# musbenlahrech/reporter

Measured on AMD Instinct MI355X. Metric: GPS points map-matched/sec (node) at 1/2/4/8 MI355X; % of HBM peak, higher is better.
Workload: dtype f32 geometry / f64 Viterbi + times / u64 (dist,time) route keys

## Files before the change

include/reporter_match.h:

```cpp
#ifndef REPORTER_MATCH_H
#define REPORTER_MATCH_H
#include <stddef.h>
#include <stdint.h>

#ifdef __cplusplus
extern "C" {
#endif

#define RM_ABI_VERSION 1

const char* rm_last_error(void);
int rm_abi_version(void);
int rm_set_device(int device);
int rm_device_count(int* count);

typedef struct rm_matcher rm_matcher;
int rm_configure(const char* conf_json_path, char* err, size_t errlen);
rm_matcher* rm_matcher_create(void);
void rm_matcher_destroy(rm_matcher* m);
int rm_match(rm_matcher* m, const char* trace_json, char** out_json);
int rm_match_batch(rm_matcher* m, const char* const* traces, size_t n, char** outs);
int rm_match_batch_packed(rm_matcher* m, const char* const* traces, size_t n, char** buf, uint64_t* off);
int rm_match_points(rm_matcher* m, const char* trace_json, char** out_json);
int rm_match_points_batch(rm_matcher* m, const char* const* traces, size_t n, char** outs);
void rm_free(char* p);
int rm_matcher_timing(const rm_matcher* m, double out[6]);
int rm_coalesce_stats(uint64_t out[4]);
int rm_coalesce_timing(double out[4]);

typedef struct {
  int32_t mode;
  float sigma_z, beta, search_radius, gps_accuracy, breakage_distance, interpolation_distance,
      max_route_distance_factor, max_route_time_factor, turn_penalty_factor;
} rm_options;
void rm_default_options(rm_options* o);

typedef struct {
  uint32_t rows, cols;
  double block_m;
  uint64_t seed;
  double center_lat, center_lon, jitter;
  uint32_t arterial_every, highway_every;
  double segment_max_m, internal_m, service_frac, oneway_frac, curve_frac, cell_m;
} rm_world_params;
void rm_default_world_params(rm_world_params* p);
int rm_world_build(const rm_world_params* p, const char* out_path);
int rm_graph_info(const char* graph_path, uint64_t out[7]);
int rm_graph_export_osm(const char* graph_path, const char* osm_path);
int rm_graph_export_pbf(const char* graph_path, const char* pbf_path);
int rm_graph_import_osm(const char* osm_path, const char* graph_path, double cell_m);
typedef struct {
  uint32_t rows, cols;
  double block_m;
  uint64_t seed;
  double center_lat, center_lon, jitter;
  uint32_t primary_every, secondary_every, boulevard_every, diagonal_every;
  double roundabout_frac, drop_frac, oneway_frac, spur_frac, service_frac, footway_frac, osmlr_local_frac,
      way_max_m;
  uint32_t trunk;
} rm_city_params;
void rm_default_city_params(rm_city_params* p);
int rm_osm_city_write(const rm_city_params* p, const char* osm_path, int pbf);

typedef struct {
  uint32_t n_traces, n_points;
  double rate_s, noise_m;
  uint64_t seed;
  int32_t mode;
  int64_t start_epoch;
  uint32_t threads;
} rm_trace_params;
void rm_default_trace_params(rm_trace_params* p);
int rm_traces_generate(const char* graph_path, const rm_trace_params* p, double* lon, double* lat, double* time,
                       float* accuracy, uint32_t* truth_edge, uint32_t* truth_off_cm);
int rm_traces_generate_ids(const char* graph_path, const rm_trace_params* p, const uint32_t* ids, double* lon,
                           double* lat, double* time, float* accuracy, uint32_t* truth_edge, uint32_t* truth_off_cm);

typedef struct rm_engine rm_engine;
typedef struct rm_runner rm_runner;

rm_engine* rm_engine_create(const char* graph_path, int device);
void rm_engine_destroy(rm_engine* e);
uint32_t rm_engine_n_segments(const rm_engine* e);
int rm_engine_segment_ids(const rm_engine* e, uint64_t* ids);
int rm_engine_set_ball_radius(rm_engine* e, double radius_m);
int rm_graph_auto_ball_radius(const char* graph_path, double* radius_m);
int rm_graph_fit_ball_radius(const char* graph_path, int mode, double start_m, double avail_gb, double* radius_m);
int rm_graph_ball_sample(const char* graph_path, int mode, double radius_m, double out[3]);
int rm_engine_ball_stats(const rm_engine* e, int mode, double out[6]);
int rm_engine_grid_split(const rm_engine* e, uint32_t* f);
int rm_engine_grid_alt(const rm_engine* e, uint32_t* f, float* radius_m);
int rm_engine_turn_rows(const rm_engine* e, uint32_t* mode_mask, double* build_ms );
int rm_graph_grid_split(const char* graph_path, uint32_t* f);
int rm_engine_ball_lookup(rm_engine* e, int mode, uint64_t n, const uint32_t* from, const uint32_t* road,
                          uint64_t* keys, uint8_t* preds);
int rm_balls_lookup(const char* graph_path, int mode, double radius_m, uint64_t n, const uint32_t* from,
                    const uint32_t* road, uint64_t* keys, uint8_t* preds);

rm_runner* rm_runner_create(rm_engine* e);
void rm_runner_destroy(rm_runner* r);

typedef struct {
  uint32_t n_traces;
  const uint32_t* trace_off;
  const float* lon;
  const float* lat;
  const double* time;
  const float* accuracy;
  uint32_t n_opts;
  const rm_options* opts;
  const uint32_t* trace_opt;
} rm_batch_desc;

typedef struct {
  double threshold_sec;
  uint32_t report_mask;
  uint32_t transition_mask;
  uint32_t* hist_dev;
  int32_t do_report;
  int32_t zero_hist;
  uint64_t* dur_dev;
} rm_run_params;
void rm_default_run_params(rm_run_params* p);

int rm_runner_run(rm_runner* r, const rm_batch_desc* b, const rm_run_params* p);
int rm_runner_rerun(rm_runner* r, const rm_run_params* p);
int rm_runners_rerun(rm_runner* const* rs, uint32_t n, const rm_run_params* p);
int rm_runner_sizes(rm_runner* r, uint64_t out[10]);
int rm_runner_route_tiers(rm_runner* r, uint64_t out[10]);
int rm_runner_get_states(rm_runner* r, uint32_t* n_states, uint32_t* state_orig);
int rm_runner_get_candidates(rm_runner* r, uint8_t* cand_n, uint32_t* road, uint32_t* s_cm, float* sq);
int rm_runner_get_routes(rm_runner* r, uint32_t* trans_off, double* gc, uint32_t* route_cm);
int rm_runner_get_route_terms(rm_runner* r, double* route_d, int* present);
int rm_runner_get_viterbi(rm_runner* r, int8_t* choice, uint8_t* chain_start);
int rm_runner_get_paths(rm_runner* r, uint32_t* path_off, uint32_t* path_cnt, uint32_t* path_edges, uint32_t* route_dist);
typedef struct {
  float lon, lat;
  float sq;
  uint32_t edge;
  uint32_t off_cm;
  uint32_t way;
  uint32_t type;
  uint32_t route_cm;
} rm_matched_point;
int rm_runner_get_matched_points(rm_runner* r, rm_matched_point* out);
int rm_runner_get_segments(rm_runner* r, uint32_t* seg_off, void* segs);
int rm_runner_get_reports(rm_runner* r, uint32_t* rep_off, void* reps, void* stats);
int rm_runner_set_isolation(rm_runner* r, int on);
int rm_runner_trace_errors(rm_runner* r, uint32_t* errs);
int rm_runner_set_locality(rm_runner* r, int mode);
int rm_runner_locality_used(rm_runner* r, int* used);
int rm_runner_set_timing(rm_runner* r, int on);
int rm_runner_set_timing_mask(rm_runner* r, uint32_t mask);
int rm_runner_kernel_times(rm_runner* r, double* ms, uint64_t* launches, int n);
int rm_runner_reset_times(rm_runner* r);
const char* rm_kernel_name(int k);
int rm_num_kernels(void);

typedef struct {
  uint32_t n_traces;
  const uint32_t* seg_off;
  const void* segs;
  const double* trace_end_time;
  const double* threshold_sec;
  const uint32_t* report_mask;
  const uint32_t* transition_mask;
} rm_report_desc;
int rm_report_segments(const rm_report_desc* d, uint32_t* rep_off, void* reps, void* stats);

typedef struct rm_comm rm_comm;
typedef struct {
  uint64_t n_points;
  const uint32_t* uuid;
  const double* time;
  const float* lon;
  const float* lat;
  const float* accuracy;
  double inactivity_sec;
  uint32_t n_uuids;
  uint32_t n_opts;
  const rm_options* opts;
  const uint32_t* uuid_opt;
} rm_points_desc;
int rm_runner_run_points(rm_runner* r, const rm_points_desc* d, const rm_run_params* p);
int rm_runner_get_trace_uuid(rm_runner* r, uint32_t* uuid);
int rm_runner_get_batch(rm_runner* r, uint32_t* trace_off, float* lon, float* lat, double* time, float* accuracy);
typedef struct {
  uint32_t quantisation;
  uint32_t privacy;
  const char* source;
  const char* mode;
} rm_tile_params;
void rm_default_tile_params(rm_tile_params* p);
int rm_runner_tiles(rm_runner* r, const rm_tile_params* p, rm_comm* comm, char** blob, size_t* len);

int rm_comm_unique_id(uint8_t id_out[128]);
rm_comm* rm_comm_init(int nranks, int rank, const uint8_t id[128], int device);
void rm_comm_destroy(rm_comm* c);
int rm_comm_allreduce(rm_comm* c, void* dev_buf, size_t count, int dtype, int op);
int rm_comm_reduce_scatter(rm_comm* c, void* buf, size_t count_per_rank, int dtype, int op);
int rm_comm_allreduce_host_f64(rm_comm* c, double* value, int op);
int rm_comm_barrier(rm_comm* c);
typedef int (*rm_host_allgather_fn)(void* ctx, const void* send, size_t bytes, void* recv);
rm_comm* rm_comm_init_host(int nranks, int rank, rm_host_allgather_fn fn, void* ctx, int device);
int rm_tile_file_owner(uint64_t bucket, uint32_t tile, int nranks);

int rm_device_alloc(size_t bytes, void** dev_ptr);
int rm_device_free(void* dev_ptr);
int rm_device_memset(void* dev_ptr, int value, size_t bytes);
int rm_device_download(void* host_dst, const void* dev_src, size_t bytes);
int rm_device_upload(void* dev_dst, const void* host_src, size_t bytes);
int rm_device_synchronize(void);

#ifdef __cplusplus
}
#endif
#endif
```

reporter_amd/_lib.py:

```python
import ctypes as C
import os
import threading

_HERE = os.path.dirname(os.path.abspath(__file__))
LIB_PATH = os.environ.get("REPORTER_MATCH_LIB") or os.path.join(_HERE, "libreporter_match.so")

_lock = threading.Lock()
_lib = None


class RmOptions(C.Structure):
    _fields_ = [("mode", C.c_int32), ("sigma_z", C.c_float), ("beta", C.c_float), ("search_radius", C.c_float),
                ("gps_accuracy", C.c_float), ("breakage_distance", C.c_float), ("interpolation_distance", C.c_float),
                ("max_route_distance_factor", C.c_float), ("max_route_time_factor", C.c_float),
                ("turn_penalty_factor", C.c_float)]


class RmWorldParams(C.Structure):
    _fields_ = [("rows", C.c_uint32), ("cols", C.c_uint32), ("block_m", C.c_double), ("seed", C.c_uint64),
                ("center_lat", C.c_double), ("center_lon", C.c_double), ("jitter", C.c_double),
                ("arterial_every", C.c_uint32), ("highway_every", C.c_uint32), ("segment_max_m", C.c_double),
                ("internal_m", C.c_double), ("service_frac", C.c_double), ("oneway_frac", C.c_double),
                ("curve_frac", C.c_double), ("cell_m", C.c_double)]


class RmCityParams(C.Structure):
    _fields_ = [("rows", C.c_uint32), ("cols", C.c_uint32), ("block_m", C.c_double), ("seed", C.c_uint64),
                ("center_lat", C.c_double), ("center_lon", C.c_double), ("jitter", C.c_double),
                ("primary_every", C.c_uint32), ("secondary_every", C.c_uint32), ("boulevard_every", C.c_uint32),
                ("diagonal_every", C.c_uint32), ("roundabout_frac", C.c_double), ("drop_frac", C.c_double),
                ("oneway_frac", C.c_double), ("spur_frac", C.c_double), ("service_frac", C.c_double),
                ("footway_frac", C.c_double), ("osmlr_local_frac", C.c_double), ("way_max_m", C.c_double),
                ("trunk", C.c_uint32)]


class RmTraceParams(C.Structure):
    _fields_ = [("n_traces", C.c_uint32), ("n_points", C.c_uint32), ("rate_s", C.c_double),
                ("noise_m", C.c_double), ("seed", C.c_uint64), ("mode", C.c_int32), ("start_epoch", C.c_int64),
                ("threads", C.c_uint32)]


class RmBatchDesc(C.Structure):
    _fields_ = [("n_traces", C.c_uint32), ("trace_off", C.c_void_p), ("lon", C.c_void_p), ("lat", C.c_void_p),
                ("time", C.c_void_p), ("accuracy", C.c_void_p), ("n_opts", C.c_uint32),
                ("opts", C.c_void_p), ("trace_opt", C.c_void_p)]


class RmRunParams(C.Structure):
    _fields_ = [("threshold_sec", C.c_double), ("report_mask", C.c_uint32), ("transition_mask", C.c_uint32),
                ("hist_dev", C.c_void_p), ("do_report", C.c_int32), ("zero_hist", C.c_int32),
                ("dur_dev", C.c_void_p)]


class RmPointsDesc(C.Structure):
    _fields_ = [("n_points", C.c_uint64), ("uuid", C.c_void_p), ("time", C.c_void_p), ("lon", C.c_void_p),
                ("lat", C.c_void_p), ("accuracy", C.c_void_p), ("inactivity_sec", C.c_double),
                ("n_uuids", C.c_uint32), ("n_opts", C.c_uint32), ("opts", C.c_void_p), ("uuid_opt", C.c_void_p)]


class RmReportDesc(C.Structure):
    _fields_ = [("n_traces", C.c_uint32), ("seg_off", C.c_void_p), ("segs", C.c_void_p),
                ("trace_end_time", C.c_void_p), ("threshold_sec", C.c_void_p), ("report_mask", C.c_void_p),
                ("transition_mask", C.c_void_p)]


class RmMatchedPoint(C.Structure):
    _fields_ = [("lon", C.c_float), ("lat", C.c_float), ("sq", C.c_float), ("edge", C.c_uint32),
                ("off_cm", C.c_uint32), ("way", C.c_uint32), ("type", C.c_uint32), ("route_cm", C.c_uint32)]


class RmTileParams(C.Structure):
    _fields_ = [("quantisation", C.c_uint32), ("privacy", C.c_uint32), ("source", C.c_char_p), ("mode", C.c_char_p)]


P = C.c_void_p
U32P = C.POINTER(C.c_uint32)

PROTOTYPES = [
    ("rm_last_error", C.c_char_p, []),
    ("rm_abi_version", C.c_int, []),
    ("rm_set_device", C.c_int, [C.c_int]),
    ("rm_device_count", C.c_int, [C.POINTER(C.c_int)]),
    ("rm_configure", C.c_int, [C.c_char_p, C.c_char_p, C.c_size_t]),
    ("rm_matcher_create", P, []),
    ("rm_matcher_destroy", None, [P]),
    ("rm_match", C.c_int, [P, C.c_char_p, C.POINTER(P)]),
    ("rm_match_batch", C.c_int, [P, C.POINTER(C.c_char_p), C.c_size_t, C.POINTER(P)]),
    ("rm_match_batch_packed", C.c_int, [P, C.POINTER(C.c_char_p), C.c_size_t, C.POINTER(P), C.POINTER(C.c_uint64)]),
    ("rm_match_points", C.c_int, [P, C.c_char_p, C.POINTER(P)]),
    ("rm_match_points_batch", C.c_int, [P, C.POINTER(C.c_char_p), C.c_size_t, C.POINTER(P)]),
    ("rm_free", None, [P]),
    ("rm_matcher_timing", C.c_int, [P, P]),
    ("rm_coalesce_stats", C.c_int, [C.POINTER(C.c_uint64)]),
    ("rm_coalesce_timing", C.c_int, [C.POINTER(C.c_double)]),
    ("rm_default_options", None, [C.POINTER(RmOptions)]),
    ("rm_default_world_params", None, [C.POINTER(RmWorldParams)]),
    ("rm_world_build", C.c_int, [C.POINTER(RmWorldParams), C.c_char_p]),
    ("rm_graph_info", C.c_int, [C.c_char_p, C.POINTER(C.c_uint64)]),
    ("rm_graph_export_osm", C.c_int, [C.c_char_p, C.c_char_p]),
    ("rm_graph_export_pbf", C.c_int, [C.c_char_p, C.c_char_p]),
    ("rm_graph_import_osm", C.c_int, [C.c_char_p, C.c_char_p, C.c_double]),
    ("rm_default_city_params", None, [C.POINTER(RmCityParams)]),
    ("rm_osm_city_write", C.c_int, [C.POINTER(RmCityParams), C.c_char_p, C.c_int]),
    ("rm_default_trace_params", None, [C.POINTER(RmTraceParams)]),
    ("rm_traces_generate", C.c_int, [C.c_char_p, C.POINTER(RmTraceParams), P, P, P, P, P, P]),
    ("rm_traces_generate_ids", C.c_int, [C.c_char_p, C.POINTER(RmTraceParams), P, P, P, P, P, P, P]),
    ("rm_engine_create", P, [C.c_char_p, C.c_int]),
    ("rm_engine_destroy", None, [P]),
    ("rm_engine_n_segments", C.c_uint32, [P]),
    ("rm_engine_segment_ids", C.c_int, [P, P]),
    ("rm_engine_set_ball_radius", C.c_int, [P, C.c_double]),
    ("rm_engine_ball_stats", C.c_int, [P, C.c_int, P]),
    ("rm_engine_grid_split", C.c_int, [P, P]),
    ("rm_engine_grid_alt", C.c_int, [P, P, P]),
    ("rm_engine_turn_rows", C.c_int, [P, P, P]),
    ("rm_engine_ball_lookup", C.c_int, [P, C.c_int, C.c_uint64, P, P, P, P]),
    ("rm_runner_route_tiers", C.c_int, [P, P]),
    ("rm_balls_lookup", C.c_int, [C.c_char_p, C.c_int, C.c_double, C.c_uint64, P, P, P, P]),
    ("rm_graph_auto_ball_radius", C.c_int, [C.c_char_p, P]),
    ("rm_graph_fit_ball_radius", C.c_int, [C.c_char_p, C.c_int, C.c_double, C.c_double, P]),
    ("rm_graph_ball_sample", C.c_int, [C.c_char_p, C.c_int, C.c_double, P]),
    ("rm_graph_grid_split", C.c_int, [C.c_char_p, P]),
    ("rm_runner_create", P, [P]),
    ("rm_runner_destroy", None, [P]),
    ("rm_default_run_params", None, [C.POINTER(RmRunParams)]),
    ("rm_runner_run", C.c_int, [P, C.POINTER(RmBatchDesc), C.POINTER(RmRunParams)]),
    ("rm_runner_rerun", C.c_int, [P, C.POINTER(RmRunParams)]),
    ("rm_runners_rerun", C.c_int, [P, C.c_uint32, C.POINTER(RmRunParams)]),
    ("rm_runner_sizes", C.c_int, [P, C.POINTER(C.c_uint64)]),
    ("rm_runner_get_states", C.c_int, [P, P, P]),
    ("rm_runner_get_candidates", C.c_int, [P, P, P, P, P]),
    ("rm_runner_get_routes", C.c_int, [P, P, P, P]),
    ("rm_runner_get_route_terms", C.c_int, [P, P, P]),
    ("rm_runner_get_viterbi", C.c_int, [P, P, P]),
    ("rm_runner_get_paths", C.c_int, [P, P, P, P, P]),
    ("rm_runner_get_matched_points", C.c_int, [P, P]),
    ("rm_runner_get_segments", C.c_int, [P, P, P]),
    ("rm_runner_get_reports", C.c_int, [P, P, P, P]),
    ("rm_runner_set_timing", C.c_int, [P, C.c_int]),
    ("rm_runner_set_timing_mask", C.c_int, [P, C.c_uint32]),
    ("rm_runner_set_isolation", C.c_int, [P, C.c_int]),
    ("rm_runner_trace_errors", C.c_int, [P, P]),
    ("rm_runner_set_locality", C.c_int, [P, C.c_int]),
    ("rm_runner_locality_used", C.c_int, [P, C.POINTER(C.c_int)]),
    ("rm_report_segments", C.c_int, [C.POINTER(RmReportDesc), P, P, P]),
    ("rm_runner_kernel_times", C.c_int, [P, P, P, C.c_int]),
    ("rm_runner_reset_times", C.c_int, [P]),
    ("rm_kernel_name", C.c_char_p, [C.c_int]),
    ("rm_num_kernels", C.c_int, []),
    ("rm_runner_run_points", C.c_int, [P, C.POINTER(RmPointsDesc), C.POINTER(RmRunParams)]),
    ("rm_runner_get_trace_uuid", C.c_int, [P, P]),
    ("rm_runner_get_batch", C.c_int, [P, P, P, P, P, P]),
    ("rm_default_tile_params", None, [C.POINTER(RmTileParams)]),
    ("rm_runner_tiles", C.c_int, [P, C.POINTER(RmTileParams), P, C.POINTER(P), C.POINTER(C.c_size_t)]),
    ("rm_comm_unique_id", C.c_int, [P]),
    ("rm_comm_init", P, [C.c_int, C.c_int, P, C.c_int]),
    ("rm_comm_destroy", None, [P]),
    ("rm_comm_allreduce", C.c_int, [P, P, C.c_size_t, C.c_int, C.c_int]),
    ("rm_comm_reduce_scatter", C.c_int, [P, P, C.c_size_t, C.c_int, C.c_int]),
    ("rm_comm_allreduce_host_f64", C.c_int, [P, C.POINTER(C.c_double), C.c_int]),
    ("rm_comm_barrier", C.c_int, [P]),
    ("rm_comm_init_host", P, [C.c_int, C.c_int, P, P, C.c_int]),
    ("rm_tile_file_owner", C.c_int, [C.c_uint64, C.c_uint32, C.c_int]),
    ("rm_device_alloc", C.c_int, [C.c_size_t, C.POINTER(P)]),
    ("rm_device_free", C.c_int, [P]),
    ("rm_device_memset", C.c_int, [P, C.c_int, C.c_size_t]),
    ("rm_device_download", C.c_int, [P, P, C.c_size_t]),
    ("rm_device_upload", C.c_int, [P, P, C.c_size_t]),
    ("rm_device_synchronize", C.c_int, []),
]


def lib():
    global _lib
    if _lib is not None:
        return _lib
    with _lock:
        if _lib is None:
            if not os.path.exists(LIB_PATH):
                raise ImportError("libreporter_match.so not built at %s (run python -m reporter_amd.build)" % LIB_PATH)
            h = C.CDLL(LIB_PATH)
            for name, res, args in PROTOTYPES:
                f = getattr(h, name)
                f.restype = res
                f.argtypes = args
            _lib = h
    return _lib


class RmError(RuntimeError):
    pass


def check(rc):
    if rc != 0:
        raise RmError(lib().rm_last_error().decode("utf-8", "replace"))
    return rc


def last_error():
    return lib().rm_last_error().decode("utf-8", "replace")
```

reporter_amd/csrc/capi.cpp:

```cpp
#include <hip/hip_runtime.h>
#include <rccl/rccl.h>

#include <atomic>
#include <sys/resource.h>
#include <cctype>
#include <chrono>
#include <cmath>
#include <condition_variable>
#include <deque>
#include <thread>
#include <vector>
#include <cstdio>
#include <cstring>
#include <memory>
#include <mutex>
#include <string>

#include "../../include/reporter_match.h"
#include "engine.hpp"
#include "graph.hpp"
#include "host_pool.hpp"
#include "json.hpp"
#include "osm_model.hpp"
#include "serve_policy.hpp"
// ... 1099 lines not shown
}

int rm_graph_grid_split(const char* graph_path, uint32_t* f) {
  return guarded([&] {
    if (!f) throw std::runtime_error("f is NULL");
    *f = choose_grid_split(Graph::load(graph_path));
  });
}

int rm_graph_auto_ball_radius(const char* graph_path, double* radius_m) {
  return guarded([&] {
    if (!radius_m) throw std::runtime_error("radius_m is NULL");
    *radius_m = auto_ball_radius_cm(Graph::load(graph_path)) / 100.0;
  });
}

int rm_graph_fit_ball_radius(const char* graph_path, int mode, double start_m, double avail_gb, double* radius_m) {
  return guarded([&] {
    if (!graph_path || !radius_m) throw std::runtime_error("path or radius_m is NULL");
    if (mode < 0 || mode > kModePedestrian) throw std::runtime_error("unknown travel mode");
    if (!(start_m >= 0.0) || start_m * 100.0 > kBallMaxRadiusCm) throw std::runtime_error("ball radius out of range (0..10000 m)");
    if (!(avail_gb >= 0.0)) throw std::runtime_error("avail_gb must be non-negative");
    const uint64_t avail = (uint64_t)std::min(avail_gb * (double)(1ull << 30), 1.8e19);
    *radius_m = fit_ball_radius_cm(Graph::load(graph_path), mode, (uint32_t)(start_m * 100.0), avail) / 100.0;
  });
}

int rm_graph_ball_sample(const char* graph_path, int mode, double radius_m, double out[3]) {
  return guarded([&] {
    if (!graph_path || !out) throw std::runtime_error("path or out is NULL");
    if (mode < 0 || mode > kModePedestrian) throw std::runtime_error("unknown travel mode");
    if (!(radius_m >= 0.0) || radius_m * 100.0 > kBallMaxRadiusCm) throw std::runtime_error("ball radius out of range (0..10000 m)");
    const BallSample bs = sample_balls(Graph::load(graph_path), (uint32_t)(radius_m * 100.0), kBallMaxKeysHost, mode);
    out[0] = bs.nodes; out[1] = bs.table_bytes; out[2] = bs.skipped_frac;
  });
}

int rm_balls_lookup(const char* graph_path, int mode, double radius_m, uint64_t n, const uint32_t* from,
                    const uint32_t* road, uint64_t* keys, uint8_t* preds) {
  return guarded([&] {
    if (mode < 0 || mode > kModePedestrian) throw std::runtime_error("unknown travel mode");
    if (!(radius_m >= 0.0) || radius_m * 100.0 > kBallMaxRadiusCm) throw std::runtime_error("ball radius out of range (0..10000 m)");
    Graph g = Graph::load(graph_path);
    BallTables bt;
    build_balls(g, mode, (uint32_t)(radius_m * 100.0), kBallMaxKeysHost, 4, bt);
    for (uint64_t i = 0; i < n; ++i) {
      keys[2 * i] = keys[2 * i + 1] = kKeyInf;
      if (preds) preds[2 * i] = preds[2 * i + 1] = (uint8_t)kBallPredNone;
      if (from[i] >= g.num_nodes() || road[i] >= g.num_roads()) throw std::runtime_error("node or road out of range");
      const uint32_t off = bt.hdr[2 * (size_t)from[i]], bits = bt.hdr[2 * (size_t)from[i] + 1];
      if (!bits) continue;
      const uint32_t mask = (1u << bits) - 1u;
      for (uint32_t s = ball_slot(road[i], bits);; s = (s + 1) & mask) {
        const uint32_t* e = bt.ent.data() + 4 * (ball_row0(off) + s);
        if (e[0] == kNone) break;
        if ((e[0] & bt.road_mask) != road[i]) continue;
        keys[2 * i] = ball_key0(e[0], e[1], e[3]);
        keys[2 * i + 1] = ball_key1(e[0], e[2], e[3]);
        if (preds) {
          preds[2 * i] = (uint8_t)ball_pred(e[0], 0, bt.road_mask);
          preds[2 * i + 1] = (uint8_t)ball_pred(e[0], 1, bt.road_mask);
        }
        break;
      }
    }
  });
}

rm_runner* rm_runner_create(rm_engine* e) {
  rm_runner* out = nullptr;
  guarded([&] {
    if (!e) throw std::runtime_error("engine is NULL");
    auto r = std::make_unique<rm_runner>();
    r->e = e->e;
    r->m = std::make_unique<Matcher>(e->e.get());
    out = r.release();
  });
  return out;
}
void rm_runner_destroy(rm_runner* r) { delete r; }

void rm_default_run_params(rm_run_params* p) {
  p->threshold_sec = 15.0; p->report_mask = 0x6; p->transition_mask = 0x6; p->hist_dev = nullptr; p->do_report = 1;
  p->zero_hist = 0; p->dur_dev = nullptr;
}

static RunParams to_rp(const rm_run_params* p) {
  RunParams rp;
  if (p) {
    rp.threshold_sec = p->threshold_sec; rp.report_mask = p->report_mask; rp.transition_mask = p->transition_mask;
    rp.hist = p->hist_dev; rp.do_report = p->do_report; rp.zero_hist = p->zero_hist;
    rp.dur = (unsigned long long*)p->dur_dev;
  }
  return rp;
}

int rm_runner_run(rm_runner* r, const rm_batch_desc* b, const rm_run_params* p) {
  return guarded([&] {
    HostBatch hb;
    hb.n_traces = b->n_traces; hb.trace_off = b->trace_off; hb.lon = b->lon; hb.lat = b->lat; hb.time = b->time;
    hb.accuracy = b->accuracy; hb.n_opts = b->n_opts; hb.opts = (const MatchOptions*)b->opts; hb.trace_opt = b->trace_opt;
    r->m->run(hb, to_rp(p));
  });
}
int rm_runner_rerun(rm_runner* r, const rm_run_params* p) { return guarded([&] { r->m->run_device(to_rp(p)); }); }

int rm_runners_rerun(rm_runner* const* rs, uint32_t n, const rm_run_params* p) {
  return guarded([&] {
    if (!rs || n == 0) throw std::runtime_error("no runners");
    for (uint32_t i = 0; i < n; ++i)
      if (!rs[i]) throw std::runtime_error("runner is NULL");
    RunParams rp = to_rp(p);
    if ((rp.hist || rp.dur) && rp.zero_hist && rp.do_report) {
      hipStream_t st = rs[0]->m->stream();
      const size_t nseg = rs[0]->m->engine().n_segments();
      if (rp.hist) RM_HIP(hipMemsetAsync(rp.hist, 0, nseg * kHistBins * sizeof(uint32_t), st));
      if (rp.dur) RM_HIP(hipMemsetAsync(rp.dur, 0, nseg * 8u, st));
      RM_HIP(hipStreamSynchronize(st));
    }
    rp.zero_hist = false;
    std::vector<std::exception_ptr> err(n);
    std::vector<std::thread> th;
    th.reserve(n - 1);
    for (uint32_t i = 1; i < n; ++i)
      th.emplace_back([&, i] {
        try { rs[i]->m->run_device(rp); } catch (...) { err[i] = std::current_exception(); }
      });
    try { rs[0]->m->run_device(rp); } catch (...) { err[0] = std::current_exception(); }
    for (auto& t : th) t.join();
    for (auto& e : err)
      if (e) std::rethrow_exception(e);
  });
}
int rm_runner_sizes(rm_runner* r, uint64_t out[10]) {
  return guarded([&] {
    out[0] = r->m->n_points(); out[1] = r->m->n_traces(); out[2] = r->m->n_trans(); out[3] = r->m->n_path_edges();
    out[4] = r->m->count_segments(); out[5] = r->m->count_reports();
    uint32_t t[4];
    r->m->tier_counts(t);
    for (int i = 0; i < 4; ++i) out[6 + i] = t[i];
  });
}
int rm_runner_route_tiers(rm_runner* r, uint64_t out[10]) {
  return guarded([&] {
    uint32_t c[kCtlWords];
    r->m->ctl_words(c);
    out[0] = c[1]; out[1] = c[3]; out[2] = c[5]; out[3] = c[8]; out[4] = c[9]; out[5] = c[10];
    out[6] = c[11]; out[7] = c[12]; out[8] = c[13]; out[9] = c[14];
#ifdef RM_K2_STATS
    out[9] = c[15];
#endif
  });
}
int rm_runner_get_states(rm_runner* r, uint32_t* a, uint32_t* b) { return guarded([&] { r->m->get_states(a, b); }); }
int rm_runner_get_candidates(rm_runner* r, uint8_t* a, uint32_t* b, uint32_t* c, float* d) {
  return guarded([&] { r->m->get_candidates(a, b, c, d); });
}
int rm_runner_get_routes(rm_runner* r, uint32_t* a, double* b, uint32_t* c) { return guarded([&] { r->m->get_routes(a, b, c); }); }
int rm_runner_get_route_terms(rm_runner* r, double* a, int* present) {
  return guarded([&] { *present = r->m->get_route_terms(a); });
}
int rm_runner_get_viterbi(rm_runner* r, int8_t* a, uint8_t* b) { return guarded([&] { r->m->get_viterbi(a, b); }); }
int rm_runner_get_paths(rm_runner* r, uint32_t* a, uint32_t* b, uint32_t* c, uint32_t* d) {
  return guarded([&] { r->m->get_paths(a, b, c, d); });
}
int rm_runner_get_matched_points(rm_runner* r, rm_matched_point* out) {
  static_assert(sizeof(rm_matched_point) == sizeof(MatchedPoint), "rm_matched_point is rm::MatchedPoint");
  return guarded([&] { r->m->matched_points(reinterpret_cast<MatchedPoint*>(out)); });
}
int rm_runner_get_segments(rm_runner* r, uint32_t* off, void* segs) {
  return guarded([&] { r->m->get_segments(off, (SegmentRec*)segs); });
}
int rm_runner_get_reports(rm_runner* r, uint32_t* off, void* reps, void* stats) {
  return guarded([&] { r->m->get_reports(off, (ReportRec*)reps, (ReportStats*)stats); });
}
int rm_runner_set_timing(rm_runner* r, int on) { return guarded([&] { r->m->set_timing(on != 0); }); }
int rm_runner_set_timing_mask(rm_runner* r, uint32_t mask) { return guarded([&] { r->m->set_timing_mask(mask); }); }
int rm_runner_set_isolation(rm_runner* r, int on) { return guarded([&] { r->m->set_isolation(on != 0); }); }
int rm_runner_set_locality(rm_runner* r, int mode) {
  return guarded([&] {
    if (mode < -1 || mode > 2) throw std::runtime_error("locality mode must be -1, 0, 1 or 2");
    r->m->set_locality(mode);
  });
}
int rm_runner_locality_used(rm_runner* r, int* used) { return guarded([&] { *used = r->m->locality_used() ? 1 : 0; }); }
int rm_runner_trace_errors(rm_runner* r, uint32_t* errs) { return guarded([&] { r->m->get_trace_errors(errs); }); }
int rm_report_segments(const rm_report_desc* d, uint32_t* rep_off, void* reps, void* stats) {
  return guarded([&] {
    if (!d || !rep_off || (d->n_traces && (!d->seg_off || !d->trace_end_time || !d->threshold_sec || !d->report_mask ||
                                           !d->transition_mask || !stats)))
      throw std::runtime_error("report descriptor or output is NULL");
    report_segments(g_device, d->n_traces, d->seg_off, (const SegmentRec*)d->segs, d->trace_end_time, d->threshold_sec,
                    d->report_mask, d->transition_mask, rep_off, (ReportRec*)reps, (ReportStats*)stats);
  });
}
int rm_runner_kernel_times(rm_runner* r, double* ms, uint64_t* launches, int n) {
  return guarded([&] {
    double t[kNumKernels];
    uint64_t l[kNumKernels];
    r->m->sync();
    r->m->kernel_times(t, l);
    for (int i = 0; i < n && i < kNumKernels; ++i) { ms[i] = t[i]; if (launches) launches[i] = l[i]; }
  });
}
int rm_runner_reset_times(rm_runner* r) { return guarded([&] { r->m->reset_kernel_times(); }); }
const char* rm_kernel_name(int k) { return (k >= 0 && k < kNumKernels) ? kKernelNames[k] : ""; }
int rm_num_kernels(void) { return kNumKernels; }

}

struct rm_comm {
  ncclComm_t comm = nullptr;
  hipStream_t stream = nullptr;
  void* scratch = nullptr;
  int device = 0;
  int rank = 0, nranks = 1;
  rm_host_allgather_fn host_fn = nullptr;
  void* host_ctx = nullptr;
  std::atomic<bool> broken{false};
};

namespace {
double comm_timeout_s();
bool comm_timeout_exit() {
  const char* e = std::getenv("RM_COMM_TIMEOUT_EXIT");
  return !(e && *e == '0');
}

constexpr uint32_t kWatchSlots = 64;
struct CommWatch {
  std::atomic<uint64_t> deadline_ns[kWatchSlots];
  const char* what[kWatchSlots];
  int rank[kWatchSlots], nranks[kWatchSlots], limit_s[kWatchSlots];
  CommWatch() {
    for (uint32_t i = 0; i < kWatchSlots; ++i) deadline_ns[i].store(0);
  }
};
CommWatch& comm_watch() {
  static CommWatch* w = [] {
    CommWatch* x = new CommWatch();
    std::thread([x] {
      for (;;) {
        std::this_thread::sleep_for(std::chrono::milliseconds(50));
        const uint64_t now = (uint64_t)std::chrono::duration_cast<std::chrono::nanoseconds>(
                                 std::chrono::steady_clock::now().time_since_epoch()).count();
        for (uint32_t i = 0; i < kWatchSlots; ++i) {
          const uint64_t d = x->deadline_ns[i].load(std::memory_order_acquire);
          if (d && now > d) {
            std::fprintf(stderr, "%s: rank %d of %d: the other ranks did not join within %d s (RM_COMM_TIMEOUT_S); "
                                 "exiting with status 3\n", x->what[i], x->rank[i], x->nranks[i], x->limit_s[i]);
            std::fflush(stderr);
            std::_Exit(3);
          }
        }
      }
    }).detach();
    return x;
  }();
  return *w;
}
uint32_t comm_watch_slot() {
  static std::atomic<uint32_t> next{0};
  thread_local const uint32_t slot = next.fetch_add(1) % kWatchSlots;
  return slot;
}

template <class F>
void comm_bounded(rm_comm* c, int rank, int nranks, const char* what, F fn) {
  if (c && c->broken.load()) throw std::runtime_error(std::string(what) + ": the communicator missed a deadline earlier and is unusable");
  const double limit = comm_timeout_s();
  struct St {
    std::mutex mu;
    std::condition_variable cv;
    bool done = false;
    std::exception_ptr err;
  };
  auto st = std::make_shared<St>();
  if (comm_timeout_exit()) {
    CommWatch& w = comm_watch();
    const uint32_t slot = comm_watch_slot();
    w.what[slot] = what;
    w.rank[slot] = rank;
    w.nranks[slot] = nranks;
    w.limit_s[slot] = (int)limit;
    const auto now = std::chrono::steady_clock::now().time_since_epoch();
    w.deadline_ns[slot].store((uint64_t)std::chrono::duration_cast<std::chrono::nanoseconds>(now).count() +
                              (uint64_t)(limit * 1e9), std::memory_order_release);
    try {
      fn();
    } catch (...) {
      w.deadline_ns[slot].store(0, std::memory_order_release);
      throw;
    }
    w.deadline_ns[slot].store(0, std::memory_order_release);
    return;
  }
  std::thread worker([st, fn]() mutable {
    std::exception_ptr e;
    try {
      fn();
    } catch (...) {
      e = std::current_exception();
    }
    std::lock_guard<std::mutex> lk(st->mu);
    st->err = e;
    st->done = true;
// ... 345 lines not shown
```

reporter_amd/csrc/engine.hip:

```cpp
#include <hip/hip_runtime.h>
#include <hipcub/hipcub.hpp>

#include <algorithm>
#include <chrono>
#include <cstdlib>
#include <cstring>
#include <functional>
#include <thread>
#include <type_traits>

#include "engine.hpp"
#include "json_points.hpp"

namespace rm {

const char* const kKernelNames[kNumKernels] = {"states", "candidates", "scan", "routes",
                                               "viterbi", "paths", "segments", "report", "locality",
                                               "points"};

namespace {

constexpr uint32_t kEmpty = 0xffffffffu;
constexpr int kWave = 64;
constexpr int kBigH = 4096;
constexpr int kMidH = 512;
constexpr uint32_t kMidGrid = 4096;
constexpr int kCandH = 256;
constexpr int kReg2Grid = 512;
constexpr uint32_t kMaxBoundCm = 100000000u;
constexpr double kQueueSpeedMps = 2.7777777777777777;

struct DevBatch {
  uint32_t T;
  uint64_t P;
  const uint32_t* trace_off; const float* lon; const float* lat; const double* time; const float* acc;
  const MatchOptions* opts; const uint32_t* trace_opt;
  uint32_t* slot_trace; uint32_t* n_states; uint32_t* state_orig; double* state_time;
  uint8_t* cand_n; uint4* cand_desc; float* cand_sq;
  uint32_t* trans_cnt; uint32_t* trans_off; double* gc; uint32_t* route; uint4* pair_info;
  double* route_d;
  uint32_t* walk;
  uint32_t* src_cnt; uint32_t* src_off; uint32_t* src_item;
  int8_t* choice; uint8_t* chain_start; uint8_t* bp;
  uint32_t* path_off; uint32_t* path_cnt; uint32_t* path_inline; uint32_t* path_pool; uint64_t path_cap; uint32_t* route_dist;
  uint2* path_sab;
  SegmentRec* segs; uint32_t* seg_base; uint32_t* seg_cnt;
  uint32_t* trav_off;
  ReportRec* reps; uint32_t* rep_cnt; ReportStats* stats;
  uint32_t* rl_routes_0;
  uint32_t* ctl; uint32_t* rl_routes_a; uint32_t* rl_routes_b; uint32_t* rl_paths_a; uint32_t* rl_paths_b;
  uint32_t* rl_cand;
  uint32_t* rl_routes_c; uint32_t* rl_paths_c;
  uint32_t* trace_err;
  const uint32_t* perm;
  const uint32_t* perm_paths;
  uint32_t search_delta;
  const unsigned long long* tot;
  uint64_t seg_cap;
  uint64_t trans_cap, src_cap;
  uint32_t gate;
};

__device__ __forceinline__ bool steady_abort(const DevBatch& b) {
  return (b.gate & 4u) && (b.tot[0] > b.trans_cap || b.tot[1] > b.src_cap);
}

__device__ __forceinline__ bool small_abort(const DevBatch& b) {
  if (!b.gate) return false;
  const uint32_t* c = b.ctl;
  return (c[2] & kErrPathOverflow) != 0u || ((b.gate & 2u) && (c[9] | c[10]) != 0u) || b.tot[2] > b.seg_cap ||
         steady_abort(b);
}

__device__ __forceinline__ void trace_fail(const DevBatch& b, uint64_t p, uint32_t bit) {
  atomicOr(&b.trace_err[b.slot_trace[p]], bit);
  atomicOr(&b.ctl[2], bit);
}

__device__ __forceinline__ bool edge_ok(uint32_t info, uint32_t acc) { return (((info >> 16) & 7u) & acc) != 0u; }
__device__ __forceinline__ uint64_t edge_key(const uint4& r, int mode) {
  return make_key(r.y, time_ms(r.y, mode_speed_dkph(mode, r.z & 0xffffu)));
}
__device__ __forceinline__ float as_f(uint32_t u) { return __uint_as_float(u); }

__device__ __forceinline__ float point_radius(const MatchOptions& o, float acc) {
  float r = o.search_radius;
  if (acc >= 0.0f && acc > r) r = acc;
  if (r > kMaxSearchRadius) r = kMaxSearchRadius;
  if (!(r > 0.0f)) r = 0.0f;
  return r;
}

__device__ __forceinline__ uint32_t xcd_block(uint32_t i, uint32_t n) {
  const uint32_t x = i & 7u, idx = i >> 3, q = n >> 3, r = n & 7u;
  return x < r ? x * (q + 1u) + idx : r * (q + 1u) + (x - r) * q + idx;
}

__device__ __forceinline__ uint32_t route_bound(double gc, const MatchOptions& o) {
  double maxd = gc * (double)o.max_route_distance_factor;
  if ((double)o.breakage_distance < maxd) maxd = (double)o.breakage_distance;
  double bcm = floor(maxd * 100.0);
  if (!(bcm >= 0.0)) bcm = 0.0;
  return bcm > (double)kMaxBoundCm ? kMaxBoundCm : (uint32_t)bcm;
}
__device__ __forceinline__ double route_term(uint32_t route_cm, uint32_t U, uint32_t factor_bits, double gc) {
  if (route_cm == kRouteInvalid) return __longlong_as_double(0x7ff0000000000000ll);
  const double tm = (double)U * ((double)__uint_as_float(factor_bits) * 0x1p-16);
  return tm + fabs((double)route_cm * 0.01 - gc);
}
__device__ __forceinline__ uint32_t time_bound(double dt, const MatchOptions& o) {
  if (!(dt > 0.0)) return 0xffffffffu;
  const double tm = floor(dt * (double)o.max_route_time_factor * 1000.0);
  return tm >= 4294967295.0 ? 0xffffffffu : (uint32_t)tm;
}

__device__ __forceinline__ uint32_t morton_spread16(uint32_t v) {
  v &= 0xffffu;
  v = (v | (v << 8)) & 0x00ff00ffu;
  v = (v | (v << 4)) & 0x0f0f0f0fu;
  v = (v | (v << 2)) & 0x33333333u;
  v = (v | (v << 1)) & 0x55555555u;
  return v;
}
constexpr uint32_t kLocBucketBits = 12, kLocBuckets = 1u << kLocBucketBits;
constexpr uint32_t kLocPerThread = 16;
__device__ __forceinline__ uint32_t loc_bucket(const DevGraph& g, const DevBatch& b, uint64_t p, uint32_t shift) {
  const uint32_t k = b.slot_trace[p];
  const uint32_t o = b.trace_off[k];
  if ((uint32_t)(p - o) >= b.n_states[k]) return kLocBuckets;
  const uint32_t pt = o + b.state_orig[p];
  const double fx = floor(((double)b.lon[pt] - g.lon0) / g.dlon), fy = floor(((double)b.lat[pt] - g.lat0) / g.dlat);
  const uint32_t cx = fx < 0.0 ? 0u : (fx > (double)(g.ncx - 1) ? g.ncx - 1 : (uint32_t)fx);
  const uint32_t cy = fy < 0.0 ? 0u : (fy > (double)(g.ncy - 1) ? g.ncy - 1 : (uint32_t)fy);
  return morton_spread16(min(cx >> shift, 63u)) | (morton_spread16(min(cy >> shift, 63u)) << 1);
}
__global__ void __launch_bounds__(256) k_loc_count(DevGraph g, DevBatch b, uint32_t shift, uint16_t* key,
                                                   uint32_t* hist) {
  __shared__ uint32_t h[kLocBuckets + 1];
  for (uint32_t q = threadIdx.x; q <= kLocBuckets; q += 256) h[q] = 0u;
  __syncthreads();
  const uint64_t p0 = (uint64_t)blockIdx.x * (256u * kLocPerThread) + threadIdx.x;
#pragma unroll 4
  for (uint32_t i = 0; i < kLocPerThread; ++i) {
    const uint64_t p = p0 + 256u * i;
    if (p < b.P) {
      const uint32_t kk = loc_bucket(g, b, p, shift);
      key[p] = (uint16_t)kk;
      atomicAdd(&h[kk], 1u);
    }
  }
  __syncthreads();
  for (uint32_t q = threadIdx.x; q <= kLocBuckets; q += 256)
    if (h[q]) atomicAdd(&hist[q], h[q]);
}
__global__ void __launch_bounds__(1024) k_loc_scan(uint32_t* hist) {
  __shared__ uint32_t ws[16];
  constexpr uint32_t per = (kLocBuckets + 1 + 1023) / 1024;
  const uint32_t q0 = threadIdx.x * per;
  uint32_t v[per], t = 0;
#pragma unroll
  for (uint32_t i = 0; i < per; ++i) { v[i] = q0 + i <= kLocBuckets ? hist[q0 + i] : 0u; t += v[i]; }
  const int lane = threadIdx.x & 63, wv = threadIdx.x >> 6;
  uint32_t incl = t;
#pragma unroll
  for (int d = 1; d < 64; d <<= 1) {
    const uint32_t u = __shfl_up(incl, d, 64);
    if (lane >= d) incl += u;
  }
  if (lane == 63) ws[wv] = incl;
  __syncthreads();
  uint32_t base = 0;
  for (int w = 0; w < wv; ++w) base += ws[w];
  uint32_t at = base + incl - t;
#pragma unroll
  for (uint32_t i = 0; i < per; ++i) {
    if (q0 + i <= kLocBuckets) hist[q0 + i] = at;
    at += v[i];
  }
}
__global__ void __launch_bounds__(256) k_loc_scatter(uint64_t P, const uint16_t* key, uint32_t* cursor, uint32_t* perm) {
  __shared__ uint32_t h[kLocBuckets + 1];
  for (uint32_t q = threadIdx.x; q <= kLocBuckets; q += 256) h[q] = 0u;
  __syncthreads();
  const uint64_t p0 = (uint64_t)blockIdx.x * (256u * kLocPerThread) + threadIdx.x;
  uint32_t kk[kLocPerThread], rk[kLocPerThread];
#pragma unroll
  for (uint32_t i = 0; i < kLocPerThread; ++i) {
    const uint64_t p = p0 + 256u * i;
    kk[i] = p < P ? key[p] : 0xffffu;
    rk[i] = kk[i] != 0xffffu ? atomicAdd(&h[kk[i]], 1u) : 0u;
  }
  __syncthreads();
  for (uint32_t q = threadIdx.x; q <= kLocBuckets; q += 256)
    if (h[q]) h[q] = atomicAdd(&cursor[q], h[q]);
  __syncthreads();
#pragma unroll
  for (uint32_t i = 0; i < kLocPerThread; ++i)
    if (kk[i] != 0xffffu) perm[h[kk[i]] + rk[i]] = (uint32_t)(p0 + 256u * i);
}
__global__ void __launch_bounds__(256) k_perm_src_count(DevBatch b, uint32_t* pcnt, unsigned long long* part);
__global__ void __launch_bounds__(256) k_scan_apply_perm(const uint32_t* a, uint64_t n, const unsigned long long* part,
                                                         const uint32_t* perm, uint32_t* src_off);

__device__ __forceinline__ float lane_f(float v, uint32_t q) {
  return __int_as_float(__builtin_amdgcn_readlane(__float_as_int(v), (int)q));
}
__device__ __forceinline__ double lane_d(double v, uint32_t q) {
  const unsigned long long u = __double_as_longlong(v);
  const uint32_t lo = (uint32_t)__builtin_amdgcn_readlane((int)(uint32_t)u, (int)q);
  const uint32_t hi = (uint32_t)__builtin_amdgcn_readlane((int)(uint32_t)(u >> 32), (int)q);
  return __longlong_as_double(((unsigned long long)hi << 32) | lo);
}

__global__ void __launch_bounds__(64) k_states(DevBatch b) {
  const uint32_t k = blockIdx.x;
  if (k >= b.T) return;
  const int lane = threadIdx.x;
  if (lane == 0) b.trace_err[k] = 0u;
  if (k == 0 && lane < kCtlWords) b.ctl[lane] = 0u;
  const uint32_t o = b.trace_off[k], n = b.trace_off[k + 1] - o;
  const MatchOptions op = b.opts[b.trace_opt[k]];
  const double interp = (double)op.interpolation_distance;
  uint32_t ns = 0, last = 0;
  float llon = 0.f, llat = 0.f;
  double lsin = 0.0, lcos = 0.0;
  float c1lo = 0.f, c1la = 0.f, c2lo = 0.f, c2la = 0.f;
  const uint32_t nl = n ? n - 1u : 0u;
  float nlo = b.lon[o + min((uint32_t)lane, nl)], nla = b.lat[o + min((uint32_t)lane, nl)];
  bool w_slot = false, w_state = false, w_gc = false;
  uint32_t w_i = 0, w_si = 0;
  double w_gcv = 0.0;
  for (uint32_t c0 = 0; c0 < n; c0 += 64) {
    const uint32_t i = c0 + lane, m = min(64u, n - c0);
    const bool act = i < n;
    float lo = act ? nlo : 0.f, la = act ? nla : 0.f;
    __asm__ volatile("" : "+v"(lo), "+v"(la) : : "memory");
    if (w_slot) b.slot_trace[o + w_i] = k;
    if (w_state) b.state_orig[o + w_si] = w_i;
    if (w_gc) b.gc[o + w_si] = w_gcv;
    __asm__ volatile("" : : : "memory");
    nlo = b.lon[o + min(i + 64u, nl)];
    nla = b.lat[o + min(i + 64u, nl)];
    w_slot = act;
    w_i = i;
    float lo1 = __shfl_up(lo, 1, 64), la1 = __shfl_up(la, 1, 64);
    float lo2 = __shfl_up(lo, 2, 64), la2 = __shfl_up(la, 2, 64);
    if (lane == 0) { lo1 = c1lo; la1 = c1la; lo2 = c2lo; la2 = c2la; }
    if (lane == 1) { lo2 = c1lo; la2 = c1la; }
    const double s0 = lat_sin(la), k0 = lat_cos(la);
    double s1 = __shfl_up(s0, 1, 64), k1 = __shfl_up(k0, 1, 64), s2 = __shfl_up(s0, 2, 64), k2 = __shfl_up(k0, 2, 64);
    if (lane <= 1) {
      const float cl = lane == 0 ? c2la : c1la;
      s2 = lat_sin(cl); k2 = lat_cos(cl);
      if (lane == 0) { s1 = lat_sin(c1la); k1 = lat_cos(c1la); }
    }
    const double d1 = gc_trig(lo1, la1, s1, k1, lo, la, s0, k0);
    const double d2 = gc_trig(lo2, la2, s2, k2, lo, la, s0, k0);
    const bool a1 = act && (i == 0 || !(d1 < interp));
    const bool a2 = act && i >= 2 && !(d2 < interp);
    const unsigned long long A = __ballot(a1), B = __ballot(a2);
    unsigned long long st = 0;
    const uint32_t last0 = last;
    double dx = 0.0;
    for (uint32_t q = 0; q < m;) {
      const uint32_t ii = c0 + q;
      if (ii == 0 || last + 1 == ii) {
        const unsigned long long rest = ~(A >> q);
        const uint32_t run = min(rest ? (uint32_t)__builtin_ctzll(rest) : 64u, m - q);
        if (run) {
          st |= (run == 64u ? ~0ull : ((1ull << run) - 1ull)) << q;
          q += run;
          last = c0 + q - 1;
        } else {
          ++q;
        }
        continue;
      }
      if (last + 2 == ii) {
        if ((B >> q) & 1ull) { st |= 1ull << q; last = ii; }
        ++q;
        continue;
      }
      float plo = llon, pla = llat;
      double ps = lsin, pc = lcos;
      if (last >= c0) {
        plo = lane_f(lo, last - c0); pla = lane_f(la, last - c0);
        ps = lane_d(s0, last - c0); pc = lane_d(k0, last - c0);
      }
      const double dv = gc_trig(plo, pla, ps, pc, lo, la, s0, k0);
      const unsigned long long far = __ballot(act && !(dv < interp)) & (~0ull << q);
      if (!far) { q = m; break; }
      const uint32_t nq = (uint32_t)__builtin_ctzll(far);
      st |= 1ull << nq;
      last = c0 + nq;
      if (lane == (int)nq) dx = dv;
      q = nq + 1;
    }
    w_state = ((st >> lane) & 1ull) != 0ull;
    w_gc = false;
    if (w_state) {
      const unsigned long long below = st & ((1ull << lane) - 1ull);
      const uint32_t si = ns + (uint32_t)__popcll(below);
      w_si = si;
      if (si > 0) {
        const uint32_t prev = below ? c0 + 63u - (uint32_t)__builtin_clzll(below) : last0;
        w_gc = true;
        w_gcv = i - prev == 1u ? d1 : (i - prev == 2u ? d2 : dx);
      }
    }
    ns += (uint32_t)__popcll(st);
    if (last >= c0) {
      llon = lane_f(lo, last - c0); llat = lane_f(la, last - c0);
      lsin = lane_d(s0, last - c0); lcos = lane_d(k0, last - c0);
    }
    c1lo = lane_f(lo, 63); c1la = lane_f(la, 63);
    c2lo = lane_f(lo, 62); c2la = lane_f(la, 62);
  }
  if (w_slot) b.slot_trace[o + w_i] = k;
  if (w_state) b.state_orig[o + w_si] = w_i;
  if (w_gc) b.gc[o + w_si] = w_gcv;
  if (lane == 0) b.n_states[k] = ns;
}

struct CandSmem {
  uint32_t road[kCandH];
  unsigned long long best[kCandH];
  uint32_t cell_lo[64], cell_hi[64];
  uint32_t used, ovf, ncell, slot_n;
  uint32_t list[kCandH];
};

__device__ __forceinline__ void project_rel(float ax, float ay, uint32_t acum, float bx, float by, uint32_t bcum,
                                            float& sq, uint32_t& s) {
  const float dx = bx - ax, dy = by - ay;
  const float l2 = dx * dx + dy * dy;
  float t = 0.0f;
  if (l2 > 0.0f) {
    t = -(ax * dx + ay * dy) / l2;
    if (t < 0.0f) t = 0.0f;
    if (t > 1.0f) t = 1.0f;
  }
  const float cx = ax + t * dx, cy = ay + t * dy;
  sq = cx * cx + cy * cy;
  const float along = (float)acum + t * (float)(bcum - acum);
  uint32_t v = (uint32_t)rintf(along);
  if (v < acum) v = acum;
  if (v > bcum) v = bcum;
  s = v;
}
__device__ __forceinline__ void project(float alon, float alat, uint32_t acum, float blon, float blat, uint32_t bcum,
                                        float lon, float lat, float mlon, float mlat, float& sq, uint32_t& s) {
  project_rel((alon - lon) * mlon, (alat - lat) * mlat, acum, (blon - lon) * mlon, (blat - lat) * mlat, bcum, sq, s);
}
#ifndef RM_K1_REJECT
#define RM_K1_REJECT 0
#endif
__device__ __forceinline__ bool outside_pad(float ax, float ay, float bx, float by, float pad) {
  if (!RM_K1_REJECT) return false;
  return (ax > pad && bx > pad) || (ax < -pad && bx < -pad) || (ay > pad && by > pad) || (ay < -pad && by < -pad);
}

__device__ __forceinline__ uint32_t time_ms_dev(uint32_t d_cm, uint32_t dkph) {
  if (d_cm > 11930464u) return time_ms(d_cm, dkph);
  const uint32_t D = dkph ? dkph : 1u;
  return (uint32_t)((double)(d_cm * 360u) / (double)D);
}

__device__ __forceinline__ void desc_from_rec(const uint4& a, const uint4& c, uint32_t road, uint32_t s, int mode,
                                              uint32_t acc, uint4& d0, uint4& d1) {
  uint32_t spf = (a.w != kNone && edge_ok(c.y, acc)) ? mode_speed_dkph(mode, c.y & 0xffffu) : 0u;
  uint32_t spr = (c.x != kNone && edge_ok(c.z, acc)) ? mode_speed_dkph(mode, c.z & 0xffffu) : 0u;
  if (a.w != kNone && edge_ok(c.y, acc) && spf == 0u) spf = 1u;
  if (c.x != kNone && edge_ok(c.z, acc) && spr == 0u) spr = 1u;
  d0 = make_uint4(road, s, a.z, spf | (spr << 16));
  d1 = make_uint4(a.x, a.y, spf ? time_ms_dev(s, spf) : 0xffffffffu, spr ? time_ms_dev(a.z - s, spr) : 0xffffffffu);
}

__device__ __forceinline__ void make_desc(const DevGraph& g, uint32_t road, uint32_t s, int mode, uint4& d0,
                                          uint4& d1) {
  desc_from_rec(g.road_rec[2 * (uint64_t)road], g.road_rec[2 * (uint64_t)road + 1], road, s, mode, mode_access(mode),
                d0, d1);
}

__device__ __forceinline__ void put_cand(const DevGraph& g, const DevBatch& b, uint64_t p, uint32_t rank, uint32_t road,
                                         uint32_t s, float sq, int mode) {
  uint4 d0, d1;
  make_desc(g, road, s, mode, d0, d1);
  const uint64_t at = p * kMaxCand + rank;
  b.cand_desc[2 * at] = d0;
  b.cand_desc[2 * at + 1] = d1;
  b.cand_sq[at] = sq;
}

#define K1_UNIFORM_STOP(c) (__ballot(c) == 0ull)

#ifndef RM_K1_ROWS
#define RM_K1_ROWS 4
#endif
constexpr int kK1Rows = RM_K1_ROWS;
#ifndef RM_K1_BATCH
#define RM_K1_BATCH 4
#endif
constexpr int kK1Batch = RM_K1_BATCH;
#ifndef RM_K1_SLOTS
#define RM_K1_SLOTS 16
#endif
constexpr int kK1Slots = RM_K1_SLOTS;
static_assert(kK1Slots % 4 == 0 && kK1Slots <= kMaxCand, "K1 slots");
#ifndef RM_K1_WPE
#define RM_K1_WPE 1
#endif
__global__ void __launch_bounds__(256) __attribute__((amdgpu_waves_per_eu(RM_K1_WPE))) k_candidates_lane(DevGraph g, DevBatch b) {
  uint64_t p = (uint64_t)blockIdx.x * blockDim.x + threadIdx.x;
  if (b.perm) {
    const uint64_t r = (uint64_t)xcd_block(blockIdx.x, gridDim.x) * blockDim.x + threadIdx.x;
    if (r >= b.P) return;
    p = b.perm[r];
  }
  if (p >= b.P) return;
  const uint32_t k = b.slot_trace[p];
  const uint32_t o = b.trace_off[k];
  const uint32_t s = (uint32_t)(p - o);
  if (s >= b.n_states[k]) return;
  const MatchOptions op = b.opts[b.trace_opt[k]];
  const uint32_t acc = mode_access(op.mode);
  const uint32_t pt = o + b.state_orig[p];
  const float lon = b.lon[pt], lat = b.lat[pt];
  const float r = point_radius(op, b.acc[pt]);
  const float mlon = meters_per_lon(lat);
  const float mlat = (float)kMetersPerDegLat;
  const float r2 = r * r;
  const float pad = r * 1.01f + 0.5f;
  const float qlon = pad / mlon, qlat = pad / mlat;
  const double fx0 = floor(((double)(lon - qlon) - g.lon0) / g.dlon);
  const double fx1 = floor(((double)(lon + qlon) - g.lon0) / g.dlon);
  const double fy0 = floor(((double)(lat - qlat) - g.lat0) / g.dlat);
  const double fy1 = floor(((double)(lat + qlat) - g.lat0) / g.dlat);
  uint32_t rroad[kK1Slots], rs[kK1Slots];
  unsigned long long rbest[kK1Slots];
  uint32_t n = 0;
  bool ovf = false;
  if (!(fx1 < 0 || fy1 < 0 || fx0 > (double)(g.ncx - 1) || fy0 > (double)(g.ncy - 1))) {
    const uint32_t x0 = fx0 < 0 ? 0u : (uint32_t)fx0, y0 = fy0 < 0 ? 0u : (uint32_t)fy0;
    const uint32_t x1 = fx1 > (double)(g.ncx - 1) ? g.ncx - 1 : (uint32_t)fx1;
    const uint32_t y1 = fy1 > (double)(g.ncy - 1) ? g.ncy - 1 : (uint32_t)fy1;
    for (uint32_t w0 = y0; w0 <= y1 && !ovf; w0 += kK1Rows) {
      const uint32_t nrow = min(y1 - w0 + 1u, (uint32_t)kK1Rows);
      uint32_t ra[kK1Rows], re[kK1Rows], base[kK1Rows], end[kK1Rows];
#pragma unroll
      for (int r = 0; r < kK1Rows; ++r) {
        const uint32_t cy = w0 + min((uint32_t)r, nrow - 1u);
        ra[r] = g.cell_off[cy * g.ncx + x0];
        re[r] = g.cell_off[cy * g.ncx + x1 + 1];
      }
      uint32_t tot = 0;
#pragma unroll
      for (int r = 0; r < kK1Rows; ++r) {
        base[r] = ra[r] - tot;
        tot += (uint32_t)r < nrow ? re[r] - ra[r] : 0u;
        end[r] = tot;
      }
      for (uint32_t q0 = 0; q0 < tot && !ovf; q0 += kK1Batch) {
        uint4 r0[kK1Batch], r1[kK1Batch];
#pragma unroll
        for (int y = 0; y < kK1Batch; ++y) {
          const uint32_t q = min(q0 + (uint32_t)y, tot - 1u);
          uint32_t bq = base[0];
#pragma unroll
          for (int r = 1; r < kK1Rows; ++r)
            if (q >= end[r - 1]) bq = base[r];
          const uint64_t it = bq + q;
          r0[y] = g.cell_rec[2 * it];
// ... 190 lines not shown
  const uint32_t n_items = all ? (uint32_t)b.P : min(b.ctl[7], (uint32_t)b.P);
  for (uint32_t item = blockIdx.x; item < n_items; item += gridDim.x) {
    const uint32_t p = all ? item : b.rl_cand[item];
    if (all) {
      const uint32_t k = b.slot_trace[p];
      if (p - b.trace_off[k] >= b.n_states[k]) continue;
    }
    cand_wave_one(g, b, sm, p);
    __syncthreads();
  }
}

__device__ __forceinline__ void block_sum2_u64(unsigned long long a, unsigned long long c, unsigned long long* part) {
  __shared__ unsigned long long sa[4], sc[4];
#pragma unroll
  for (int d = 32; d > 0; d >>= 1) {
    a += __shfl_down(a, d, 64);
    c += __shfl_down(c, d, 64);
  }
  if ((threadIdx.x & 63) == 0) { sa[threadIdx.x >> 6] = a; sc[threadIdx.x >> 6] = c; }
  __syncthreads();
  if (threadIdx.x == 0)
    reinterpret_cast<ulonglong2*>(part)[blockIdx.x] =
        make_ulonglong2(sa[0] + sa[1] + sa[2] + sa[3], sc[0] + sc[1] + sc[2] + sc[3]);
}

__device__ __forceinline__ void block_excl_scan2(unsigned long long a, unsigned long long c, unsigned long long& ea,
                                                 unsigned long long& ec, unsigned long long* sa, unsigned long long* sc,
                                                 int nwaves) {
  const int lane = threadIdx.x & 63, wv = threadIdx.x >> 6;
  unsigned long long ia = a, ic = c;
#pragma unroll
  for (int d = 1; d < 64; d <<= 1) {
    const unsigned long long ta = __shfl_up(ia, d, 64), tc = __shfl_up(ic, d, 64);
    if (lane >= d) { ia += ta; ic += tc; }
  }
  if (lane == 63) { sa[wv] = ia; sc[wv] = ic; }
  __syncthreads();
  unsigned long long ba = 0, bc = 0;
  for (int w = 0; w < nwaves; ++w) {
    const unsigned long long xa = sa[w], xc = sc[w];
    ba += w < wv ? xa : 0ull;
    bc += w < wv ? xc : 0ull;
  }
  ea = ba + ia - a;
  ec = bc + ic - c;
}

__global__ void __launch_bounds__(1024) k_scan_parts(unsigned long long* part, uint32_t nb, unsigned long long* out) {
  __shared__ unsigned long long sa[16], sc[16];
  const uint32_t per = (nb + 1023u) / 1024u;
  const uint32_t b0 = min(threadIdx.x * per, nb), b1 = min(b0 + per, nb);
  ulonglong2* pp = reinterpret_cast<ulonglong2*>(part);
  unsigned long long a = 0, c = 0;
#pragma unroll 8
  for (uint32_t q = b0; q < b1; ++q) { const ulonglong2 v = pp[q]; a += v.x; c += v.y; }
  unsigned long long ea, ec;
  block_excl_scan2(a, c, ea, ec, sa, sc, 16);
#pragma unroll 8
  for (uint32_t q = b0; q < b1; ++q) {
    const ulonglong2 v = pp[q];
    pp[q] = make_ulonglong2(ea, ec);
    ea += v.x;
    ec += v.y;
  }
  if (threadIdx.x == 1023) { out[0] = ea; out[1] = ec; }
}

__global__ void __launch_bounds__(256) k_scan_apply2(const uint32_t* a, const uint32_t* c, uint64_t n,
                                                     const unsigned long long* part, uint32_t* ao, uint32_t* co) {
  __shared__ uint32_t sa[4], sc[4];
  const uint64_t p = (uint64_t)blockIdx.x * 256u + threadIdx.x;
  const ulonglong2 base = reinterpret_cast<const ulonglong2*>(part)[blockIdx.x];
  const uint32_t va = p < n ? a[p] : 0u, vc = p < n ? c[p] : 0u;
  const int lane = threadIdx.x & 63, wv = threadIdx.x >> 6;
  uint32_t ia = va, ic = vc;
#pragma unroll
  for (int d = 1; d < 64; d <<= 1) {
    const uint32_t ta = __shfl_up(ia, d, 64), tc = __shfl_up(ic, d, 64);
    if (lane >= d) { ia += ta; ic += tc; }
  }
  if (lane == 63) { sa[wv] = ia; sc[wv] = ic; }
  __syncthreads();
  uint32_t ba = 0, bc = 0;
#pragma unroll
  for (int w = 0; w < 4; ++w) {
    ba += w < wv ? sa[w] : 0u;
    bc += w < wv ? sc[w] : 0u;
  }
  if (p < n) {
    ao[p] = (uint32_t)base.x + ba + ia - va;
    co[p] = (uint32_t)base.y + bc + ic - vc;
  }
}

__global__ void __launch_bounds__(256) k_scan_apply4(const uint32_t* a, uint64_t n, const unsigned long long* part,
                                                     uint32_t* ao) {
  __shared__ unsigned long long sa[4], sc[4];
  const uint64_t i = ((uint64_t)blockIdx.x * 256u + threadIdx.x) * 4u;
  uint32_t v[4] = {0u, 0u, 0u, 0u};
  if (i + 4 <= n) {
    const uint4 q = *reinterpret_cast<const uint4*>(a + i);
    v[0] = q.x; v[1] = q.y; v[2] = q.z; v[3] = q.w;
  } else {
    for (uint64_t x = i; x < n; ++x) v[x - i] = a[x];
  }
  unsigned long long ea, ec;
  block_excl_scan2((unsigned long long)v[0] + v[1] + v[2] + v[3], 0ull, ea, ec, sa, sc, 4);
  const unsigned long long base = part[2 * blockIdx.x] + ea;
  const uint32_t o0 = (uint32_t)base, o1 = o0 + v[0], o2 = o1 + v[1], o3 = o2 + v[2];
  if (i + 4 <= n) {
    *reinterpret_cast<uint4*>(ao + i) = make_uint4(o0, o1, o2, o3);
  } else {
    const uint32_t o[4] = {o0, o1, o2, o3};
    for (uint64_t x = i; x < n; ++x) ao[x] = o[x - i];
  }
}

__global__ void __launch_bounds__(256) k_perm_src_count(DevBatch b, uint32_t* pcnt, unsigned long long* part) {
  const uint64_t r = (uint64_t)blockIdx.x * 256u + threadIdx.x;
  uint32_t c = 0;
  if (r < b.P) {
    const uint64_t q = (uint64_t)b.perm[r] + 1u;
    c = q < b.P ? b.src_cnt[q] : 0u;
    pcnt[r] = c;
  }
  block_sum2_u64(c, 0ull, part);
}
__global__ void __launch_bounds__(256) k_scan_apply_perm(const uint32_t* a, uint64_t n, const unsigned long long* part,
                                                         const uint32_t* perm, uint32_t* src_off) {
  __shared__ uint32_t sa[4];
  const uint64_t r = (uint64_t)blockIdx.x * 256u + threadIdx.x;
  const uint32_t base = (uint32_t)reinterpret_cast<const ulonglong2*>(part)[blockIdx.x].x;
  const uint32_t v = r < n ? a[r] : 0u;
  const int lane = threadIdx.x & 63, wv = threadIdx.x >> 6;
  uint32_t iv = v;
#pragma unroll
  for (int d = 1; d < 64; d <<= 1) {
    const uint32_t t = __shfl_up(iv, d, 64);
    if (lane >= d) iv += t;
  }
  if (lane == 63) sa[wv] = iv;
  __syncthreads();
  uint32_t bb = 0;
#pragma unroll
  for (int w = 0; w < 4; ++w) bb += w < wv ? sa[w] : 0u;
  if (r < n && v) src_off[perm[r] + 1u] = base + bb + iv - v;
}

__global__ void __launch_bounds__(256) k_trans_count(DevBatch b, unsigned long long* part) {
  const uint64_t p = (uint64_t)blockIdx.x * blockDim.x + threadIdx.x;
  uint32_t c = 0, ns = 0;
  if (p < b.P) {
    b.choice[p] = -1;
    b.path_cnt[p] = 0u;
    const uint32_t k = b.slot_trace[p];
    const uint32_t o = b.trace_off[k];
    const uint32_t s = (uint32_t)(p - o);
    const uint32_t S = b.n_states[k];
    if (s < S) b.state_time[p] = b.time[o + b.state_orig[p]];
    if (s >= 1 && s < S) {
      const uint32_t KA = b.cand_n[p - 1], KB = b.cand_n[p];
      c = KA * KB;
      ns = KB ? KA : 0u;
      const uint32_t pa = o + b.state_orig[p - 1], pb = o + b.state_orig[p];
      const double gc = b.gc[p];
      const MatchOptions op = b.opts[b.trace_opt[k]];
      b.pair_info[p] = make_uint4(route_bound(gc, op), time_bound(b.time[pb] - b.time[pa], op),
                                  KA | (KB << 8) | ((uint32_t)op.mode << 16),
                                  op.turn_penalty_factor > 0.f ? __float_as_uint(op.turn_penalty_factor) : 0u);
    }
    b.trans_cnt[p] = c;
    b.src_cnt[p] = ns;
  }
  block_sum2_u64(c, ns, part);
}

__global__ void k_src_items(DevBatch b) {
  if (steady_abort(b)) return;
  const uint64_t p = (uint64_t)blockIdx.x * blockDim.x + threadIdx.x;
  if (p >= b.P) return;
  const uint32_t n = b.src_cnt[p], at = b.src_off[p];
  for (uint32_t i = 0; i < n; ++i) b.src_item[at + i] = (uint32_t)p;
}

__device__ __forceinline__ void block_prefix_parts(const unsigned long long* part, uint32_t nb, uint32_t upto,
                                                   unsigned long long* pre, unsigned long long* all) {
  __shared__ unsigned long long s[4][4];
  unsigned long long a = 0, c = 0, ta = 0, tc = 0;
  const ulonglong2* pp = reinterpret_cast<const ulonglong2*>(part);
  for (uint32_t q = threadIdx.x; q < nb; q += blockDim.x) {
    const ulonglong2 v = pp[q];
    ta += v.x; tc += v.y;
    if (q < upto) { a += v.x; c += v.y; }
  }
#pragma unroll
  for (int d = 32; d > 0; d >>= 1) {
    a += __shfl_down(a, d, 64); c += __shfl_down(c, d, 64);
    ta += __shfl_down(ta, d, 64); tc += __shfl_down(tc, d, 64);
  }
  const int wv = threadIdx.x >> 6;
  if ((threadIdx.x & 63) == 0) { s[wv][0] = a; s[wv][1] = c; s[wv][2] = ta; s[wv][3] = tc; }
  __syncthreads();
  for (int j = 0; j < 4; ++j) {
    unsigned long long x = 0;
    for (int w = 0; w < (int)(blockDim.x >> 6); ++w) x += s[w][j];
    if (j < 2) pre[j] = x; else all[j - 2] = x;
  }
}

__global__ void __launch_bounds__(256) k_trans_apply_small(DevBatch b, const unsigned long long* part, uint32_t nb,
                                                           unsigned long long* tot) {
  unsigned long long pre[2], all[2];
  block_prefix_parts(part, nb, blockIdx.x, pre, all);
  if (blockIdx.x == 0 && threadIdx.x == 0) { tot[0] = all[0]; tot[1] = all[1]; }
  __shared__ uint32_t sa[4], sc[4];
  const uint64_t p = (uint64_t)blockIdx.x * 256u + threadIdx.x;
  const uint32_t va = p < b.P ? b.trans_cnt[p] : 0u, vc = p < b.P ? b.src_cnt[p] : 0u;
  const int lane = threadIdx.x & 63, wv = threadIdx.x >> 6;
  uint32_t ia = va, ic = vc;
#pragma unroll
  for (int d = 1; d < 64; d <<= 1) {
    const uint32_t ta = __shfl_up(ia, d, 64), tc = __shfl_up(ic, d, 64);
    if (lane >= d) { ia += ta; ic += tc; }
  }
  if (lane == 63) { sa[wv] = ia; sc[wv] = ic; }
  __syncthreads();
  uint32_t ba = 0, bc = 0;
#pragma unroll
  for (int w = 0; w < 4; ++w) {
    ba += w < wv ? sa[w] : 0u;
    bc += w < wv ? sc[w] : 0u;
  }
  if (p < b.P) {
    const uint32_t at = (uint32_t)pre[1] + bc + ic - vc;
    b.trans_off[p] = (uint32_t)pre[0] + ba + ia - va;
    b.src_off[p] = at;
    for (uint32_t i = 0; i < vc; ++i) b.src_item[at + i] = (uint32_t)p;
  }
}

__global__ void __launch_bounds__(256) k_path_apply_small(DevBatch b, const unsigned long long* part, uint32_t nb,
                                                          unsigned long long* tot, uint32_t* rec_slot) {
  unsigned long long pre[2], all[2];
  block_prefix_parts(part, nb, blockIdx.x, pre, all);
  if (blockIdx.x == 0 && threadIdx.x == 0) tot[2] = all[0];
  __shared__ unsigned long long sa[4], sc[4];
  const uint64_t n = b.P;
  const uint64_t i = ((uint64_t)blockIdx.x * 256u + threadIdx.x) * 4u;
  uint32_t v[4] = {0u, 0u, 0u, 0u};
  for (uint64_t x = i; x < n && x < i + 4; ++x) v[x - i] = b.path_cnt[x];
  unsigned long long ea, ec;
  block_excl_scan2((unsigned long long)v[0] + v[1] + v[2] + v[3], 0ull, ea, ec, sa, sc, 4);
  uint64_t o = pre[0] + ea;
  for (uint64_t x = i; x < n && x < i + 4; ++x) {
    b.trav_off[x] = (uint32_t)o;
    const uint32_t c = v[x - i];
    for (uint32_t q = 0; q < c; ++q)
      if (o + q < b.seg_cap) rec_slot[o + q] = (uint32_t)x;
    o += c;
  }
}

__global__ void __launch_bounds__(64) k_gather_recs(uint32_t T, const uint32_t* base, const uint32_t* cnt,
                                                    const uint32_t* off, const unsigned long long* src, uint32_t words,
                                                    unsigned long long* dst) {
  for (uint32_t k = blockIdx.x; k < T; k += gridDim.x) {
    const uint64_t n = (uint64_t)cnt[k] * words;
    const unsigned long long* s = src + (uint64_t)base[k] * words;
    unsigned long long* d = dst + (uint64_t)off[k] * words;
    for (uint64_t q = threadIdx.x; q < n; q += 64) d[q] = s[q];
  }
}

__global__ void __launch_bounds__(1024) k_seg_offsets_small(DevBatch b, uint32_t* off) {
  __shared__ unsigned long long sa[16], sc[16];
  const uint32_t T = b.T;
  const bool off_gate = small_abort(b);
  const uint32_t per = (T + 1023u) / 1024u;
  const uint32_t k0 = min(threadIdx.x * per, T), k1 = min(k0 + per, T);
  unsigned long long a = 0;
  for (uint32_t k = k0; k < k1; ++k) a += off_gate ? 0u : b.seg_cnt[k];
  unsigned long long ea, ec;
  block_excl_scan2(a, 0ull, ea, ec, sa, sc, 16);
  for (uint32_t k = k0; k < k1; ++k) {
    off[k] = (uint32_t)ea;
    if (off_gate) b.seg_cnt[k] = 0u;
    else ea += b.seg_cnt[k];
  }
  if (threadIdx.x == 1023) off[T] = (uint32_t)ea;
}

__device__ __forceinline__ uint32_t d_spf(const uint4& d0) { return d0.w & 0xffffu; }
__device__ __forceinline__ uint32_t d_spr(const uint4& d0) { return d0.w >> 16; }

__device__ __forceinline__ unsigned long long route_key_vals(const uint4& a0, const uint4& b0, const uint4& b1,
                                                             unsigned long long lab0, unsigned long long lab1,
                                                             int* combo) {
  const uint32_t sa = a0.y, rb = b0.x, sb = b0.y, L = b0.z, spf = d_spf(b0), spr = d_spr(b0);
  unsigned long long best = kKeyInf;
  int bc = -1;
  if (a0.x == rb) {
    const bool fw = sb > sa || (sb == sa && spf);
    const uint32_t sp = fw ? spf : spr, d = fw ? sb - sa : sa - sb;
    if (sp) { best = make_key(d, time_ms_dev(d, sp)); bc = fw ? 0 : 1; }
  }
  if (spf && lab0 != kKeyInf) { const unsigned long long k = lab0 + make_key(sb, b1.z); if (k < best) { best = k; bc = 2; } }
  if (spr && lab1 != kKeyInf) { const unsigned long long k = lab1 + make_key(L - sb, b1.w); if (k < best) { best = k; bc = 3; } }
  if (combo) *combo = bc;
  return best;
}

template <class Label>
__device__ __forceinline__ unsigned long long route_key(const Label& label, const uint4& a0, const uint4& b0,
                                                        const uint4& b1, int* combo) {
  const unsigned long long lab0 = d_spf(b0) ? label(b1.x) : kKeyInf;
  const unsigned long long lab1 = d_spr(b0) ? label(b1.y) : kKeyInf;
  return route_key_vals(a0, b0, b1, lab0, lab1, combo);
}

__device__ __forceinline__ void exit_keys(const uint4& a0, uint32_t bound, unsigned long long& rk1,
                                          unsigned long long& rk0) {
  const uint32_t s = a0.y, L = a0.z, spf = d_spf(a0), spr = d_spr(a0);
  rk1 = (spf && L - s <= bound) ? make_key(L - s, time_ms_dev(L - s, spf)) : kKeyInf;
  rk0 = (spr && s <= bound) ? make_key(s, time_ms_dev(s, spr)) : kKeyInf;
}

template <int H, bool PATH>
struct SearchSmem {
  using FIdx = typename std::conditional<(H >= 65536), uint32_t, uint16_t>::type;
  uint32_t key[H];
  unsigned long long lab[H];
  FIdx fa[H], fb[H];
  uint32_t inq[(H + 31) / 32];
  uint32_t pred[PATH ? H : 1];
  uint32_t nf, nn, used, ovf;
};

__device__ __forceinline__ bool inq_set(uint32_t* inq, uint32_t slot) {
  const uint32_t bit = 1u << (slot & 31);
  return (atomicOr(&inq[slot >> 5], bit) & bit) == 0u;
}
__device__ __forceinline__ void inq_clear(uint32_t* inq, uint32_t slot) { atomicAnd(&inq[slot >> 5], ~(1u << (slot & 31))); }

template <int H, bool PATH>
__device__ __forceinline__ int h_insert(SearchSmem<H, PATH>& sm, uint32_t key) {
  uint32_t h = (key * 2654435761u) & (H - 1);
  for (int probe = 0; probe < H; ++probe) {
    uint32_t cur = sm.key[h];
    if (cur == key) return (int)h;
    if (cur == kEmpty) {
      cur = atomicCAS(&sm.key[h], kEmpty, key);
      if (cur == kEmpty) {
        if (atomicAdd(&sm.used, 1u) >= (uint32_t)(H * 3 / 4)) sm.ovf = 1u;
        return (int)h;
      }
      if (cur == key) return (int)h;
    }
    h = (h + 1) & (H - 1);
  }
  sm.ovf = 1u;
  return -1;
}

template <int H, bool PATH>
__device__ __forceinline__ int h_find(const SearchSmem<H, PATH>& sm, uint32_t key) {
  uint32_t h = (key * 2654435761u) & (H - 1);
  for (int probe = 0; probe < H; ++probe) {
    const uint32_t cur = sm.key[h];
    if (cur == key) return (int)h;
    if (cur == kEmpty) return -1;
    h = (h + 1) & (H - 1);
  }
  return -1;
}

template <int H, bool PATH>
__device__ __forceinline__ unsigned long long h_label(const SearchSmem<H, PATH>& sm, uint32_t key) {
  const int h = h_find(sm, key);
  return h < 0 ? kKeyInf : sm.lab[h];
}

__device__ __forceinline__ uint32_t wave_append(uint32_t* counter) {
  const unsigned long long m = __ballot(1);
  const int lane = (int)(threadIdx.x & (kWave - 1));
  const int leader = __builtin_ctzll(m);
  uint32_t base = 0;
  if (lane == leader) base = atomicAdd(counter, (uint32_t)__popcll(m));
  base = (uint32_t)__shfl((int)base, leader, kWave);
  return base + (uint32_t)__popcll(m & ((1ull << lane) - 1ull));
}

template <int H, bool PATH>
struct HashLabel {
  const SearchSmem<H, PATH>& sm;
  uint32_t srcbits;
  __device__ unsigned long long operator()(uint32_t node) const { return h_label(sm, srcbits | node); }
};
template <int H, bool PATH>
struct HashPathLabel {
  const SearchSmem<H, PATH>& sm;
  __device__ unsigned long long operator()(uint32_t node, uint32_t, uint32_t) const { return h_label(sm, node); }
};

struct SearchTargets {
  const uint4* tg;
  uint32_t n;
  uint32_t delta;
};

__device__ __forceinline__ void wave_sync() {
  __builtin_amdgcn_fence(__ATOMIC_RELEASE, "wavefront");
  __builtin_amdgcn_wave_barrier();
  __builtin_amdgcn_fence(__ATOMIC_ACQUIRE, "wavefront");
// ... 3407 lines not shown
                     d_inc, d_bits, (const uint2*)d_hdr, d_ent, d_stats);
  RM_HIP(hipGetLastError());
  RM_HIP(hipDeviceSynchronize());
  tmp.erase(std::remove(tmp.begin(), tmp.end(), (void*)d_hdr), tmp.end());
  tmp.erase(std::remove(tmp.begin(), tmp.end(), (void*)d_ent), tmp.end());
  allocs_.push_back(d_hdr);
  allocs_.push_back(d_ent);
  dg_.ball_hdr[mode] = d_hdr;
  dg_.ball_ent[mode] = d_ent;
  dg_.ball_radius[mode] = radius_cm;
  dg_.ball_mask |= 1u << mode;
  ball_bytes_ += total * 16;
  ball_info_[mode][0] = (double)st[0];
  ball_info_[mode][1] = (double)total;
  ball_info_[mode][2] = (double)st[2];
  ball_info_[mode][3] = std::chrono::duration<double, std::milli>(std::chrono::steady_clock::now() - t0).count();
  ball_gpu_ |= 1u << mode;
  return true;
}

void Engine::ball_lookup(int mode, uint64_t n, const uint32_t* from, const uint32_t* road, uint64_t* keys,
                         uint8_t* preds) {
  std::lock_guard<std::mutex> lk(ball_mu_);
  RM_HIP(hipSetDevice(device_));
  for (uint64_t i = 0; i < n; ++i) {
    keys[2 * i] = keys[2 * i + 1] = kKeyInf;
    if (preds) preds[2 * i] = preds[2 * i + 1] = (uint8_t)kBallPredNone;
    if (from[i] >= host_.num_nodes() || road[i] >= host_.num_roads()) throw std::runtime_error("node or road out of range");
  }
  if (!((ball_built_ >> mode) & 1u) || n == 0) return;
  std::vector<void*> tmp;
  struct Free { std::vector<void*>& l; ~Free() { for (void* p : l) (void)hipFree(p); } } fr{tmp};
  uint32_t* d_from = dalloc<uint32_t>(tmp, n);
  uint32_t* d_road = dalloc<uint32_t>(tmp, n);
  unsigned long long* d_keys = dalloc<unsigned long long>(tmp, 2 * n);
  uint8_t* d_pred = preds ? dalloc<uint8_t>(tmp, 2 * n) : nullptr;
  RM_HIP(hipMemcpy(d_from, from, n * 4, hipMemcpyHostToDevice));
  RM_HIP(hipMemcpy(d_road, road, n * 4, hipMemcpyHostToDevice));
  hipLaunchKernelGGL(k_ball_lookup, dim3((uint32_t)((n + 255) / 256)), dim3(256), 0, 0, dg_, mode, n, d_from, d_road,
                     d_keys, d_pred);
  RM_HIP(hipGetLastError());
  RM_HIP(hipMemcpy(keys, d_keys, 2 * n * 8, hipMemcpyDeviceToHost));
  if (preds) RM_HIP(hipMemcpy(preds, d_pred, 2 * n, hipMemcpyDeviceToHost));
}


Workspace::~Workspace() { release(); }
void Workspace::release() {
  for (void* p : allocs) (void)hipFree(p);
  allocs.clear();
  cap_points = cap_traces = cap_trans = cap_path = cap_opts = cap_segs = cap_src = cap_sort = cap_turn = 0;
  perm = loc_cursor = pcnt = nullptr;
  route_d = nullptr;
  walk = nullptr;
  cap_walk = 0;
  loc_key = nullptr;
}

Matcher::Matcher(Engine* e) : eng_(e) {
  RM_HIP(hipSetDevice(e->device()));
  RM_HIP(hipStreamCreateWithFlags(&stream_, hipStreamNonBlocking));
  if (const char* lv = std::getenv("RM_LOCALITY"); lv && *lv) locality_ = std::max(-1, std::min(2, std::atoi(lv)));
}

void Matcher::ensure_sort(uint64_t n) {
  grow_workspace([&] {
    Workspace& w = ws_;
    if (n <= w.cap_sort && w.perm) return;
    for (void** q : {(void**)&w.perm, (void**)&w.loc_key, (void**)&w.loc_cursor, (void**)&w.pcnt}) {
      if (*q) {
        (void)hipFree(*q);
        w.allocs.erase(std::find(w.allocs.begin(), w.allocs.end(), *q));
      }
      *q = nullptr;
    }
    w.cap_sort = 0;
    const uint64_t c = std::max<uint64_t>(n, w.cap_points);
    if (c >= (uint64_t)INT32_MAX) throw BatchTooLarge("batch too large for the locality sort");
    std::vector<void*>& L = w.allocs;
    w.perm = dalloc<uint32_t>(L, c);
    w.loc_key = dalloc<uint16_t>(L, c);
    w.loc_cursor = dalloc<uint32_t>(L, kLocBuckets + 1);
    w.pcnt = dalloc<uint32_t>(L, c);
    w.cap_sort = c;
  });
}

Matcher::~Matcher() {
  (void)hipSetDevice(eng_->device());
  if (stream_) (void)hipStreamSynchronize(stream_);
  for (auto& ev : pending_) { (void)hipEventDestroy(ev.a); (void)hipEventDestroy(ev.b); }
  for (auto& ev : free_ev_) { (void)hipEventDestroy(ev.a); (void)hipEventDestroy(ev.b); }
  ws_.release();
  if (dl_dev_) (void)hipFree(dl_dev_);
  if (mp_dev_) (void)hipFree(mp_dev_);
  if (dl_host_) (void)hipHostFree(dl_host_);
  for (void* q : {(void*)jdev_, jspan_, (void*)jflag_, jtsp_})
    if (q) (void)hipFree(q);
  if (stream_) (void)hipStreamDestroy(stream_);
  if (hctl_) (void)hipHostFree(hctl_);
  if (hpack_) (void)hipHostFree(hpack_);
  if (dpack_) (void)hipFree(dpack_);
  if (hoff_) (void)hipHostFree(hoff_);
}

void Matcher::ensure(uint64_t points, uint32_t traces, uint32_t nopts) {
  grow_workspace([&] {
    Workspace& w = ws_;
    if (points <= w.cap_points && traces <= w.cap_traces && nopts <= w.cap_opts && w.ctl) return;
    const uint64_t keep_trans = w.cap_trans, keep_path = w.cap_path, keep_segs = w.cap_segs, keep_src = w.cap_src;
    const uint64_t gp = std::max<uint64_t>(points, w.cap_points + w.cap_points / 2) + 64;
    const uint64_t gt = std::max<uint64_t>(traces, w.cap_traces + w.cap_traces / 2) + 16;
    const uint64_t go = std::max<uint64_t>(nopts, w.cap_opts + w.cap_opts / 2) + 4;
    try {
      alloc_points(gp, gt, go, keep_trans, keep_path, keep_segs, keep_src);
    } catch (const OutOfDeviceMemory&) {
      if (gp == points + 64 && gt == traces + 16 && go == nopts + 4) throw;
      alloc_points(points + 64, traces + 16, nopts + 4, 1, 1, 1, 1);
    }
  });
}

void Matcher::alloc_points(uint64_t cp, uint64_t ct, uint64_t co, uint64_t keep_trans, uint64_t keep_path,
                           uint64_t keep_segs, uint64_t keep_src) {
  {
    Workspace& w = ws_;
    w.release();
    if (const char* lim = std::getenv("RM_TEST_WS_POINTS_LIMIT"); lim && *lim && cp > std::strtoull(lim, nullptr, 10))
      throw OutOfDeviceMemory("workspace above RM_TEST_WS_POINTS_LIMIT");
    std::vector<void*>& L = w.allocs;
    w.trace_off = dalloc<uint32_t>(L, ct + 1);
    w.lon = dalloc<float>(L, cp); w.lat = dalloc<float>(L, cp); w.time = dalloc<double>(L, cp);
    w.acc = dalloc<float>(L, cp); w.opts = dalloc<MatchOptions>(L, co); w.trace_opt = dalloc<uint32_t>(L, ct);
    w.slot_trace = dalloc<uint32_t>(L, cp); w.n_states = dalloc<uint32_t>(L, ct); w.state_orig = dalloc<uint32_t>(L, cp);
    w.state_time = dalloc<double>(L, cp);
    w.cand_n = dalloc<uint8_t>(L, cp); w.cand_desc = dalloc<uint4>(L, cp * kMaxCand * 2);
    w.cand_sq = dalloc<float>(L, cp * kMaxCand); w.pair_info = dalloc<uint4>(L, cp);
    w.trans_cnt = dalloc<uint32_t>(L, cp); w.trans_off = dalloc<uint32_t>(L, cp); w.gc = dalloc<double>(L, cp);
    w.src_cnt = dalloc<uint32_t>(L, cp); w.src_off = dalloc<uint32_t>(L, cp);
    w.choice = dalloc<int8_t>(L, cp); w.chain_start = dalloc<uint8_t>(L, cp); w.bp = dalloc<uint8_t>(L, cp * kMaxCand);
    w.path_off = dalloc<uint32_t>(L, cp); w.path_cnt = dalloc<uint32_t>(L, cp); w.route_dist = dalloc<uint32_t>(L, cp);
    w.path_sab = dalloc<uint2>(L, cp);
    w.path_inline = dalloc<uint32_t>(L, cp * kInlinePath);
    w.trav_off = dalloc<uint32_t>(L, cp);
    w.seg_base = dalloc<uint32_t>(L, ct); w.seg_cnt = dalloc<uint32_t>(L, ct);
    w.rep_cnt = dalloc<uint32_t>(L, ct); w.stats = dalloc<ReportStats>(L, ct);
    w.ctl = dalloc<uint32_t>(L, kCtlWords);
    w.rl_paths_a = dalloc<uint32_t>(L, cp); w.rl_paths_b = dalloc<uint32_t>(L, cp);
    w.rl_cand = dalloc<uint32_t>(L, cp);
    w.rl_paths_c = dalloc<uint32_t>(L, cp);
    w.trace_err = dalloc<uint32_t>(L, ct);
    w.tot64 = dalloc<unsigned long long>(L, 4);
    w.tot_part = dalloc<unsigned long long>(L, 2 * ((cp + 255) / 256) + 2);
    w.cap_points = cp; w.cap_traces = ct; w.cap_opts = co;
    w.gsearch = nullptr;
    w.route = nullptr; w.route_d = nullptr; w.cap_turn = 0; w.walk = nullptr; w.cap_walk = 0; w.rl_routes_a = nullptr; w.rl_routes_b = nullptr; w.rl_routes_0 = nullptr; w.rl_routes_c = nullptr; w.path_pool = nullptr; w.segs = nullptr; w.reps = nullptr; w.src_item = nullptr; w.rec_slot = nullptr;
    w.cap_trans = 0; w.cap_path = 0; w.cap_segs = 0; w.cap_src = 0;
    ensure_trans_raw(std::max<uint64_t>(keep_trans, 1), std::max<uint64_t>(keep_src, 1));
    ensure_path_raw(std::max<uint64_t>(keep_path, cp / 8 + 1024));
    ensure_segs_raw(std::max<uint64_t>(keep_segs, cp / 2 + 1024));
  }
}

static void free_one(Workspace& w, void* q) {
  if (!q) return;
  (void)hipFree(q);
  w.allocs.erase(std::find(w.allocs.begin(), w.allocs.end(), q));
}

void Matcher::ensure_trans(uint64_t n, uint64_t n_src) { grow_workspace([&] { ensure_trans_raw(n, n_src); }); }
void Matcher::ensure_path(uint64_t n) { grow_workspace([&] { ensure_path_raw(n); }); }
void Matcher::ensure_segs(uint64_t n) { grow_workspace([&] { ensure_segs_raw(n); }); }

void Matcher::ensure_turns() {
  grow_workspace([&] {
    Workspace& w = ws_;
    const uint64_t want_walk = (w.cap_src / kK2Items + 2) * (kWalkPerBlock + 1);
    if (w.route_d && w.cap_turn >= w.cap_trans && w.cap_walk >= want_walk) return;
    free_one(w, w.route_d);
    free_one(w, w.walk);
    w.route_d = nullptr;
    w.walk = nullptr;
    w.cap_turn = 0;
    w.cap_walk = 0;
    w.route_d = dalloc<double>(w.allocs, w.cap_trans);
    w.cap_turn = w.cap_trans;
    w.cap_walk = want_walk;
    w.walk = dalloc<uint32_t>(w.allocs, w.cap_walk);
  });
}

void Matcher::ensure_trans_raw(uint64_t n, uint64_t n_src) {
  {
    Workspace& w = ws_;
    if (!(n <= w.cap_trans && w.route)) {
      free_one(w, w.route);
      free_one(w, w.route_d);
      free_one(w, w.walk);
      w.route = nullptr;
      w.route_d = nullptr;
      w.walk = nullptr;
      w.cap_trans = 0;
      w.cap_turn = 0;
      w.cap_walk = 0;
      const uint64_t c = n + n / 4 + 1024;
      w.route = dalloc<uint32_t>(w.allocs, c);
      w.cap_trans = c;
    }
    if (!(n_src <= w.cap_src && w.src_item)) {
      for (uint32_t** q : {&w.src_item, &w.rl_routes_a, &w.rl_routes_b, &w.rl_routes_0, &w.rl_routes_c}) {
        free_one(w, *q);
        *q = nullptr;
      }
      w.cap_src = 0;
      const uint64_t c = n_src + n_src / 4 + 1024;
      w.src_item = dalloc<uint32_t>(w.allocs, c);
      w.rl_routes_a = dalloc<uint32_t>(w.allocs, c);
      w.rl_routes_b = dalloc<uint32_t>(w.allocs, c);
      w.rl_routes_0 = dalloc<uint32_t>(w.allocs, c);
      w.rl_routes_c = dalloc<uint32_t>(w.allocs, c);
      w.cap_src = c;
    }
  }
}

void Matcher::ensure_path_raw(uint64_t n) {
  {
    Workspace& w = ws_;
    if (n <= w.cap_path && w.path_pool) return;
    free_one(w, w.path_pool);
    w.path_pool = nullptr;
    w.cap_path = 0;
    const uint64_t c = n + n / 4 + 1024;
    w.path_pool = dalloc<uint32_t>(w.allocs, c);
    w.cap_path = c;
  }
}

void Matcher::ensure_segs_raw(uint64_t n) {
  {
    Workspace& w = ws_;
    if (n <= w.cap_segs && w.segs) return;
    for (void** q : {(void**)&w.segs, (void**)&w.reps, (void**)&w.rec_slot}) {
      free_one(w, *q);
      *q = nullptr;
    }
    w.cap_segs = 0;
    const uint64_t c = n + n / 4 + 1024;
    w.segs = dalloc<SegmentRec>(w.allocs, c);
    w.reps = dalloc<ReportRec>(w.allocs, c);
    w.rec_slot = dalloc<uint32_t>(w.allocs, c);
    w.cap_segs = c;
  }
}

void Matcher::tic(int k) {
  if (!((timing_mask_ >> k) & 1u)) return;
  Ev ev;
  if (!free_ev_.empty()) { ev = free_ev_.back(); free_ev_.pop_back(); }
  else { RM_HIP(hipEventCreate(&ev.a)); RM_HIP(hipEventCreate(&ev.b)); }
  ev.k = k;
  RM_HIP(hipEventRecord(ev.a, stream_));
  pending_.push_back(ev);
}
void Matcher::toc(int k) {
  if (!((timing_mask_ >> k) & 1u) || pending_.empty()) return;
  RM_HIP(hipEventRecord(pending_.back().b, stream_));
}
void Matcher::harvest_times() {
  for (auto& ev : pending_) {
    float ms = 0.f;
    RM_HIP(hipEventElapsedTime(&ms, ev.a, ev.b));
    kms_[ev.k] += ms;
    klaunch_[ev.k] += 1;
    free_ev_.push_back(ev);
  }
  pending_.clear();
}
void Matcher::kernel_times(double* ms, uint64_t* launches) {
  for (int i = 0; i < kNumKernels; ++i) { ms[i] = kms_[i]; if (launches) launches[i] = klaunch_[i]; }
}
void Matcher::reset_kernel_times() {
  for (int i = 0; i < kNumKernels; ++i) { kms_[i] = 0; klaunch_[i] = 0; }
}

void Matcher::sync() {
  RM_HIP(hipStreamSynchronize(stream_));
  harvest_times();
}

#ifndef RM_SEARCH_DELTA_M
#define RM_SEARCH_DELTA_M 0
#endif
uint32_t search_delta_cm() {
  static const uint32_t d = [] {
    const char* e = std::getenv("RM_SEARCH_DELTA_M");
    const double m = e && *e ? std::strtod(e, nullptr) : (double)RM_SEARCH_DELTA_M;
    return m > 0.0 ? (uint32_t)std::min(m * 100.0, 4.0e9) : kNone;
  }();
  return d;
}

static DevBatch make_view(const Workspace& w, const InputView& in, uint32_t T, uint64_t P) {
  DevBatch v;
  v.T = T; v.P = P;
  v.trace_off = in.trace_off; v.lon = in.lon; v.lat = in.lat; v.time = in.time; v.acc = in.acc;
// ... 324 lines not shown
  hipStream_t st = stream_;
  unsigned long long* htot = reinterpret_cast<unsigned long long*>(hctl_ + 16);
  uint64_t Pc = 4096;
  while (Pc < P) Pc <<= 1;
  ensure_trans(Pc * kMaxCand * kMaxCand, Pc * kMaxCand);
  if (turn_mask_) ensure_turns();
  ensure_segs(Pc * kInlinePath + w.cap_path);
  DevBatch v = make_view(w, in_, T, P);
  v.route = w.route;
  if (turn_mask_) { v.route_d = w.route_d; v.walk = w.walk; }
  v.src_item = w.src_item;
  v.rl_routes_a = w.rl_routes_a; v.rl_routes_b = w.rl_routes_b; v.rl_routes_0 = w.rl_routes_0;
  v.rl_routes_c = w.rl_routes_c;
  v.segs = w.segs; v.reps = w.reps; v.seg_cap = w.cap_segs;
  v.gate = w.gsearch ? 1u : 3u;
  locality_used_ = false;
  const uint32_t count_grid = (uint32_t)((P + 255) / 256);
  const uint32_t sum_grid = (uint32_t)((P + 1023) / 1024);
  const uint64_t max_src = P * kMaxCand;
  const uint32_t item_grid = (uint32_t)((max_src + kK2Items - 1) / kK2Items);
  const uint32_t lane_grid = (uint32_t)((max_src + 255) / 256);
  const auto tgrid = [P](uint32_t full) { return tier_grid(P, full); };

  tic(kKStates);
  hipLaunchKernelGGL(k_states, dim3(T), dim3(64), 0, st, v);
  toc(kKStates);
  tic(kKCandidates);
  DevGraph gk = g;
  eng_->k1_grid(batch_radius_, gk);
  if (P <= kSmallWaveK1) {
    hipLaunchKernelGGL(k_candidates_wave, dim3((uint32_t)P), dim3(64), 0, st, gk, v, 1);
  } else {
    hipLaunchKernelGGL(k_candidates_lane, dim3(count_grid), dim3(256), 0, st, gk, v);
    hipLaunchKernelGGL(k_candidates_wave, dim3(tgrid(2048)), dim3(64), 0, st, gk, v, 0);
  }
  toc(kKCandidates);
  tic(kKScan);
  hipLaunchKernelGGL(k_trans_count, dim3(count_grid), dim3(256), 0, st, v, w.tot_part);
  hipLaunchKernelGGL(k_trans_apply_small, dim3(count_grid), dim3(256), 0, st, v, (const unsigned long long*)w.tot_part,
                     count_grid, w.tot64);
  toc(kKScan);
  const bool balls = (mode_mask_ & g.ball_mask) != 0u;
  const char* sc_env = std::getenv("RM_SMALL_SHORT_CHAIN");
  const bool short_chain = balls && !(sc_env && *sc_env == '0');
  tic(kKRoutes);
  if (balls) {
    if (v.route_d) {
      hipLaunchKernelGGL(k_routes_ball2<true>, dim3(item_grid), dim3(kK2Threads), 0, st, g, v, kNone);
      hipLaunchKernelGGL(k_turn_walks, dim3(item_grid), dim3(kWalkThreads), 0, st, g, v, kNone);
      hipLaunchKernelGGL(k_turn_walks_marked, dim3(kWalkScanGrid), dim3(256), 0, st, g, v);
    } else {
      hipLaunchKernelGGL(k_routes_ball2<false>, dim3(item_grid), dim3(kK2Threads), 0, st, g, v, kNone);
    }
    if (!short_chain) {
      const uint32_t lg = (uint32_t)std::min<uint64_t>(lane_grid, kListedGrid);
      if (v.route_d) hipLaunchKernelGGL(k_routes_lane<true>, dim3(lg), dim3(256), 0, st, g, v, 0u, 1);
      else hipLaunchKernelGGL(k_routes_lane<false>, dim3(lg), dim3(256), 0, st, g, v, 0u, 1);
    }
  } else {
    if (v.route_d) hipLaunchKernelGGL(k_routes_lane<true>, dim3(lane_grid), dim3(256), 0, st, g, v, kNone, 0);
    else hipLaunchKernelGGL(k_routes_lane<false>, dim3(lane_grid), dim3(256), 0, st, g, v, kNone, 0);
  }
  if (!short_chain) hipLaunchKernelGGL(k_routes_reg2, dim3(tgrid(kReg2Grid)), dim3(256), 0, st, g, v);
  hipLaunchKernelGGL(k_routes_grp, dim3(tgrid(kGrpGrid)), dim3(64), 0, st, g, v, short_chain ? 1 : 0);
  if (!short_chain) hipLaunchKernelGGL(k_routes_wave_s, dim3(tgrid(kMidGrid)), dim3(64), 0, st, g, v);
  hipLaunchKernelGGL(k_routes_wave, dim3(tgrid(1024)), dim3(64), 0, st, g, v, short_chain ? 1 : 0);
  if (w.gsearch) hipLaunchKernelGGL(k_routes_global, dim3(kGlobalGrid), dim3(64), 0, st, g, v, (GlobalPathSmem*)w.gsearch);
  toc(kKRoutes);
  tic(kKViterbi);
  launch_viterbi(T, st, v);
  toc(kKViterbi);
  tic(kKPaths);
  if (balls) {
    hipLaunchKernelGGL(k_paths_ball, dim3(count_grid), dim3(256), 0, st, g, v);
    if (!short_chain)
      hipLaunchKernelGGL(k_paths_lane, dim3((uint32_t)std::min<uint64_t>(count_grid, kListedGrid)), dim3(256), 0, st, g, v, 1);
  } else {
    hipLaunchKernelGGL(k_paths_lane, dim3(count_grid), dim3(256), 0, st, g, v, 0);
  }
  if (!short_chain) hipLaunchKernelGGL(k_paths_reg2, dim3(tgrid(kReg2Grid)), dim3(256), 0, st, g, v);
  hipLaunchKernelGGL(k_paths_grp, dim3(tgrid(kGrpGrid)), dim3(64), 0, st, g, v, short_chain ? 1 : 0);
  if (!short_chain) hipLaunchKernelGGL(k_paths_wave_s, dim3(tgrid(kMidGrid)), dim3(64), 0, st, g, v);
  hipLaunchKernelGGL(k_paths_wave, dim3(tgrid(1024)), dim3(64), 0, st, g, v, short_chain ? 1 : 0);
  if (w.gsearch) hipLaunchKernelGGL(k_paths_global, dim3(kGlobalGrid), dim3(64), 0, st, g, v, (GlobalPathSmem*)w.gsearch);
  toc(kKPaths);
  tic(kKSegments);
  hipLaunchKernelGGL(k_sum_u64, dim3(sum_grid), dim3(256), 0, st, w.path_cnt, P, w.tot_part);
  hipLaunchKernelGGL(k_path_apply_small, dim3(sum_grid), dim3(256), 0, st, v, (const unsigned long long*)w.tot_part,
                     sum_grid, w.tot64, w.rec_slot);
  if (rp.do_report && rp.zero_hist) zero_hist(rp);
  hipLaunchKernelGGL(k_seg_wave, dim3(T), dim3(64), 0, st, g, v, (const uint32_t*)w.rec_slot, kNone, report_args(rp));
  toc(kKSegments);
  constexpr uint32_t kSegWords = sizeof(SegmentRec) / 8;
  const size_t offb = ((T + 1) * 4ull + 7) & ~(size_t)7;
  bool prefetch = rp.prefetch_segments != 0;
  if (prefetch) {
    try {
      grow_dl_dev(offb + v.seg_cap * sizeof(SegmentRec));
    } catch (const BatchTooLarge&) {
      prefetch = false;
    }
  }
  if (prefetch) {
    if (T + 1 > hoff_cap_) {
      if (hoff_) RM_HIP(hipHostFree(hoff_));
      hoff_ = nullptr; hoff_cap_ = 0;
      const uint64_t c = std::max<uint64_t>(T + 1 + T / 2, 4096);
      RM_HIP(hipHostMalloc((void**)&hoff_, c * 4, hipHostMallocDefault));
      hoff_cap_ = c;
    }
    uint32_t* d_off = (uint32_t*)dl_dev_;
    hipLaunchKernelGGL(k_seg_offsets_small, dim3(1), dim3(1024), 0, st, v, d_off);
    hipLaunchKernelGGL(k_gather_recs, dim3(std::min<uint32_t>(T, 8192u)), dim3(64), 0, st, T, (const uint32_t*)w.seg_base,
                       (const uint32_t*)w.seg_cnt, (const uint32_t*)d_off, (const unsigned long long*)w.segs, kSegWords,
                       (unsigned long long*)((char*)dl_dev_ + offb));
    RM_HIP(hipMemcpyAsync(hoff_, d_off, (T + 1) * 4ull, hipMemcpyDeviceToHost, st));
  }
  RM_HIP(hipGetLastError());
  RM_HIP(hipMemcpyAsync(hctl_, w.ctl, kCtlWords * sizeof(uint32_t), hipMemcpyDeviceToHost, st));
  RM_HIP(hipMemcpyAsync(htot, w.tot64, 3 * sizeof(unsigned long long), hipMemcpyDeviceToHost, st));
  sync();
  if ((hctl_[2] & kErrPathOverflow) || (!w.gsearch && (hctl_[9] | hctl_[10])) || htot[2] > v.seg_cap) return false;
  n_trans_ = htot[0];
  n_path_ = htot[2];
  seg_used_ = htot[2];
  has_report_ = rp.do_report != 0;
  seg_prefetched_ = prefetch;
  err_bits_ = hctl_[2] & (kErrCandOverflow | kErrSearchOverflow | kErrRounds);
  if (err_bits_ && !isolate_) throw std::runtime_error(error_text(err_bits_));
  return true;
}

bool Matcher::run_steady(const RunParams& rp, const DevGraph& g) {
  const uint32_t T = n_traces_;
  const uint64_t P = n_points_;
  Workspace& w = ws_;
  hipStream_t st = stream_;
  unsigned long long* htot = reinterpret_cast<unsigned long long*>(hctl_ + 16);
  if (turn_mask_) ensure_turns();
  DevBatch v = make_view(w, in_, T, P);
  v.route = w.route;
  if (turn_mask_) { v.route_d = w.route_d; v.walk = w.walk; }
  v.src_item = w.src_item;
  v.rl_routes_a = w.rl_routes_a; v.rl_routes_b = w.rl_routes_b; v.rl_routes_0 = w.rl_routes_0;
  v.rl_routes_c = w.rl_routes_c;
  v.segs = w.segs; v.reps = w.reps; v.seg_cap = w.cap_segs;
  const uint64_t src_cover = std::min<uint64_t>(w.cap_src, steady_src_ + steady_src_ / 8 + 4096);
  v.trans_cap = w.cap_trans;
  v.src_cap = src_cover;
  v.gate = (w.gsearch ? 1u : 3u) | 4u;
  locality_used_ = false;
  const uint32_t count_grid = (uint32_t)((P + 255) / 256);
  const uint32_t sum_grid = (uint32_t)((P + 1023) / 1024);
  static const bool prev_grids = [] { const char* e = std::getenv("RM_STEADY_GRIDS"); return !(e && *e == '0'); }();
  const auto sgrid = [&](uint32_t full, int word, uint32_t per_block) {
    if (!prev_grids) return (uint32_t)(full == 2048u ? 2048u : tier_grid(P, full));
    const uint64_t want = 4ull * (((uint64_t)steady_ctl_[word] + per_block - 1) / per_block);
    return (uint32_t)std::min<uint64_t>(tier_grid(P, full), std::max<uint64_t>(64u, want));
  };

  tic(kKStates);
  hipLaunchKernelGGL(k_states, dim3(T), dim3(64), 0, st, v);
  toc(kKStates);
  tic(kKCandidates);
  DevGraph gk = g;
  eng_->k1_grid(batch_radius_, gk);
  hipLaunchKernelGGL(k_candidates_lane, dim3(count_grid), dim3(256), 0, st, gk, v);
  hipLaunchKernelGGL(k_candidates_wave, dim3(sgrid(2048, 7, 1)), dim3(64), 0, st, gk, v, 0);
  toc(kKCandidates);
  tic(kKScan);
  hipLaunchKernelGGL(k_trans_count, dim3(count_grid), dim3(256), 0, st, v, w.tot_part);
  hipLaunchKernelGGL(k_scan_parts, dim3(1), dim3(1024), 0, st, w.tot_part, count_grid, w.tot64);
  hipLaunchKernelGGL(k_scan_apply2, dim3(count_grid), dim3(256), 0, st, (const uint32_t*)w.trans_cnt,
                     (const uint32_t*)w.src_cnt, P, (const unsigned long long*)w.tot_part, w.trans_off, w.src_off);
  toc(kKScan);
  const bool balls = (mode_mask_ & g.ball_mask) != 0u;
  const uint32_t item_grid = (uint32_t)((src_cover + kK2Items - 1) / kK2Items);
  const uint32_t lane_grid = (uint32_t)((src_cover + 255) / 256);
  tic(kKRoutes);
  hipLaunchKernelGGL(k_src_items, dim3(count_grid), dim3(256), 0, st, v);
  if (balls) {
    if (v.route_d) {
      hipLaunchKernelGGL(k_routes_ball2<true>, dim3(item_grid), dim3(kK2Threads), 0, st, g, v, kNone);
      hipLaunchKernelGGL(k_turn_walks, dim3(item_grid), dim3(kWalkThreads), 0, st, g, v, kNone);
      hipLaunchKernelGGL(k_turn_walks_marked, dim3(kWalkScanGrid), dim3(256), 0, st, g, v);
    } else {
      hipLaunchKernelGGL(k_routes_ball2<false>, dim3(item_grid), dim3(kK2Threads), 0, st, g, v, kNone);
    }
    const uint32_t lg = std::min<uint32_t>(lane_grid, sgrid(kListedGrid, 1, 256));
    if (v.route_d) hipLaunchKernelGGL(k_routes_lane<true>, dim3(lg), dim3(256), 0, st, g, v, 0u, 1);
    else hipLaunchKernelGGL(k_routes_lane<false>, dim3(lg), dim3(256), 0, st, g, v, 0u, 1);
  } else {
    if (v.route_d) hipLaunchKernelGGL(k_routes_lane<true>, dim3(lane_grid), dim3(256), 0, st, g, v, kNone, 0);
    else hipLaunchKernelGGL(k_routes_lane<false>, dim3(lane_grid), dim3(256), 0, st, g, v, kNone, 0);
  }
  hipLaunchKernelGGL(k_routes_reg2, dim3(sgrid(kReg2Grid, 3, 256)), dim3(256), 0, st, g, v);
  hipLaunchKernelGGL(k_routes_grp, dim3(sgrid(kGrpGrid, 5, kWave / kGrpW)), dim3(64), 0, st, g, v, 0);
  hipLaunchKernelGGL(k_routes_wave_s, dim3(sgrid(kMidGrid, 11, 1)), dim3(64), 0, st, g, v);
  hipLaunchKernelGGL(k_routes_wave, dim3(sgrid(1024, 13, 1)), dim3(64), 0, st, g, v, 0);
  if (w.gsearch) hipLaunchKernelGGL(k_routes_global, dim3(kGlobalGrid), dim3(64), 0, st, g, v, (GlobalPathSmem*)w.gsearch);
  toc(kKRoutes);
  tic(kKViterbi);
  launch_viterbi(T, st, v);
  toc(kKViterbi);
  tic(kKPaths);
  if (balls) {
    hipLaunchKernelGGL(k_paths_ball, dim3(count_grid), dim3(256), 0, st, g, v);
    hipLaunchKernelGGL(k_paths_lane, dim3(std::min<uint32_t>(count_grid, sgrid(kListedGrid, 8, 256))), dim3(256), 0, st, g, v, 1);
  } else {
    hipLaunchKernelGGL(k_paths_lane, dim3(count_grid), dim3(256), 0, st, g, v, 0);
  }
  hipLaunchKernelGGL(k_paths_reg2, dim3(sgrid(kReg2Grid, 4, 256)), dim3(256), 0, st, g, v);
  hipLaunchKernelGGL(k_paths_grp, dim3(sgrid(kGrpGrid, 6, kWave / kGrpW)), dim3(64), 0, st, g, v, 0);
  hipLaunchKernelGGL(k_paths_wave_s, dim3(sgrid(kMidGrid, 12, 1)), dim3(64), 0, st, g, v);
  hipLaunchKernelGGL(k_paths_wave, dim3(sgrid(1024, 14, 1)), dim3(64), 0, st, g, v, 0);
  if (w.gsearch) hipLaunchKernelGGL(k_paths_global, dim3(kGlobalGrid), dim3(64), 0, st, g, v, (GlobalPathSmem*)w.gsearch);
  toc(kKPaths);
  tic(kKSegments);
  hipLaunchKernelGGL(k_sum_u64, dim3(sum_grid), dim3(256), 0, st, w.path_cnt, P, w.tot_part);
  hipLaunchKernelGGL(k_scan_parts, dim3(1), dim3(1024), 0, st, w.tot_part, sum_grid, w.tot64 + 2);
  hipLaunchKernelGGL(k_scan_apply4, dim3(sum_grid), dim3(256), 0, st, (const uint32_t*)w.path_cnt, P,
                     (const unsigned long long*)w.tot_part, w.trav_off);
  if (rp.do_report && rp.zero_hist) zero_hist(rp);
  hipLaunchKernelGGL(k_rec_slot, dim3(count_grid), dim3(256), 0, st, v, w.rec_slot);
  hipLaunchKernelGGL(k_seg_wave, dim3(T), dim3(64), 0, st, g, v, (const uint32_t*)w.rec_slot, kNone, report_args(rp));
  toc(kKSegments);
  RM_HIP(hipGetLastError());
  RM_HIP(hipMemcpyAsync(hctl_, w.ctl, kCtlWords * sizeof(uint32_t), hipMemcpyDeviceToHost, st));
  RM_HIP(hipMemcpyAsync(htot, w.tot64, 3 * sizeof(unsigned long long), hipMemcpyDeviceToHost, st));
  sync();
  if (htot[0] > w.cap_trans || htot[1] > src_cover || (hctl_[2] & kErrPathOverflow) ||
      (!w.gsearch && (hctl_[9] | hctl_[10])) || htot[2] > v.seg_cap)
    return false;
  n_trans_ = htot[0];
  n_path_ = htot[2];
  seg_used_ = htot[2];
  steady_src_ = htot[1];
  std::memcpy(steady_ctl_, hctl_, sizeof(steady_ctl_));
  has_report_ = rp.do_report != 0;
  err_bits_ = hctl_[2] & (kErrCandOverflow | kErrSearchOverflow | kErrRounds);
  if (err_bits_ && !isolate_) throw std::runtime_error(error_text(err_bits_));
  return true;
}

void Matcher::run_device(const RunParams& rp) {
  RM_HIP(hipSetDevice(eng_->device()));
  const uint32_t T = n_traces_;
  const uint64_t P = n_points_;
  err_bits_ = 0;
  if (T == 0) return;
  if (P >= (uint64_t)kTravLast) throw BatchTooLarge("batch too large (slots >= 2^30); split it");
  Workspace& w = ws_;
  hipStream_t st = stream_;
  eng_->ensure_balls(mode_mask_);
  if (turn_mask_) eng_->ensure_turn_rows(turn_mask_);
  const DevGraph g = eng_->dev_snapshot();
  if (!hctl_) RM_HIP(hipHostMalloc((void**)&hctl_, 32 * sizeof(uint32_t), hipHostMallocDefault));
  unsigned long long* htot = reinterpret_cast<unsigned long long*>(hctl_ + 16);
  seg_prefetched_ = false;
  if (P <= small_batch_points() && locality_ <= 0 && run_small(rp, g)) return;
  const char* steady_env = std::getenv("RM_STEADY");
  const bool steady_on = !(steady_env && *steady_env == '0');
  if (steady_on && steady_src_ && w.route && w.src_item && w.path_pool && w.segs && T > 0) {
    int lm = locality_;
    if (lm < 0) lm = eng_->locality_default() ? 2 : (batch_sparse_ ? 1 : 0);
    if (eng_->locality_bits() == 0) lm = 0;
    if (lm == 0 && run_steady(rp, g)) return;
    steady_src_ = 0;
  }
  DevBatch v = make_view(w, in_, T, P);
  const uint32_t count_grid = (uint32_t)((P + 255) / 256);
  const uint32_t sum_grid = (uint32_t)((P + 1023) / 1024);

  tic(kKStates);
  hipLaunchKernelGGL(k_states, dim3(T), dim3(64), 0, st, v);
  toc(kKStates);
  int lmode = locality_;
  if (lmode < 0) lmode = eng_->locality_default() ? 2 : (batch_sparse_ ? 1 : 0);
  if (eng_->locality_bits() == 0) lmode = 0;
  locality_used_ = lmode > 0;
  if (locality_used_) {
    tic(kKLocality);
    ensure_sort(P);
    const uint32_t lgrid = (uint32_t)((P + 256u * kLocPerThread - 1) / (256u * kLocPerThread));
    RM_HIP(hipMemsetAsync(w.loc_cursor, 0, (kLocBuckets + 1) * sizeof(uint32_t), st));
    hipLaunchKernelGGL(k_loc_count, dim3(lgrid), dim3(256), 0, st, g, v, eng_->locality_shift(), w.loc_key,
                       w.loc_cursor);
    hipLaunchKernelGGL(k_loc_scan, dim3(1), dim3(1024), 0, st, w.loc_cursor);
    hipLaunchKernelGGL(k_loc_scatter, dim3(lgrid), dim3(256), 0, st, P, (const uint16_t*)w.loc_key, w.loc_cursor, w.perm);
    v.perm = w.perm;
    if (lmode >= 2) v.perm_paths = w.perm;
    toc(kKLocality);
  }
  tic(kKCandidates);
  DevGraph gk = g;
  eng_->k1_grid(batch_radius_, gk);
  static const bool k1_wave_all = [] { const char* e = std::getenv("RM_K1_WAVE_ALL"); return e && *e == '1'; }();
  if (k1_wave_all) {
    hipLaunchKernelGGL(k_candidates_wave, dim3((uint32_t)std::min<uint64_t>(P, 1u << 20)), dim3(64), 0, st, gk, v, 1);
  } else {
    hipLaunchKernelGGL(k_candidates_lane, dim3((uint32_t)((P + 255) / 256)), dim3(256), 0, st, gk, v);
    hipLaunchKernelGGL(k_candidates_wave, dim3(2048), dim3(64), 0, st, gk, v, 0);
  }
  toc(kKCandidates);
  tic(kKScan);
  hipLaunchKernelGGL(k_trans_count, dim3(count_grid), dim3(256), 0, st, v, w.tot_part);
  hipLaunchKernelGGL(k_scan_parts, dim3(1), dim3(1024), 0, st, w.tot_part, count_grid, w.tot64);
  hipLaunchKernelGGL(k_scan_apply2, dim3(count_grid), dim3(256), 0, st, (const uint32_t*)w.trans_cnt,
                     (const uint32_t*)w.src_cnt, P, (const unsigned long long*)w.tot_part, w.trans_off, w.src_off);
  if (v.perm) {
    hipLaunchKernelGGL(k_perm_src_count, dim3(count_grid), dim3(256), 0, st, v, w.pcnt, w.tot_part);
    hipLaunchKernelGGL(k_scan_parts, dim3(1), dim3(1024), 0, st, w.tot_part, count_grid, w.tot64 + 2);
    hipLaunchKernelGGL(k_scan_apply_perm, dim3(count_grid), dim3(256), 0, st, (const uint32_t*)w.pcnt, P,
                       (const unsigned long long*)w.tot_part, (const uint32_t*)w.perm, w.src_off);
  }
  toc(kKScan);
  RM_HIP(hipMemcpyAsync(htot, w.tot64, 2 * sizeof(unsigned long long), hipMemcpyDeviceToHost, st));
  RM_HIP(hipStreamSynchronize(st));
  const uint64_t total = htot[0];
  const uint64_t n_src = htot[1];
  if (total >= kMaxTransitions) throw BatchTooLarge("batch too large (transitions >= 0xF0000000); split it");
  uint64_t steady_next = n_src ? n_src : 1;
  n_trans_ = total;
  ensure_trans(total, n_src);
  v.route = w.route;
  if (turn_mask_) {
    ensure_turns();
    v.route_d = w.route_d;
    v.walk = w.walk;
  }
  v.src_item = w.src_item;
  v.rl_routes_a = w.rl_routes_a;
  v.rl_routes_b = w.rl_routes_b;
  v.rl_routes_0 = w.rl_routes_0;
  v.rl_routes_c = w.rl_routes_c;

  const bool balls = (mode_mask_ & g.ball_mask) != 0u;
  tic(kKRoutes);
  hipLaunchKernelGGL(k_src_items, dim3((uint32_t)((P + 255) / 256)), dim3(256), 0, st, v);
  if (n_src && balls) {
    if (v.route_d) {
      hipLaunchKernelGGL(k_routes_ball2<true>, dim3((uint32_t)((n_src + kK2Items - 1) / kK2Items)), dim3(kK2Threads), 0, st,
                         g, v, (uint32_t)n_src);
      hipLaunchKernelGGL(k_turn_walks, dim3((uint32_t)((n_src + kK2Items - 1) / kK2Items)), dim3(kWalkThreads), 0, st, g, v,
                         (uint32_t)n_src);
      hipLaunchKernelGGL(k_turn_walks_marked, dim3(kWalkScanGrid), dim3(256), 0, st, g, v);
    } else
      hipLaunchKernelGGL(k_routes_ball2<false>, dim3((uint32_t)((n_src + kK2Items - 1) / kK2Items)), dim3(kK2Threads), 0, st,
                         g, v, (uint32_t)n_src);
    if (v.route_d)
      hipLaunchKernelGGL(k_routes_lane<true>, dim3((uint32_t)std::min<uint64_t>((n_src + 255) / 256, kListedGrid)), dim3(256),
                         0, st, g, v, 0u, 1);
    else
      hipLaunchKernelGGL(k_routes_lane<false>, dim3((uint32_t)std::min<uint64_t>((n_src + 255) / 256, kListedGrid)),
                         dim3(256), 0, st, g, v, 0u, 1);
  } else if (n_src) {
    if (v.route_d)
      hipLaunchKernelGGL(k_routes_lane<true>, dim3((uint32_t)((n_src + 255) / 256)), dim3(256), 0, st, g, v, (uint32_t)n_src, 0);
    else
      hipLaunchKernelGGL(k_routes_lane<false>, dim3((uint32_t)((n_src + 255) / 256)), dim3(256), 0, st, g, v, (uint32_t)n_src, 0);
  }
  const auto tgrid = [P](uint32_t full) { return tier_grid(P, full); };
  hipLaunchKernelGGL(k_routes_reg2, dim3(tgrid(kReg2Grid)), dim3(256), 0, st, g, v);
  hipLaunchKernelGGL(k_routes_grp, dim3(tgrid(kGrpGrid)), dim3(64), 0, st, g, v, 0);
  hipLaunchKernelGGL(k_routes_wave_s, dim3(tgrid(kMidGrid)), dim3(64), 0, st, g, v);
  hipLaunchKernelGGL(k_routes_wave, dim3(tgrid(1024)), dim3(64), 0, st, g, v, 0);
  bool routes_global_done = w.gsearch != nullptr;
  if (routes_global_done)
    hipLaunchKernelGGL(k_routes_global, dim3(kGlobalGrid), dim3(64), 0, st, g, v, (GlobalPathSmem*)w.gsearch);
  toc(kKRoutes);
  tic(kKViterbi);
  launch_viterbi(T, st, v);
  toc(kKViterbi);
  for (int attempt = 0;; ++attempt) {
    tic(kKPaths);
    if (attempt) {
      RM_HIP(hipMemsetAsync(w.ctl + 8, 0, sizeof(uint32_t), st));
      RM_HIP(hipMemsetAsync(w.ctl + 10, 0, sizeof(uint32_t), st));
      RM_HIP(hipMemsetAsync(w.ctl + 12, 0, sizeof(uint32_t), st));
      RM_HIP(hipMemsetAsync(w.ctl + 14, 0, sizeof(uint32_t), st));
    }
    if (balls) {
      hipLaunchKernelGGL(k_paths_ball, dim3((uint32_t)((P + 255) / 256)), dim3(256), 0, st, g, v);
      hipLaunchKernelGGL(k_paths_lane, dim3((uint32_t)std::min<uint64_t>((P + 255) / 256, kListedGrid)), dim3(256), 0,
                         st, g, v, 1);
    } else {
      hipLaunchKernelGGL(k_paths_lane, dim3((uint32_t)((P + 255) / 256)), dim3(256), 0, st, g, v, 0);
    }
    hipLaunchKernelGGL(k_paths_reg2, dim3(tgrid(kReg2Grid)), dim3(256), 0, st, g, v);
    hipLaunchKernelGGL(k_paths_grp, dim3(tgrid(kGrpGrid)), dim3(64), 0, st, g, v, 0);
    hipLaunchKernelGGL(k_paths_wave_s, dim3(tgrid(kMidGrid)), dim3(64), 0, st, g, v);
    hipLaunchKernelGGL(k_paths_wave, dim3(tgrid(1024)), dim3(64), 0, st, g, v, 0);
    if (w.gsearch) hipLaunchKernelGGL(k_paths_global, dim3(kGlobalGrid), dim3(64), 0, st, g, v, (GlobalPathSmem*)w.gsearch);
    toc(kKPaths);
    tic(kKSegments);
    hipLaunchKernelGGL(k_sum_u64, dim3(sum_grid), dim3(256), 0, st, w.path_cnt, P, w.tot_part);
    hipLaunchKernelGGL(k_scan_parts, dim3(1), dim3(1024), 0, st, w.tot_part, sum_grid, w.tot64 + 2);
    hipLaunchKernelGGL(k_scan_apply4, dim3(sum_grid), dim3(256), 0, st, (const uint32_t*)w.path_cnt, P,
                       (const unsigned long long*)w.tot_part, w.trav_off);
    toc(kKSegments);
    RM_HIP(hipMemcpyAsync(htot + 2, w.tot64 + 2, sizeof(unsigned long long), hipMemcpyDeviceToHost, st));
    read_ctl();
    if (!routes_global_done && hctl_[9]) {
      ensure_global_search();
      routes_global_done = true;
      hipLaunchKernelGGL(k_routes_global, dim3(kGlobalGrid), dim3(64), 0, st, g, v, (GlobalPathSmem*)w.gsearch);
      launch_viterbi(T, st, v);
      RM_HIP(hipMemsetAsync(w.path_cnt, 0, P * sizeof(uint32_t), st));
      for (int c : {0, 4, 6}) RM_HIP(hipMemsetAsync(w.ctl + c, 0, sizeof(uint32_t), st));
      uint32_t flags = hctl_[2] & ~kErrPathOverflow;
      RM_HIP(hipMemcpyAsync(w.ctl + 2, &flags, sizeof(uint32_t), hipMemcpyHostToDevice, st));
      RM_HIP(hipStreamSynchronize(st));
      continue;
    }
    if (!w.gsearch && hctl_[10]) {
      ensure_global_search();
      hipLaunchKernelGGL(k_paths_global, dim3(kGlobalGrid), dim3(64), 0, st, g, v, (GlobalPathSmem*)w.gsearch);
      hipLaunchKernelGGL(k_sum_u64, dim3(sum_grid), dim3(256), 0, st, w.path_cnt, P, w.tot_part);
      hipLaunchKernelGGL(k_scan_parts, dim3(1), dim3(1024), 0, st, w.tot_part, sum_grid, w.tot64 + 2);
      hipLaunchKernelGGL(k_scan_apply4, dim3(sum_grid), dim3(256), 0, st, (const uint32_t*)w.path_cnt, P,
                         (const unsigned long long*)w.tot_part, w.trav_off);
      RM_HIP(hipMemcpyAsync(htot + 2, w.tot64 + 2, sizeof(unsigned long long), hipMemcpyDeviceToHost, st));
      read_ctl();
    }
    if (!(hctl_[2] & kErrPathOverflow)) break;
    if (attempt > 3) throw BatchTooLarge("path pool overflow persists");
    ensure_path((uint64_t)hctl_[0]);
    v.path_pool = w.path_pool; v.path_cap = w.cap_path;
    RM_HIP(hipMemsetAsync(w.ctl, 0, sizeof(uint32_t), st));
    RM_HIP(hipMemsetAsync(w.ctl + 4, 0, sizeof(uint32_t), st));
    RM_HIP(hipMemsetAsync(w.ctl + 6, 0, sizeof(uint32_t), st));
    uint32_t flags = hctl_[2] & ~kErrPathOverflow;
    RM_HIP(hipMemcpyAsync(w.ctl + 2, &flags, sizeof(uint32_t), hipMemcpyHostToDevice, st));
    RM_HIP(hipStreamSynchronize(st));
  }
  const uint64_t seg_total = htot[2];
  if (seg_total >= kMaxRecords) throw BatchTooLarge("batch too large (path edges >= 1.7e9); split it");
  n_path_ = seg_total;
  ensure_segs(seg_total);
  v.segs = w.segs; v.reps = w.reps; v.seg_cap = w.cap_segs;
  tic(kKSegments);
  if (rp.do_report && rp.zero_hist) zero_hist(rp);
  if (T) {
    hipLaunchKernelGGL(k_rec_slot, dim3((uint32_t)((P + 255) / 256)), dim3(256), 0, st, v, w.rec_slot);
    hipLaunchKernelGGL(k_seg_wave, dim3(T), dim3(64), 0, st, g, v, (const uint32_t*)w.rec_slot, (uint32_t)seg_total,
                       report_args(rp));
  }
  toc(kKSegments);
  RM_HIP(hipGetLastError());
  RM_HIP(hipMemcpyAsync(hctl_, w.ctl, kCtlWords * sizeof(uint32_t), hipMemcpyDeviceToHost, st));
  sync();
  seg_used_ = seg_total;
  has_report_ = rp.do_report != 0;
  if (!locality_used_) {
    steady_src_ = steady_next;
    std::memcpy(steady_ctl_, hctl_, sizeof(steady_ctl_));
  }
  err_bits_ = hctl_[2] & (kErrCandOverflow | kErrSearchOverflow | kErrRounds);
  if (err_bits_ && !isolate_) throw std::runtime_error(error_text(err_bits_));
}

void Matcher::get_trace_errors(uint32_t* out) {
  sync();
  if (n_traces_) RM_HIP(hipMemcpy(out, ws_.trace_err, n_traces_ * 4ull, hipMemcpyDeviceToHost));
}

void report_segments(int device, uint32_t T, const uint32_t* seg_off, const SegmentRec* segs, const double* end_time,
                     const double* threshold, const uint32_t* rmask, const uint32_t* tmask, uint32_t* rep_off,
                     ReportRec* reps, ReportStats* stats) {
  RM_HIP(hipSetDevice(device));
  if (T == 0) { rep_off[0] = 0; return; }
  for (uint32_t k = 0; k < T; ++k)
    if (seg_off[k + 1] < seg_off[k]) throw std::runtime_error("segment offsets not monotone");
  const uint64_t S = seg_off[T];
  std::vector<void*> L;
  struct Free { std::vector<void*>& l; ~Free() { for (void* p : l) (void)hipFree(p); } } fr{L};
  uint32_t* d_off = dalloc<uint32_t>(L, T + 1);
  SegmentRec* d_segs = dalloc<SegmentRec>(L, S);
  double* d_end = dalloc<double>(L, T);
  double* d_thr = dalloc<double>(L, T);
  uint32_t* d_rm = dalloc<uint32_t>(L, T);
  uint32_t* d_tm = dalloc<uint32_t>(L, T);
  ReportRec* d_reps = dalloc<ReportRec>(L, S);
  ReportStats* d_st = dalloc<ReportStats>(L, T);
  RM_HIP(hipMemcpy(d_off, seg_off, (T + 1) * 4ull, hipMemcpyHostToDevice));
  if (S) RM_HIP(hipMemcpy(d_segs, segs, S * sizeof(SegmentRec), hipMemcpyHostToDevice));
  RM_HIP(hipMemcpy(d_end, end_time, T * 8ull, hipMemcpyHostToDevice));
  RM_HIP(hipMemcpy(d_thr, threshold, T * 8ull, hipMemcpyHostToDevice));
  RM_HIP(hipMemcpy(d_rm, rmask, T * 4ull, hipMemcpyHostToDevice));
  RM_HIP(hipMemcpy(d_tm, tmask, T * 4ull, hipMemcpyHostToDevice));
  hipLaunchKernelGGL(k_report_lists, dim3(T), dim3(64), 0, 0, T, d_off, d_segs, d_end, d_thr, d_rm, d_tm,
                     d_reps, d_st);
  RM_HIP(hipGetLastError());
  std::vector<ReportRec> all(S);
  if (S) RM_HIP(hipMemcpy(all.data(), d_reps, S * sizeof(ReportRec), hipMemcpyDeviceToHost));
  RM_HIP(hipMemcpy(stats, d_st, T * sizeof(ReportStats), hipMemcpyDeviceToHost));
  uint64_t at = 0;
  for (uint32_t k = 0; k < T; ++k) {
    rep_off[k] = (uint32_t)at;
    const uint32_t c = (uint32_t)stats[k].n_reports;
    if (c) std::memcpy(reps + at, all.data() + seg_off[k], c * sizeof(ReportRec));
    at += c;
  }
  rep_off[T] = (uint32_t)at;
}

void Matcher::get_states(uint32_t* n_states, uint32_t* state_orig) {
  sync();
  RM_HIP(hipMemcpy(n_states, ws_.n_states, n_traces_ * 4ull, hipMemcpyDeviceToHost));
  RM_HIP(hipMemcpy(state_orig, ws_.state_orig, n_points_ * 4, hipMemcpyDeviceToHost));
}
void Matcher::get_candidates(uint8_t* cand_n, uint32_t* road, uint32_t* s_cm, float* sq) {
  sync();
  RM_HIP(hipMemcpy(cand_n, ws_.cand_n, n_points_, hipMemcpyDeviceToHost));
  {
    std::vector<uint4> desc(n_points_ * kMaxCand * 2);
    RM_HIP(hipMemcpy(desc.data(), ws_.cand_desc, desc.size() * sizeof(uint4), hipMemcpyDeviceToHost));
    for (uint64_t x = 0; x < n_points_ * kMaxCand; ++x) { road[x] = desc[2 * x].x; s_cm[x] = desc[2 * x].y; }
  }
  RM_HIP(hipMemcpy(sq, ws_.cand_sq, n_points_ * kMaxCand * 4, hipMemcpyDeviceToHost));
}
void Matcher::get_routes(uint32_t* trans_off, double* gc, uint32_t* route) {
  sync();
  RM_HIP(hipMemcpy(trans_off, ws_.trans_off, n_points_ * 4, hipMemcpyDeviceToHost));
  RM_HIP(hipMemcpy(gc, ws_.gc, n_points_ * 8, hipMemcpyDeviceToHost));
  if (n_trans_) RM_HIP(hipMemcpy(route, ws_.route, n_trans_ * 4, hipMemcpyDeviceToHost));
}
int Matcher::get_route_terms(double* out) {
  sync();
  if (!turn_mask_ || !ws_.route_d) return 0;
  if (n_trans_) RM_HIP(hipMemcpy(out, ws_.route_d, n_trans_ * 8, hipMemcpyDeviceToHost));
  return 1;
}
void Matcher::get_viterbi(int8_t* choice, uint8_t* chain_start) {
  sync();
  RM_HIP(hipMemcpy(choice, ws_.choice, n_points_, hipMemcpyDeviceToHost));
  RM_HIP(hipMemcpy(chain_start, ws_.chain_start, n_points_, hipMemcpyDeviceToHost));
}
void Matcher::get_paths(uint32_t* path_off, uint32_t* path_cnt, uint32_t* pool, uint32_t* route_dist) {
  sync();
  const uint64_t P = n_points_;
  std::vector<uint32_t> off(P), inl(P * kInlinePath), used(1, 0);
  RM_HIP(hipMemcpy(off.data(), ws_.path_off, P * 4, hipMemcpyDeviceToHost));
  RM_HIP(hipMemcpy(path_cnt, ws_.path_cnt, P * 4, hipMemcpyDeviceToHost));
  RM_HIP(hipMemcpy(inl.data(), ws_.path_inline, P * kInlinePath * 4, hipMemcpyDeviceToHost));
  RM_HIP(hipMemcpy(route_dist, ws_.route_dist, P * 4, hipMemcpyDeviceToHost));
  RM_HIP(hipMemcpy(used.data(), ws_.ctl, 4, hipMemcpyDeviceToHost));
  std::vector<uint32_t> dpool(used[0]);
  if (used[0]) RM_HIP(hipMemcpy(dpool.data(), ws_.path_pool, used[0] * 4ull, hipMemcpyDeviceToHost));
  std::vector<uint32_t> choice_ok(P, 0);
  {
    std::vector<int8_t> ch(P);
    std::vector<uint8_t> cs(P);
    RM_HIP(hipMemcpy(ch.data(), ws_.choice, P, hipMemcpyDeviceToHost));
    RM_HIP(hipMemcpy(cs.data(), ws_.chain_start, P, hipMemcpyDeviceToHost));
    std::vector<uint32_t> tro(n_traces_ + 1), ns(n_traces_);
    RM_HIP(hipMemcpy(tro.data(), in_.trace_off, (n_traces_ + 1) * 4ull, hipMemcpyDeviceToHost));
    RM_HIP(hipMemcpy(ns.data(), ws_.n_states, n_traces_ * 4ull, hipMemcpyDeviceToHost));
    for (uint32_t k = 0; k < n_traces_; ++k)
      for (uint32_t s = 1; s < ns[k]; ++s) {
        const uint64_t l = tro[k] + s;
        choice_ok[l] = (!cs[l] && ch[l] >= 0) ? 1u : 0u;
      }
  }
  uint64_t at = 0;
  for (uint64_t p = 0; p < P; ++p) {
    if (!choice_ok[p]) { path_off[p] = (uint32_t)at; path_cnt[p] = 0; continue; }
    const uint32_t n = path_cnt[p];
    path_off[p] = (uint32_t)at;
    const uint32_t* src = n <= (uint32_t)kInlinePath ? inl.data() + p * kInlinePath : dpool.data() + off[p];
    std::memcpy(pool + at, src, n * 4ull);
    at += n;
  }
}

void Matcher::ctl_words(uint32_t* out) {
  sync();
  for (int i = 0; i < kCtlWords; ++i) out[i] = 0;
  if (ws_.ctl && n_traces_) RM_HIP(hipMemcpy(out, ws_.ctl, kCtlWords * sizeof(uint32_t), hipMemcpyDeviceToHost));
}

void Matcher::tier_counts(uint32_t* out4) {
  uint32_t c[kCtlWords];
  ctl_words(c);
  out4[0] = c[3]; out4[1] = c[5]; out4[2] = c[4]; out4[3] = c[7];
}

uint64_t Matcher::count_segments() {
  sync();
  std::vector<uint32_t> cnt(n_traces_);
  if (n_traces_) RM_HIP(hipMemcpy(cnt.data(), ws_.seg_cnt, n_traces_ * 4ull, hipMemcpyDeviceToHost));
  uint64_t t = 0;
  for (uint32_t c : cnt) t += c;
  return t;
}
void Matcher::grow_dl_host(size_t need) {
  if (need <= dl_host_bytes_) return;
  const size_t want = std::max(need, dl_host_bytes_ + dl_host_bytes_ / 2);
  if (dl_host_) RM_HIP(hipHostFree(dl_host_));
  dl_host_ = nullptr;
  dl_host_bytes_ = 0;
  void* p = nullptr;
  size_t got = want;
  hipError_t e = hipHostMalloc(&p, want, hipHostMallocDefault);
  if (e != hipSuccess && want > need) {
    (void)hipGetLastError();
    got = need;
    e = hipHostMalloc(&p, need, hipHostMallocDefault);
  }
  if (e != hipSuccess) {
    (void)hipGetLastError();
    throw BatchTooLarge("pinned download buffer of " + std::to_string(need) + " bytes: " + hipGetErrorString(e));
  }
  dl_host_ = p;
  dl_host_bytes_ = got;
}

void Matcher::grow_dl_dev(size_t dev_need) {
  if (dev_need <= dl_dev_bytes_) return;
  const size_t want = std::max(dev_need, dl_dev_bytes_ + dl_dev_bytes_ / 2);
  if (dl_dev_) RM_HIP(hipFree(dl_dev_));
  dl_dev_ = nullptr;
  dl_dev_bytes_ = 0;
  const char* lim = std::getenv("RM_TEST_DOWNLOAD_ALLOC_LIMIT");
  const size_t limit = lim && *lim ? (size_t)std::strtoull(lim, nullptr, 10) : ~(size_t)0;
  void* p = nullptr;
  size_t got = 0;
  for (const size_t sz : {want, dev_need}) {
    if (sz > limit) continue;
    std::vector<void*> buf;
    try {
      dalloc<char>(buf, sz);
    } catch (const OutOfDeviceMemory&) {
      continue;
    }
    p = buf[0];
    got = sz;
    break;
  }
  if (!p) throw BatchTooLarge("segment download buffer of " + std::to_string(dev_need) + " bytes does not fit in HBM");
  dl_dev_ = p;
  dl_dev_bytes_ = got;
}

void Matcher::download_compacted(const uint32_t* d_base, const uint32_t* d_cnt, const void* d_src, uint32_t words,
                                 uint32_t* off, void* dst, const std::function<void*(uint64_t)>& dst_for) {
  const uint32_t T = n_traces_;
  hipStream_t st = stream_;
  RM_HIP(hipSetDevice(eng_->device()));
  seg_prefetched_ = false;
  const size_t offb = ((size_t)T + 1) * 4;
  grow_dl_host(offb);
  uint32_t* hc = (uint32_t*)dl_host_;
  RM_HIP(hipMemcpyAsync(hc, d_cnt, T * 4ull, hipMemcpyDeviceToHost, st));
  RM_HIP(hipStreamSynchronize(st));
  uint64_t at = 0;
  for (uint32_t k = 0; k < T; ++k) {
    off[k] = (uint32_t)at;
    at += hc[k];
  }
  off[T] = (uint32_t)at;
  if (dst_for) dst = dst_for(at);
  if (at == 0) return;
  const size_t recb = (size_t)at * words * 8;
  const size_t dev_need = offb + recb + 8;
  grow_dl_dev(dev_need);
  grow_dl_host(offb + recb + 8);
  hc = (uint32_t*)dl_host_;
  std::memcpy(hc, off, offb);
  uint32_t* d_off = (uint32_t*)dl_dev_;
  unsigned long long* d_dst = (unsigned long long*)((char*)dl_dev_ + ((offb + 7) & ~(size_t)7));
  RM_HIP(hipMemcpyAsync(d_off, hc, offb, hipMemcpyHostToDevice, st));
  hipLaunchKernelGGL(k_gather_recs, dim3(std::min<uint32_t>(T, 8192u)), dim3(64), 0, st, T, d_base, d_cnt, d_off,
                     (const unsigned long long*)d_src, words, d_dst);
  char* h_dst = (char*)dl_host_ + ((offb + 7) & ~(size_t)7);
  RM_HIP(hipMemcpyAsync(h_dst, d_dst, recb, hipMemcpyDeviceToHost, st));
  RM_HIP(hipStreamSynchronize(st));
  std::memcpy(dst, h_dst, recb);
}

bool Matcher::download_prefetched(uint32_t* off, void* dst, const std::function<void*(uint64_t)>& dst_for) {
  if (!seg_prefetched_) return false;
  seg_prefetched_ = false;
  const uint32_t T = n_traces_;
  std::memcpy(off, hoff_, ((size_t)T + 1) * 4);
  const uint64_t at = off[T];
  if (dst_for) dst = dst_for(at);
  if (at == 0) return true;
  const size_t offb = (((size_t)T + 1) * 4 + 7) & ~(size_t)7;
  const size_t recb = (size_t)at * sizeof(SegmentRec);
  grow_dl_host(recb);
  RM_HIP(hipMemcpyAsync(dl_host_, (const char*)dl_dev_ + offb, recb, hipMemcpyDeviceToHost, stream_));
  RM_HIP(hipStreamSynchronize(stream_));
  std::memcpy(dst, dl_host_, recb);
  return true;
}

void Matcher::get_segments(uint32_t* seg_off, SegmentRec* segs) {
  sync();
  if (!n_traces_) { seg_off[0] = 0; return; }
  static_assert(sizeof(SegmentRec) % 8 == 0, "records move as u64 words");
  if (download_prefetched(seg_off, segs, nullptr)) return;
  download_compacted(ws_.seg_base, ws_.seg_cnt, ws_.segs, sizeof(SegmentRec) / 8, seg_off, segs, nullptr);
}
void Matcher::get_segments(std::vector<uint32_t>& seg_off, std::vector<SegmentRec>& segs) {
  sync();
  seg_off.assign((size_t)n_traces_ + 1, 0u);
  segs.clear();
  if (!n_traces_) return;
  if (download_prefetched(seg_off.data(), nullptr, [&](uint64_t n) -> void* {
        segs.resize(n);
        return segs.data();
      }))
    return;
  download_compacted(ws_.seg_base, ws_.seg_cnt, ws_.segs, sizeof(SegmentRec) / 8, seg_off.data(), nullptr,
                     [&](uint64_t n) -> void* {
                       segs.resize(n);
                       return segs.data();
                     });
}
uint64_t Matcher::count_reports() {
  sync();
  if (!has_report_) return 0;
  std::vector<uint32_t> cnt(n_traces_);
  if (n_traces_) RM_HIP(hipMemcpy(cnt.data(), ws_.rep_cnt, n_traces_ * 4ull, hipMemcpyDeviceToHost));
  uint64_t t = 0;
  for (uint32_t c : cnt) t += c;
  return t;
// ... 12 lines not shown
```

reporter_amd/csrc/engine.hpp:

```cpp
#pragma once
#include <hip/hip_runtime.h>

#include <functional>
#include <memory>
#include <mutex>
#include <stdexcept>
#include <string>
#include <vector>

#include "balls.hpp"
#include "graph.hpp"
#include "rm_common.hpp"
#include "serve_policy.hpp"

namespace rm {

#define RM_HIP(x)                                                                                \
  do {                                                                                           \
    hipError_t _e = (x);                                                                         \
    if (_e != hipSuccess)                                                                        \
      throw std::runtime_error(std::string("HIP error ") + hipGetErrorString(_e) + " at " #x);   \
  } while (0)

struct OutOfDeviceMemory : std::runtime_error {
  using std::runtime_error::runtime_error;
};

struct DevGraph {
  const uint32_t* node_off;
  const uint4* edges;
  const uint32_t* edge_src;
  const uint32_t* in_off;
  const uint32_t* in_edge;
  const uint4* in_rec;
  const uint32_t* in_info;
  const uint32_t* edge_seg;
  const uint32_t* edge_seg_off;
  const uint32_t* edge_way;
  const uint32_t* road_node0;
  const uint32_t* road_node1;
  const uint32_t* road_fwd;
  const uint32_t* road_rev;
  const uint32_t* road_len;
  const uint4* verts;
  const unsigned long long* seg_id;
  const uint32_t* seg_len;
  const uint32_t* cell_off;
  const uint32_t* cell_item;
  const uint4* cell_rec;
  const uint4* road_rec;
  const uint4* relax[5];
  const uint32_t* node_rng;
  const uint4* seg_rec;
  const uint2* ball_hdr[5];
  const uint4* ball_ent[5];
  uint32_t ball_radius[5];
  uint32_t ball_mask;
  uint32_t ball_road_mask;
  const uint32_t* road_head;
  const uint32_t* turn_w;
  const uint2* ball_turn[5];
  uint32_t ball_turn_mask;
  double lon0, lat0, dlon, dlat;
  uint32_t ncx, ncy, n_nodes, n_edges, n_segments, pad;
};

struct HostBatch {
  uint32_t n_traces = 0;
  const uint32_t* trace_off = nullptr;
  const float* lon = nullptr;
  const float* lat = nullptr;
  const double* time = nullptr;
  const float* accuracy = nullptr;
  uint32_t n_opts = 0;
  const MatchOptions* opts = nullptr;
  const uint32_t* trace_opt = nullptr;
};

struct RunParams {
  double threshold_sec = 15.0;
  uint32_t report_mask = 0b0110;
  uint32_t transition_mask = 0b0110;
  uint32_t* hist = nullptr;
  int do_report = 1;
  int zero_hist = 0;
  unsigned long long* dur = nullptr;
  int prefetch_segments = 0;
};

struct InputView {
  const uint32_t* trace_off = nullptr;
  const float* lon = nullptr;
  const float* lat = nullptr;
  const double* time = nullptr;
  const float* acc = nullptr;
  const MatchOptions* opts = nullptr;
  const uint32_t* trace_opt = nullptr;
};

enum KernelId { kKStates = 0, kKCandidates, kKScan, kKRoutes, kKViterbi, kKPaths, kKSegments, kKReport, kKLocality,
                kKPoints, kNumKernels };
extern const char* const kKernelNames[kNumKernels];

constexpr int kCtlWords = 16;
constexpr int kInlinePath = 8;

struct Workspace {
  uint64_t cap_points = 0, cap_traces = 0, cap_trans = 0, cap_path = 0, cap_opts = 0, cap_segs = 0, cap_src = 0;
  uint32_t* trace_off = nullptr; float* lon = nullptr; float* lat = nullptr; double* time = nullptr;
  float* acc = nullptr; MatchOptions* opts = nullptr; uint32_t* trace_opt = nullptr;
  uint32_t* slot_trace = nullptr; uint32_t* n_states = nullptr; uint32_t* state_orig = nullptr;
  double* state_time = nullptr;
  uint8_t* cand_n = nullptr; uint4* cand_desc = nullptr; float* cand_sq = nullptr;
  uint32_t* trans_cnt = nullptr; uint32_t* trans_off = nullptr; double* gc = nullptr; uint32_t* route = nullptr;
  double* route_d = nullptr;
  uint64_t cap_turn = 0;
  uint32_t* walk = nullptr;
  uint64_t cap_walk = 0;
  uint4* pair_info = nullptr;
  uint32_t* src_cnt = nullptr; uint32_t* src_off = nullptr; uint32_t* src_item = nullptr;
  int8_t* choice = nullptr; uint8_t* chain_start = nullptr; uint8_t* bp = nullptr;
  uint32_t* path_off = nullptr; uint32_t* path_cnt = nullptr; uint32_t* path_pool = nullptr; uint32_t* route_dist = nullptr;
  uint2* path_sab = nullptr;
  uint32_t* path_inline = nullptr;
  SegmentRec* segs = nullptr; uint32_t* seg_base = nullptr; uint32_t* seg_cnt = nullptr;
  uint32_t* trav_off = nullptr;
  uint32_t* rec_slot = nullptr;
  ReportRec* reps = nullptr; uint32_t* rep_cnt = nullptr; ReportStats* stats = nullptr;
  uint32_t* ctl = nullptr;
  uint32_t* rl_routes_a = nullptr; uint32_t* rl_routes_b = nullptr; uint32_t* rl_routes_0 = nullptr;
  uint32_t* rl_paths_a = nullptr; uint32_t* rl_paths_b = nullptr; uint32_t* rl_cand = nullptr;
  uint32_t* rl_routes_c = nullptr; uint32_t* rl_paths_c = nullptr; void* gsearch = nullptr;
  uint32_t* trace_err = nullptr;
  unsigned long long* tot64 = nullptr;
  unsigned long long* tot_part = nullptr;
  uint64_t cap_sort = 0;
  uint32_t* perm = nullptr; uint16_t* loc_key = nullptr; uint32_t* loc_cursor = nullptr; uint32_t* pcnt = nullptr;
  std::vector<void*> allocs;
  ~Workspace();
  void release();
};

struct PointsDesc {
  uint64_t n_points = 0;
  const uint32_t* uuid = nullptr;
  const double* time = nullptr;
  const float* lon = nullptr;
  const float* lat = nullptr;
  const float* accuracy = nullptr;
  double inactivity = 120.0;
  uint32_t n_uuids = 0;
  uint32_t n_opts = 0;
  const MatchOptions* opts = nullptr;
  const uint32_t* uuid_opt = nullptr;
};

struct TileParams {
  uint32_t quantisation = 3600;
  uint32_t privacy = 2;
  std::string source = "smpl_rprt";
  std::string mode = "AUTO";
};

struct TileRow {
  uint64_t id, next_id;
  int64_t start, end;
  int32_t duration, length, queue;
  uint32_t bucket;
  uint32_t tile;
  uint32_t pad[3];
};
static_assert(sizeof(TileRow) == 64, "TileRow is four dwordx4");

struct StageBufs {
  std::vector<void*> allocs;
  uint64_t cap_pts = 0, cap_rows = 0;
  uint32_t cap_tr = 0;
  uint32_t* derr = nullptr;
  uint32_t* p_uuid = nullptr; double* p_time = nullptr; float* p_lon = nullptr; float* p_lat = nullptr;
  float* p_acc = nullptr; uint32_t* p_uopt = nullptr; MatchOptions* p_opts = nullptr;
  unsigned long long* k0 = nullptr; unsigned long long* k1 = nullptr; uint32_t* v0 = nullptr; uint32_t* v1 = nullptr;
  uint32_t* flag = nullptr; uint32_t* idx = nullptr; uint32_t* wstart = nullptr; uint32_t* wcnt = nullptr;
  uint32_t* wofs = nullptr; uint32_t* wflag = nullptr; uint32_t* widx = nullptr;
  uint32_t* trace_uuid = nullptr;
  TileRow* rows = nullptr; TileRow* rows2 = nullptr;
  unsigned long long* rk = nullptr; unsigned long long* rk2 = nullptr;
  uint32_t* rperm = nullptr; uint32_t* rperm2 = nullptr; uint32_t* rflag = nullptr; uint32_t* ridx = nullptr;
  uint32_t* gpos = nullptr; uint8_t* gkeep = nullptr; uint32_t* tcnt = nullptr; uint32_t* tofs = nullptr;
  void* tmp = nullptr; size_t tmp_bytes = 0;
  uint32_t* hctl = nullptr;
  uint32_t cap_uuids = 0;
  ~StageBufs();
};

constexpr uint32_t kErrCandOverflow = 1u, kErrSearchOverflow = 2u, kErrPathOverflow = 4u, kErrRounds = 8u;
const char* error_text(uint32_t bits);

class Engine;

void report_segments(int device, uint32_t T, const uint32_t* seg_off, const SegmentRec* segs, const double* end_time,
                     const double* threshold, const uint32_t* rmask, const uint32_t* tmask, uint32_t* rep_off,
                     ReportRec* reps, ReportStats* stats);

struct TileComm {
  int rank = 0, nranks = 1;
  virtual ~TileComm() = default;
  virtual uint64_t max_u64(uint64_t v, hipStream_t st) = 0;
  virtual void allgather(const void* send, void* recv, size_t bytes, hipStream_t st) = 0;
};

class Matcher {
 public:
  explicit Matcher(Engine* e);
  ~Matcher();
  Matcher(const Matcher&) = delete;
  Matcher& operator=(const Matcher&) = delete;

  void run(const HostBatch& b, const RunParams& rp);
  void run_device(const RunParams& rp);
  void json_reserve_bytes(uint64_t bytes);
  void json_reserve(uint64_t points, uint32_t traces, uint32_t nopts);
  void json_upload(uint64_t off, const void* src, uint64_t n);
  void json_parse(const uint64_t* span, const uint32_t* trace_off, uint32_t T, uint32_t* flags, double* tspan);
  void upload_points(uint64_t first, uint64_t n, const float* lon, const float* lat, const double* time, const float* acc);
  void run_parsed(const uint32_t* trace_off, uint32_t T, const MatchOptions* opts, uint32_t n_opts,
                  const uint32_t* trace_opt, const double* tspan, const RunParams& rp);
  void sync();
  uint32_t n_traces() const { return n_traces_; }
  uint64_t n_points() const { return n_points_; }
  uint64_t n_trans() const { return n_trans_; }
  uint64_t n_path_edges() const { return n_path_; }
  uint64_t seg_pool_used() const { return seg_used_; }
  void get_states(uint32_t* n_states, uint32_t* state_orig);
  void get_candidates(uint8_t* cand_n, uint32_t* road, uint32_t* s_cm, float* sq);
  void get_routes(uint32_t* trans_off, double* gc, uint32_t* route);
  int get_route_terms(double* route_d);
  void get_viterbi(int8_t* choice, uint8_t* chain_start);
  void get_paths(uint32_t* path_off, uint32_t* path_cnt, uint32_t* pool, uint32_t* route_dist);
  void get_segments(uint32_t* seg_off, SegmentRec* segs);
  void get_segments(std::vector<uint32_t>& seg_off, std::vector<SegmentRec>& segs);
  uint64_t count_segments();
  void get_reports(uint32_t* rep_off, ReportRec* reps, ReportStats* stats);
  uint64_t count_reports();
  void matched_points(MatchedPoint* out);
  void kernel_times(double* ms, uint64_t* launches);
  void tier_counts(uint32_t* out4);
  void ctl_words(uint32_t* out);
  void reset_kernel_times();
  void set_timing(bool on) { timing_mask_ = on ? ~0u : 0u; }
  void set_timing_mask(uint32_t mask) { timing_mask_ = mask; }
  void set_isolation(bool on) { isolate_ = on; }
  void set_locality(int mode) { locality_ = mode; }
  bool locality_used() const { return locality_used_; }
  uint32_t error_bits() const { return err_bits_; }
  void get_trace_errors(uint32_t* out);
  hipStream_t stream() const { return stream_; }
  const Engine& engine() const { return *eng_; }

  void run_points(const PointsDesc& pd, const RunParams& rp);
  void get_trace_uuid(uint32_t* out);
  void get_batch(uint32_t* trace_off, float* lon, float* lat, double* time, float* acc);
  std::string tiles(const TileParams& tp, struct TileComm* comm = nullptr);

 private:
  void ensure(uint64_t points, uint32_t traces, uint32_t nopts);
  void check_batch(uint32_t T, const uint32_t* trace_off, const MatchOptions* opts, uint32_t n_opts,
                   const uint32_t* trace_opt);
  void scan_options(const MatchOptions* opts, uint32_t n_opts);
  char* jdev_ = nullptr;
  uint64_t jcap_ = 0;
  void* jspan_ = nullptr;
  uint32_t* jflag_ = nullptr;
  void* jtsp_ = nullptr;
  uint32_t jtcap_ = 0;
  void ensure_trans(uint64_t n, uint64_t n_src);
  void ensure_path(uint64_t n);
  void ensure_segs(uint64_t n);
  void ensure_turns();
  void alloc_points(uint64_t cp, uint64_t ct, uint64_t co, uint64_t keep_trans, uint64_t keep_path, uint64_t keep_segs,
                    uint64_t keep_src);
  void ensure_trans_raw(uint64_t n, uint64_t n_src);
  void ensure_path_raw(uint64_t n);
  void ensure_segs_raw(uint64_t n);
  void ensure_global_search();
  void read_ctl();
  void tic(int k);
  void toc(int k);
  void harvest_times();
  void download_compacted(const uint32_t* d_base, const uint32_t* d_cnt, const void* d_src, uint32_t words,
                          uint32_t* off, void* dst, const std::function<void*(uint64_t)>& dst_for);
  void grow_dl_host(size_t need);
  bool download_prefetched(uint32_t* off, void* dst, const std::function<void*(uint64_t)>& dst_for);
  void grow_dl_dev(size_t need);
  bool run_small(const RunParams& rp, const DevGraph& g);
  bool run_steady(const RunParams& rp, const DevGraph& g);
  uint64_t steady_src_ = 0;
  uint32_t steady_ctl_[16] = {0};
  void zero_hist(const RunParams& rp);
  void use_ws_inputs();
  void ensure_pack(uint64_t bytes);

  Engine* eng_;
  InputView in_;
  char* hpack_ = nullptr;
  char* dpack_ = nullptr;
  uint64_t pack_cap_ = 0;
  uint32_t* hoff_ = nullptr;
  uint64_t hoff_cap_ = 0;
  bool seg_prefetched_ = false;
  void* dl_dev_ = nullptr;
  void* dl_host_ = nullptr;
  size_t dl_dev_bytes_ = 0, dl_host_bytes_ = 0;
  void* mp_dev_ = nullptr;
  uint64_t mp_cap_ = 0;
  hipStream_t stream_ = nullptr;
  Workspace ws_;
  uint32_t n_traces_ = 0;
  uint64_t n_points_ = 0, n_trans_ = 0, n_path_ = 0, seg_used_ = 0;
  uint32_t timing_mask_ = 0;
  bool has_report_ = false;
  bool isolate_ = false;
  int locality_ = -1;
  bool batch_sparse_ = false;
  bool locality_used_ = false;
  void ensure_sort(uint64_t n);
  uint32_t err_bits_ = 0;
  uint32_t* hctl_ = nullptr;
  StageBufs sb_;
  bool from_points_ = false;
  uint32_t mode_mask_ = 0;
  uint32_t turn_mask_ = 0;
  float batch_radius_ = 0.f;
  void ensure_points(uint64_t n, uint32_t n_uuids, uint32_t n_opts);
  void ensure_rows(uint64_t n, uint32_t traces);
  struct Ev { hipEvent_t a, b; int k; };
  std::vector<Ev> pending_, free_ev_;
  double kms_[kNumKernels] = {0};
  uint64_t klaunch_[kNumKernels] = {0};
};

uint32_t choose_grid_split(const Graph& g);
uint32_t choose_grid_split_for(const Graph& g, float radius_m);

struct K1Grid {
  const uint32_t* cell_off = nullptr;
  const uint4* cell_rec = nullptr;
  double lon0 = 0, lat0 = 0, dlon = 0, dlat = 0;
  uint32_t ncx = 0, ncy = 0, split = 1;
};

class Engine {
 public:
  Engine(const Graph& g, int device);
  ~Engine();
  Engine(const Engine&) = delete;
  Engine& operator=(const Engine&) = delete;
  const DevGraph& dev() const { return dg_; }
  DevGraph dev_snapshot() const;
  int device() const { return device_; }
  const Graph& host() const { return host_; }
  uint32_t n_segments() const { return host_.num_segments(); }
  void ensure_balls(uint32_t mode_mask);
  void ensure_turn_rows(uint32_t mode_mask);
  uint32_t turn_row_mask() const { return dg_.ball_turn_mask; }
  double turn_build_ms(int mode) const { return mode >= 0 && mode <= kModePedestrian ? turn_ms_[mode] : 0.0; }
  void set_ball_radius(uint32_t radius_cm);
  uint32_t ball_radius() const { return ball_radius_cm_; }
  void ball_stats(int mode, double* out4) const;
  uint32_t mode_ball_radius(int mode) const;
  uint32_t ball_gpu_mask() const { return ball_gpu_; }
  void ball_lookup(int mode, uint64_t n, const uint32_t* from, const uint32_t* road, uint64_t* keys, uint8_t* preds);
  uint32_t grid_split() const { return grid_split_; }
  void k1_grid(float radius_m, DevGraph& g) const;
  uint32_t grid_alt_split() const { return n_grids_ > 1 ? grids_[1].split : 0u; }
  float grid_alt_radius() const { return grid_alt_radius_; }
  bool locality_default() const { return locality_default_; }
  uint32_t locality_shift() const { return locality_shift_; }
  uint32_t locality_bits() const { return locality_bits_; }
  const uint32_t* road_vert_off_dev();

 private:
  int device_;
  Graph host_;
  DevGraph dg_{};
  std::vector<void*> allocs_;
  mutable std::mutex ball_mu_;
  uint32_t ball_radius_cm_ = 40000;
  uint32_t ball_built_ = 0;
  uint32_t ball_gpu_ = 0;
  uint32_t grid_split_ = 1;
  K1Grid grids_[2];
  int n_grids_ = 1;
  float grid_alt_radius_ = 0.f;
  bool locality_default_ = false;
  uint32_t locality_shift_ = 0, locality_bits_ = 0;
  uint64_t ball_bytes_ = 0;
  uint32_t turn_tried_ = 0;
  double turn_ms_[5] = {};
  bool build_balls_gpu(int mode, uint32_t radius_cm, uint32_t max_keys, uint64_t avail_bytes);
  double ball_info_[5][4] = {};
  uint32_t* road_vert_off_ = nullptr;
};

}
```

reporter_amd/csrc/rm_common.hpp:

```cpp
#pragma once
#include <math.h>
#include <stdint.h>

#if defined(__HIP__) || defined(__HIPCC__)
#include <hip/hip_runtime.h>
#define RM_HD __host__ __device__ __forceinline__
#else
#define RM_HD static inline
#endif

namespace rm {

constexpr int kLevelBits = 3;
constexpr int kTileIndexBits = 22;
constexpr int kSegmentIndexBits = 21;
constexpr uint64_t kInvalidSegmentId = 0x3fffffffffffull;
constexpr uint32_t kNone = 0xffffffffu;

constexpr double kMetersPerDegLat = 110567.0;
constexpr double kMetersPerDegLonEq = 111320.0;
constexpr double kDegToRad = 0.017453292519943295;
constexpr double kPi = 3.141592653589793;
constexpr double kRadEarthMeters = 6378160.187;

// ... 188 lines not shown
  else if (mode == kModeMotorScooter) cap = 450;
  return edge_dkph < cap ? edge_dkph : cap;
}
RM_HD uint32_t time_ms(uint32_t d_cm, uint32_t dkph) {
  return (uint32_t)(((uint64_t)d_cm * 360ull) / (uint64_t)(dkph ? dkph : 1u));
}

RM_HD uint64_t make_key(uint32_t d_cm, uint32_t t_ms) { return ((uint64_t)d_cm << 32) | t_ms; }
RM_HD uint32_t key_dist(uint64_t k) { return (uint32_t)(k >> 32); }
RM_HD uint32_t key_time(uint64_t k) { return (uint32_t)k; }
constexpr uint64_t kKeyInf = ~0ull;

#ifdef RM_BALL_SLOT_RANDOM
RM_HD uint32_t ball_slot(uint32_t v, uint32_t bits) { return (v * 2654435761u) >> (32u - bits); }
#else
#ifndef RM_BALL_GROUP_LOG
#define RM_BALL_GROUP_LOG 3
#endif
#ifndef RM_BALL_GROUP_BITS
#define RM_BALL_GROUP_BITS 10
#endif
constexpr uint32_t kBallGroupBits = RM_BALL_GROUP_BITS, kBallGroupLog = RM_BALL_GROUP_LOG;
#ifndef RM_BALL_SLOTS_PER_ROW
#define RM_BALL_SLOTS_PER_ROW 2
#endif
constexpr uint32_t kBallSlotsPerRow = RM_BALL_SLOTS_PER_ROW;
RM_HD uint32_t ball_slot(uint32_t v, uint32_t bits) {
  if (bits < kBallGroupBits) return (v * 2654435761u) >> (32u - bits);
  return ((((v >> kBallGroupLog) * 2654435761u) >> (32u + kBallGroupLog - bits)) << kBallGroupLog) |
         (v & ((1u << kBallGroupLog) - 1u));
}
constexpr uint32_t kBallRoadBits = 26;
constexpr uint32_t kBallPredNone = 7u;
RM_HD uint32_t ball_road_mask(uint32_t n_roads) {
  return n_roads < (1u << kBallRoadBits) - 1u ? (1u << kBallRoadBits) - 1u : ~0u;
}
RM_HD uint32_t ball_road_word(uint32_t road, uint32_t p0, uint32_t p1, uint32_t mask) {
  return mask == ~0u ? road : road | p0 << kBallRoadBits | p1 << (kBallRoadBits + 3u);
}
RM_HD uint32_t ball_pred(uint32_t word, uint32_t side, uint32_t mask) {
  return mask == ~0u ? kBallPredNone : (word >> (kBallRoadBits + 3u * side)) & 7u;
}

RM_HD int tile_file_owner(uint64_t bucket, uint32_t tile, int nranks) {
  const unsigned long long h = (((unsigned long long)bucket << 25) | tile) * 0x9e3779b97f4a7c15ull;
  return (int)((h >> 33) % (unsigned long long)(nranks > 0 ? nranks : 1));
}

#endif

constexpr uint64_t kBallMaxRows = 1ull << 33;
RM_HD uint64_t ball_row0(uint32_t hx) { return (uint64_t)hx << 1; }

constexpr uint32_t kBallNoDist = 0xffffffu;
constexpr uint32_t kBallMaxField = 0xfffffeu;
RM_HD uint64_t ball_key0(uint32_t x, uint32_t y, uint32_t w) {
  const uint32_t d = y & 0xffffffu;
  return (x == 0xffffffffu || d == kBallNoDist) ? ~0ull : make_key(d, (y >> 24) | ((w & 0xffffu) << 8));
}
RM_HD uint64_t ball_key1(uint32_t x, uint32_t z, uint32_t w) {
  const uint32_t d = z & 0xffffffu;
  return (x == 0xffffffffu || d == kBallNoDist) ? ~0ull : make_key(d, (z >> 24) | ((w >> 16) << 8));
}
RM_HD void ball_pack(uint64_t k0, uint64_t k1, uint32_t& y, uint32_t& z, uint32_t& w) {
  const uint32_t d0 = k0 == ~0ull ? kBallNoDist : key_dist(k0), t0 = k0 == ~0ull ? 0u : key_time(k0);
  const uint32_t d1 = k1 == ~0ull ? kBallNoDist : key_dist(k1), t1 = k1 == ~0ull ? 0u : key_time(k1);
  y = d0 | (t0 & 0xffu) << 24;
  z = d1 | (t1 & 0xffu) << 24;
  w = (t0 >> 8) | (t1 >> 8) << 16;
}
RM_HD bool ball_key_fits(uint64_t k) { return key_dist(k) <= kBallMaxField && key_time(k) <= kBallMaxField; }

constexpr int kMaxCand = 16;
constexpr float kMaxSearchRadius = 200.f;
constexpr uint32_t kRouteInvalid = 0xffffffffu;

struct MatchOptions {
  int32_t mode;
  float sigma_z;
  float beta;
  float search_radius;
  float gps_accuracy;
  float breakage_distance;
  float interpolation_distance;
  float max_route_distance_factor;
  float max_route_time_factor;
  float turn_penalty_factor;
};
constexpr const char* kTurnPenaltyError = "turn_penalty_factor must be non-negative and finite";
RM_HD bool turn_factor_ok(float f) { return f >= 0.f && f - f == 0.f; }

RM_HD MatchOptions default_options() {
  MatchOptions o;
  o.mode = kModeAuto; o.sigma_z = 4.07f; o.beta = 3.f; o.search_radius = 50.f; o.gps_accuracy = 5.f;
  o.breakage_distance = 2000.f; o.interpolation_distance = 10.f; o.max_route_distance_factor = 5.f;
  o.max_route_time_factor = 2.f; o.turn_penalty_factor = 0.f;
  return o;
}

struct SegmentRec {
  uint64_t segment_id;
  double start_time;
  double end_time;
  int32_t length;
  int32_t queue_length;
  uint32_t flags;
  uint32_t begin_shape_index;
  uint32_t end_shape_index;
  uint32_t seg_dense;
  uint32_t way_first;
  uint32_t way_last;
};
static_assert(sizeof(SegmentRec) == 56, "SegmentRec layout is shared with oracle/meili_oracle.h");

struct ReportRec {
  uint64_t id;
  uint64_t next_id;
  double t0, t1;
  int32_t length, queue_length;
  uint32_t seg_dense;
  uint32_t pad;
};
static_assert(sizeof(ReportRec) == 48, "ReportRec layout is shared with oracle/meili_oracle.h");

struct TravRec {
  uint32_t e, b, en, slot;
  double tb, te;
  uint32_t sd, soff, len, way;
};
static_assert(sizeof(TravRec) == 48, "TravRec is three dwordx4");
constexpr uint32_t kTravInternal = 1u << 31, kTravLast = 1u << 30, kTravSlotMask = kTravLast - 1u;

struct ReportStats {
  int32_t successful_count, unreported_count;
  int32_t successful_length_m, unreported_length_m;
  int32_t discontinuities, invalid_speeds, invalid_times, unassociated;
  int32_t shape_used;
  int32_t n_reports;
};

struct MatchedPoint {
  float lon, lat;
  float sq;
  uint32_t edge;
  uint32_t off_cm;
  uint32_t way;
  uint32_t type;
  uint32_t route_cm;
};
static_assert(sizeof(MatchedPoint) == 32, "MatchedPoint is two dwordx4");

constexpr int kHistBins = 16;

}
```

reporter_amd/engine.py:

```python
import ctypes as C
import os

import numpy as np

from . import _lib

SEGMENT_DTYPE = np.dtype([
    ("segment_id", "<u8"), ("start_time", "<f8"), ("end_time", "<f8"), ("length", "<i4"),
    ("queue_length", "<i4"), ("flags", "<u4"), ("begin_shape_index", "<u4"), ("end_shape_index", "<u4"),
    ("seg_dense", "<u4"), ("way_first", "<u4"), ("way_last", "<u4")])
assert SEGMENT_DTYPE.itemsize == 56

REPORT_DTYPE = np.dtype([
    ("id", "<u8"), ("next_id", "<u8"), ("t0", "<f8"), ("t1", "<f8"), ("length", "<i4"),
    ("queue_length", "<i4"), ("seg_dense", "<u4"), ("pad", "<u4")])
assert REPORT_DTYPE.itemsize == 48

STATS_DTYPE = np.dtype([
    ("successful_count", "<i4"), ("unreported_count", "<i4"), ("successful_length_m", "<i4"),
    ("unreported_length_m", "<i4"), ("discontinuities", "<i4"), ("invalid_speeds", "<i4"),
    ("invalid_times", "<i4"), ("unassociated", "<i4"), ("shape_used", "<i4"), ("n_reports", "<i4")])
assert STATS_DTYPE.itemsize == 40

MATCHED_POINT_DTYPE = np.dtype([
# ... 67 lines not shown

    def grid_split(self):
        out = np.zeros(1, np.uint32)
        _lib.check(_lib.lib().rm_engine_grid_split(self._h, out.ctypes.data))
        return int(out[0])

    def grid_alt(self):
        f = np.zeros(1, np.uint32)
        r = np.zeros(1, np.float32)
        _lib.check(_lib.lib().rm_engine_grid_alt(self._h, f.ctypes.data, r.ctypes.data))
        return int(f[0]), float(r[0])

    def ball_lookup(self, mode, from_nodes, roads, preds=False):
        f = _c(from_nodes, np.uint32)
        r = _c(roads, np.uint32)
        keys = np.empty((len(f), 2), np.uint64)
        pr = np.empty((len(f), 2), np.uint8)
        _lib.check(_lib.lib().rm_engine_ball_lookup(self._h, int(mode), len(f), f.ctypes.data, r.ctypes.data,
                                                    keys.ctypes.data, pr.ctypes.data if preds else None))
        return (keys, pr) if preds else keys

    def close(self):
        if getattr(self, "_h", None):
            _lib.lib().rm_engine_destroy(self._h)
            self._h = None

    def __del__(self):
        self.close()


def _c(a, dt):
    return np.ascontiguousarray(a, dtype=dt)


class BatchMatcher:

    def __init__(self, engine):
        self.engine = engine
        self._h = _lib.lib().rm_runner_create(engine._h)
        if not self._h:
            raise _lib.RmError(_lib.last_error())
        self._keep = None

    def close(self):
        if getattr(self, "_h", None):
            _lib.lib().rm_runner_destroy(self._h)
            self._h = None

    def __del__(self):
        self.close()

    @staticmethod
    def run_params(threshold_sec=15.0, report_levels=(0, 1), transition_levels=(0, 1), hist_dev=None,
                   do_report=True, zero_hist=False, dur_dev=None):
        rp = _lib.RmRunParams()
        rp.threshold_sec = threshold_sec
        rp.report_mask = levels_mask(report_levels)
        rp.transition_mask = levels_mask(transition_levels)
        rp.hist_dev = hist_dev or None
        rp.do_report = 1 if do_report else 0
        rp.zero_hist = 1 if zero_hist else 0
        rp.dur_dev = dur_dev or None
        return rp

    def run(self, trace_off, lon, lat, time, accuracy=None, opts=None, trace_opt=None, **rp_kw):
        trace_off = _c(trace_off, np.uint32)
        T = len(trace_off) - 1
        P = int(trace_off[-1])
        lon = _c(lon, np.float32)
        lat = _c(lat, np.float32)
        time = _c(time, np.float64)
        accuracy = _c(np.full(P, -1.0, np.float32) if accuracy is None else accuracy, np.float32)
        opts = default_options(1) if opts is None else _c(opts, OPTIONS_DTYPE)
        trace_opt = np.zeros(T, np.uint32) if trace_opt is None else _c(trace_opt, np.uint32)
        if not (len(lon) == len(lat) == len(time) == len(accuracy) == P):
            raise ValueError("point arrays must all have trace_off[-1] elements")
        if len(trace_opt) != T:
            raise ValueError("trace_opt must have one entry per trace")
        d = _lib.RmBatchDesc(T, trace_off.ctypes.data, lon.ctypes.data, lat.ctypes.data, time.ctypes.data,
                             accuracy.ctypes.data, len(opts), opts.ctypes.data, trace_opt.ctypes.data)
        self._keep = (trace_off, lon, lat, time, accuracy, opts, trace_opt)
        rp = self.run_params(**rp_kw)
        _lib.check(_lib.lib().rm_runner_run(self._h, C.byref(d), C.byref(rp)))
        return self

    def run_points(self, uuid, time, lon, lat, accuracy=None, inactivity=120.0, opts=None, uuid_opt=None, n_uuids=None,
                   **rp_kw):
        uuid = _c(uuid, np.uint32)
        n = len(uuid)
        time = _c(time, np.float64)
        lon = _c(lon, np.float32)
        lat = _c(lat, np.float32)
        accuracy = None if accuracy is None else _c(accuracy, np.float32)
        if not (len(time) == len(lon) == len(lat) == n) or (accuracy is not None and len(accuracy) != n):
            raise ValueError("point arrays must have equal lengths")
        nu = int(n_uuids if n_uuids is not None else (int(uuid.max()) + 1 if n else 0))
        opts = default_options(1) if opts is None else _c(opts, OPTIONS_DTYPE)
        uuid_opt = None if uuid_opt is None else _c(uuid_opt, np.uint32)
        if uuid_opt is not None and len(uuid_opt) != nu:
            raise ValueError("uuid_opt must have one entry per vehicle")
        d = _lib.RmPointsDesc(n, uuid.ctypes.data, time.ctypes.data, lon.ctypes.data, lat.ctypes.data,
                              accuracy.ctypes.data if accuracy is not None else None, float(inactivity), nu, len(opts),
                              opts.ctypes.data, uuid_opt.ctypes.data if uuid_opt is not None else None)
        self._keep = (uuid, time, lon, lat, accuracy, opts, uuid_opt)
        rp = self.run_params(**rp_kw)
        _lib.check(_lib.lib().rm_runner_run_points(self._h, C.byref(d), C.byref(rp)))
        return self

    def trace_uuid(self):
        out = np.empty(self.sizes()["traces"], np.uint32)
        _lib.check(_lib.lib().rm_runner_get_trace_uuid(self._h, out.ctypes.data))
        return out

    def batch(self):
        sz = self.sizes()
        P, T = sz["points"], sz["traces"]
        off = np.empty(T + 1, np.uint32)
        lon, lat, acc = (np.empty(P, np.float32) for _ in range(3))
        time = np.empty(P, np.float64)
        _lib.check(_lib.lib().rm_runner_get_batch(self._h, off.ctypes.data, lon.ctypes.data, lat.ctypes.data,
                                                  time.ctypes.data, acc.ctypes.data))
        return dict(trace_off=off, lon=lon, lat=lat, time=time, accuracy=acc)

    def tiles(self, quantisation=3600, privacy=2, source="smpl_rprt", mode="auto", comm=None):
        tp = _lib.RmTileParams(int(quantisation), int(privacy), source.encode(), mode.encode())
        blob = C.c_void_p()
        n = C.c_size_t()
        _lib.check(_lib.lib().rm_runner_tiles(self._h, C.byref(tp), comm._h if comm is not None else None,
                                              C.byref(blob), C.byref(n)))
        try:
            raw = C.string_at(blob.value, n.value) if n.value else b""
        finally:
            _lib.lib().rm_free(blob)
        parts = raw.split(b"\0")
        return {parts[i].decode(): parts[i + 1].decode() for i in range(0, len(parts) - 1, 2)}

    def rerun(self, **rp_kw):
        rp = self.run_params(**rp_kw)
        _lib.check(_lib.lib().rm_runner_rerun(self._h, C.byref(rp)))

    def sizes(self):
        out = (C.c_uint64 * 10)()
        _lib.check(_lib.lib().rm_runner_sizes(self._h, out))
        return dict(zip(("points", "traces", "transitions", "path_edges", "segments", "reports", "routes_tier2",
                         "routes_tier3", "paths_tier2", "cand_tier2"), [int(x) for x in out]))

    def route_tiers(self):
        out = (C.c_uint64 * 10)()
        _lib.check(_lib.lib().rm_runner_route_tiers(self._h, out))
        return dict(zip(("ball_to_search", "lane_to_tier2", "tier2_to_wave", "paths_ball_to_search",
                         "wave_to_global", "paths_wave_to_global", "group_to_wave512", "paths_group_to_wave512",
                         "wave512_to_wave4096", "paths_wave512_to_wave4096"), [int(x) for x in out]))

    def states(self):
        s = self.sizes()
        n_states = np.empty(s["traces"], np.uint32)
        orig = np.empty(s["points"], np.uint32)
        _lib.check(_lib.lib().rm_runner_get_states(self._h, n_states.ctypes.data, orig.ctypes.data))
        return n_states, orig

    def candidates(self):
        P = self.sizes()["points"]
        n = np.empty(P, np.uint8)
        road = np.empty(P * MAX_CAND, np.uint32)
        s = np.empty(P * MAX_CAND, np.uint32)
        sq = np.empty(P * MAX_CAND, np.float32)
        _lib.check(_lib.lib().rm_runner_get_candidates(self._h, n.ctypes.data, road.ctypes.data, s.ctypes.data,
                                                       sq.ctypes.data))
        return n, road.reshape(P, MAX_CAND), s.reshape(P, MAX_CAND), sq.reshape(P, MAX_CAND)

    def routes(self):
        sz = self.sizes()
        off = np.empty(sz["points"], np.uint32)
        gc = np.empty(sz["points"], np.float64)
        route = np.empty(max(sz["transitions"], 1), np.uint32)
        _lib.check(_lib.lib().rm_runner_get_routes(self._h, off.ctypes.data, gc.ctypes.data, route.ctypes.data))
        return off, gc, route[: sz["transitions"]]

    def route_terms(self):
        n = self.sizes()["transitions"]
        out = np.empty(max(n, 1), np.float64)
        present = C.c_int(0)
        _lib.check(_lib.lib().rm_runner_get_route_terms(self._h, out.ctypes.data, C.byref(present)))
        return out[:n] if present.value else None

    def viterbi(self):
        P = self.sizes()["points"]
        choice = np.empty(P, np.int8)
        cs = np.empty(P, np.uint8)
        _lib.check(_lib.lib().rm_runner_get_viterbi(self._h, choice.ctypes.data, cs.ctypes.data))
        return choice, cs

    def paths(self):
        sz = self.sizes()
        off = np.empty(sz["points"], np.uint32)
        cnt = np.empty(sz["points"], np.uint32)
        pool = np.empty(max(sz["path_edges"], 1), np.uint32)
        dist = np.empty(sz["points"], np.uint32)
        _lib.check(_lib.lib().rm_runner_get_paths(self._h, off.ctypes.data, cnt.ctypes.data, pool.ctypes.data,
                                                  dist.ctypes.data))
        return off, cnt, pool, dist

    def segments(self):
        sz = self.sizes()
        off = np.empty(sz["traces"] + 1, np.uint32)
        segs = np.empty(max(sz["segments"], 1), SEGMENT_DTYPE)
        _lib.check(_lib.lib().rm_runner_get_segments(self._h, off.ctypes.data, segs.ctypes.data))
        return off, segs[: sz["segments"]]

    def matched_points(self):
        out = np.empty(self.sizes()["points"], MATCHED_POINT_DTYPE)
        _lib.check(_lib.lib().rm_runner_get_matched_points(self._h, out.ctypes.data))
        return out

    def reports(self):
        sz = self.sizes()
        off = np.empty(sz["traces"] + 1, np.uint32)
        reps = np.empty(max(sz["reports"], 1), REPORT_DTYPE)
        stats = np.empty(sz["traces"], STATS_DTYPE)
        _lib.check(_lib.lib().rm_runner_get_reports(self._h, off.ctypes.data, reps.ctypes.data, stats.ctypes.data))
        return off, reps[: sz["reports"]], stats

    def set_isolation(self, on=True):
        _lib.check(_lib.lib().rm_runner_set_isolation(self._h, 1 if on else 0))

    def set_locality(self, mode):
        _lib.check(_lib.lib().rm_runner_set_locality(self._h, int(mode)))

    def locality_used(self):
        v = C.c_int(0)
        _lib.check(_lib.lib().rm_runner_locality_used(self._h, C.byref(v)))
        return bool(v.value)

    def trace_errors(self):
        out = np.zeros(self.sizes()["traces"], np.uint32)
        _lib.check(_lib.lib().rm_runner_trace_errors(self._h, out.ctypes.data))
        return out

    def set_timing(self, on=True):
        _lib.check(_lib.lib().rm_runner_set_timing(self._h, 1 if on else 0))

    def set_timing_stages(self, names):
        n = _lib.lib().rm_num_kernels()
        idx = {_lib.lib().rm_kernel_name(i).decode(): i for i in range(n)}
        mask = 0
        for nm in names:
            mask |= 1 << idx[nm]
        _lib.check(_lib.lib().rm_runner_set_timing_mask(self._h, mask))

    def reset_times(self):
        _lib.check(_lib.lib().rm_runner_reset_times(self._h))

    def kernel_times(self):
        n = _lib.lib().rm_num_kernels()
        ms = np.zeros(n, np.float64)
        la = np.zeros(n, np.uint64)
        _lib.check(_lib.lib().rm_runner_kernel_times(self._h, ms.ctypes.data, la.ctypes.data, n))
        names = [_lib.lib().rm_kernel_name(i).decode() for i in range(n)]
        return {names[i]: (float(ms[i]), int(la[i])) for i in range(n)}


def split_by_points(trace_off, parts):
    trace_off = np.asarray(trace_off, np.uint64)
    T = len(trace_off) - 1
    P = int(trace_off[-1]) if T >= 0 else 0
    cuts = [0] + [int(np.searchsorted(trace_off, P * k / parts)) for k in range(1, max(1, int(parts)))] + [T]
    return sorted(set(min(max(c, 0), T) for c in cuts))


class MultiMatcher:

    def __init__(self, engine, parts=2):
        self.engine = engine
        self.parts = max(1, int(parts))
        self.bms = []

    def run(self, trace_off, lon, lat, time, accuracy=None, opts=None, trace_opt=None, **rp_kw):
        trace_off = np.asarray(trace_off, np.uint64)
        T = len(trace_off) - 1
        P = int(trace_off[-1])
        accuracy = np.full(P, -1.0, np.float32) if accuracy is None else np.asarray(accuracy, np.float32)
        trace_opt = np.zeros(T, np.uint32) if trace_opt is None else np.asarray(trace_opt, np.uint32)
        cuts = split_by_points(trace_off, self.parts)
        for bm in self.bms:
            bm.close()
        self.bms = []
        zero = rp_kw.pop("zero_hist", False)
        if zero and rp_kw.get("hist_dev"):
            _lib.check(_lib.lib().rm_device_memset(rp_kw["hist_dev"], 0, self.engine.n_segments * 16 * 4))
        if zero and rp_kw.get("dur_dev"):
            _lib.check(_lib.lib().rm_device_memset(rp_kw["dur_dev"], 0, self.engine.n_segments * 8))
        for t0, t1 in zip(cuts[:-1], cuts[1:]):
            if t1 <= t0:
                continue
            o0, o1 = int(trace_off[t0]), int(trace_off[t1])
            bm = BatchMatcher(self.engine)
            bm.run(trace_off[t0:t1 + 1] - o0, lon[o0:o1], lat[o0:o1], time[o0:o1], accuracy[o0:o1], opts,
                   trace_opt[t0:t1], **rp_kw)
            self.bms.append(bm)
        return self

    def rerun(self, **rp_kw):
        rp = BatchMatcher.run_params(**rp_kw)
        hs = (C.c_void_p * len(self.bms))(*[bm._h for bm in self.bms])
        _lib.check(_lib.lib().rm_runners_rerun(hs, len(self.bms), C.byref(rp)))

# ... 83 lines not shown
```

Baseline: 2.037 billion.

## Skip clean fallback route/path tiers in steady runs and fuse scan kernels

In steady reruns, when the previous two runs sent no work to the fallback route or path tiers, those tier kernels are skipped. Gate bits make the ball kernels abort if work would have overflowed, and a host check then forces a full rerun. The three-kernel scans are replaced by a bucketed base scan with apply kernels that also fill src_item and rec_slot, removing k_src_items, k_scan_parts and k_rec_slot. Per-point initialisation (choice, path_cnt, state_time) moves into the state-building kernel. The cost is a possible full rerun when the skip guess is wrong.

```diff
diff --git a/include/reporter_match.h b/include/reporter_match.h
--- a/include/reporter_match.h
+++ b/include/reporter_match.h
@@ -128,6 +128,8 @@
 int rm_runners_rerun(rm_runner* const* rs, uint32_t n, const rm_run_params* p);
 int rm_runner_sizes(rm_runner* r, uint64_t out[10]);
 int rm_runner_route_tiers(rm_runner* r, uint64_t out[10]);
+int rm_runner_run_stats(rm_runner* r, uint64_t out[4]);
+int rm_scan_block_bases(const uint64_t* part, uint32_t nb, uint32_t lanes, uint64_t* base);
 int rm_runner_get_states(rm_runner* r, uint32_t* n_states, uint32_t* state_orig);
 int rm_runner_get_candidates(rm_runner* r, uint8_t* cand_n, uint32_t* road, uint32_t* s_cm, float* sq);
 int rm_runner_get_routes(rm_runner* r, uint32_t* trans_off, double* gc, uint32_t* route_cm);
diff --git a/reporter_amd/_lib.py b/reporter_amd/_lib.py
--- a/reporter_amd/_lib.py
+++ b/reporter_amd/_lib.py
@@ -116,6 +116,8 @@
     ("rm_engine_turn_rows", C.c_int, [P, P, P]),
     ("rm_engine_ball_lookup", C.c_int, [P, C.c_int, C.c_uint64, P, P, P, P]),
     ("rm_runner_route_tiers", C.c_int, [P, P]),
+    ("rm_runner_run_stats", C.c_int, [P, P]),
+    ("rm_scan_block_bases", C.c_int, [P, C.c_uint32, C.c_uint32, P]),
     ("rm_balls_lookup", C.c_int, [C.c_char_p, C.c_int, C.c_double, C.c_uint64, P, P, P, P]),
     ("rm_graph_auto_ball_radius", C.c_int, [C.c_char_p, P]),
     ("rm_graph_fit_ball_radius", C.c_int, [C.c_char_p, C.c_int, C.c_double, C.c_double, P]),
diff --git a/reporter_amd/csrc/capi.cpp b/reporter_amd/csrc/capi.cpp
--- a/reporter_amd/csrc/capi.cpp
+++ b/reporter_amd/csrc/capi.cpp
@@ -1275,6 +1275,27 @@
 #endif
   });
 }
+int rm_runner_run_stats(rm_runner* r, uint64_t out[4]) { return guarded([&] { r->m->run_stats(out); }); }
+int rm_scan_block_bases(const uint64_t* part, uint32_t nb, uint32_t lanes, uint64_t* base) {
+  return guarded([&] {
+    if (!lanes) throw std::invalid_argument("lanes must be positive");
+    std::vector<unsigned long long> p(2 * (size_t)nb), bkt(2 * (size_t)scan_buckets(nb) + 2, 0ull);
+    for (size_t i = 0; i < p.size(); ++i) p[i] = part[i];
+    for (uint32_t q = 0; q < nb; ++q) {
+      bkt[2 * (size_t)scan_bucket(q)] += p[2 * (size_t)q];
+      bkt[2 * (size_t)scan_bucket(q) + 1] += p[2 * (size_t)q + 1];
+    }
+    for (uint32_t q = 0; q < nb; ++q) {
+      unsigned long long a = 0, c = 0;
+      for (uint32_t l = 0; l < lanes; ++l) {
+        unsigned long long la, lc;
+        scan_base_lane(p.data(), bkt.data(), q, l, lanes, la, lc);
+        a += la; c += lc;
+      }
+      base[2 * (size_t)q] = a; base[2 * (size_t)q + 1] = c;
+    }
+  });
+}
 int rm_runner_get_states(rm_runner* r, uint32_t* a, uint32_t* b) { return guarded([&] { r->m->get_states(a, b); }); }
 int rm_runner_get_candidates(rm_runner* r, uint8_t* a, uint32_t* b, uint32_t* c, float* d) {
   return guarded([&] { r->m->get_candidates(a, b, c, d); });
diff --git a/reporter_amd/csrc/engine.hip b/reporter_amd/csrc/engine.hip
--- a/reporter_amd/csrc/engine.hip
+++ b/reporter_amd/csrc/engine.hip
@@ -62,14 +62,14 @@
 };
 
 __device__ __forceinline__ bool steady_abort(const DevBatch& b) {
-  return (b.gate & 4u) && (b.tot[0] > b.trans_cap || b.tot[1] > b.src_cap);
+  return ((b.gate & 4u) && (b.tot[0] > b.trans_cap || b.tot[1] > b.src_cap)) || ((b.gate & 8u) && b.ctl[1] != 0u);
 }
 
 __device__ __forceinline__ bool small_abort(const DevBatch& b) {
   if (!b.gate) return false;
   const uint32_t* c = b.ctl;
   return (c[2] & kErrPathOverflow) != 0u || ((b.gate & 2u) && (c[9] | c[10]) != 0u) || b.tot[2] > b.seg_cap ||
-         steady_abort(b);
+         ((b.gate & 16u) && c[8] != 0u) || steady_abort(b);
 }
 
 __device__ __forceinline__ void trace_fail(const DevBatch& b, uint64_t p, uint32_t bit) {
@@ -227,20 +227,23 @@
   float c1lo = 0.f, c1la = 0.f, c2lo = 0.f, c2la = 0.f;
   const uint32_t nl = n ? n - 1u : 0u;
   float nlo = b.lon[o + min((uint32_t)lane, nl)], nla = b.lat[o + min((uint32_t)lane, nl)];
+  double ntm = b.time[o + min((uint32_t)lane, nl)];
   bool w_slot = false, w_state = false, w_gc = false;
   uint32_t w_i = 0, w_si = 0;
-  double w_gcv = 0.0;
+  double w_gcv = 0.0, w_tm = 0.0;
   for (uint32_t c0 = 0; c0 < n; c0 += 64) {
     const uint32_t i = c0 + lane, m = min(64u, n - c0);
     const bool act = i < n;
     float lo = act ? nlo : 0.f, la = act ? nla : 0.f;
-    __asm__ volatile("" : "+v"(lo), "+v"(la) : : "memory");
-    if (w_slot) b.slot_trace[o + w_i] = k;
-    if (w_state) b.state_orig[o + w_si] = w_i;
+    double tm = act ? ntm : 0.0;
+    __asm__ volatile("" : "+v"(lo), "+v"(la), "+v"(tm) : : "memory");
+    if (w_slot) { b.slot_trace[o + w_i] = k; b.choice[o + w_i] = -1; b.path_cnt[o + w_i] = 0u; }
+    if (w_state) { b.state_orig[o + w_si] = w_i; b.state_time[o + w_si] = w_tm; }
     if (w_gc) b.gc[o + w_si] = w_gcv;
     __asm__ volatile("" : : : "memory");
     nlo = b.lon[o + min(i + 64u, nl)];
     nla = b.lat[o + min(i + 64u, nl)];
+    ntm = b.time[o + min(i + 64u, nl)];
     w_slot = act;
     w_i = i;
     float lo1 = __shfl_up(lo, 1, 64), la1 = __shfl_up(la, 1, 64);
@@ -297,6 +300,7 @@
       q = nq + 1;
     }
     w_state = ((st >> lane) & 1ull) != 0ull;
+    w_tm = tm;
     w_gc = false;
     if (w_state) {
       const unsigned long long below = st & ((1ull << lane) - 1ull);
@@ -316,8 +320,8 @@
     c1lo = lane_f(lo, 63); c1la = lane_f(la, 63);
     c2lo = lane_f(lo, 62); c2la = lane_f(la, 62);
   }
-  if (w_slot) b.slot_trace[o + w_i] = k;
-  if (w_state) b.state_orig[o + w_si] = w_i;
+  if (w_slot) { b.slot_trace[o + w_i] = k; b.choice[o + w_i] = -1; b.path_cnt[o + w_i] = 0u; }
+  if (w_state) { b.state_orig[o + w_si] = w_i; b.state_time[o + w_si] = w_tm; }
   if (w_gc) b.gc[o + w_si] = w_gcv;
   if (lane == 0) b.n_states[k] = ns;
 }
@@ -814,21 +818,17 @@
   const uint64_t p = (uint64_t)blockIdx.x * blockDim.x + threadIdx.x;
   uint32_t c = 0, ns = 0;
   if (p < b.P) {
-    b.choice[p] = -1;
-    b.path_cnt[p] = 0u;
     const uint32_t k = b.slot_trace[p];
     const uint32_t o = b.trace_off[k];
     const uint32_t s = (uint32_t)(p - o);
     const uint32_t S = b.n_states[k];
-    if (s < S) b.state_time[p] = b.time[o + b.state_orig[p]];
     if (s >= 1 && s < S) {
       const uint32_t KA = b.cand_n[p - 1], KB = b.cand_n[p];
       c = KA * KB;
       ns = KB ? KA : 0u;
-      const uint32_t pa = o + b.state_orig[p - 1], pb = o + b.state_orig[p];
       const double gc = b.gc[p];
       const MatchOptions op = b.opts[b.trace_opt[k]];
-      b.pair_info[p] = make_uint4(route_bound(gc, op), time_bound(b.time[pb] - b.time[pa], op),
+      b.pair_info[p] = make_uint4(route_bound(gc, op), time_bound(b.state_time[p] - b.state_time[p - 1], op),
                                   KA | (KB << 8) | ((uint32_t)op.mode << 16),
                                   op.turn_penalty_factor > 0.f ? __float_as_uint(op.turn_penalty_factor) : 0u);
     }
@@ -922,6 +922,107 @@
       if (o + q < b.seg_cap) rec_slot[o + q] = (uint32_t)x;
     o += c;
   }
+}
+
+__global__ void __launch_bounds__(256) k_scan_buckets(const unsigned long long* part, uint32_t nb, unsigned long long* bkt) {
+  const uint32_t g = blockIdx.x * 4u + (threadIdx.x >> 6);
+  if (g >= scan_buckets(nb)) return;
+  const uint32_t q = g * kScanGroup + (threadIdx.x & 63u);
+  static_assert(kScanGroup == 64, "one lane per partial of the bucket");
+  unsigned long long a = q < nb ? part[2 * (uint64_t)q] : 0ull, c = q < nb ? part[2 * (uint64_t)q + 1] : 0ull;
+#pragma unroll
+  for (int d = 32; d > 0; d >>= 1) {
+    a += __shfl_down(a, d, 64); c += __shfl_down(c, d, 64);
+  }
+  if ((threadIdx.x & 63u) == 0) { bkt[2 * (uint64_t)g] = a; bkt[2 * (uint64_t)g + 1] = c; }
+}
+
+__device__ __forceinline__ void block_base_parts(const unsigned long long* part, const unsigned long long* bkt,
+                                                 unsigned long long* pre) {
+  __shared__ unsigned long long s[4][2];
+  unsigned long long a, c;
+  scan_base_lane(part, bkt, blockIdx.x, threadIdx.x, blockDim.x, a, c);
+#pragma unroll
+  for (int d = 32; d > 0; d >>= 1) {
+    a += __shfl_down(a, d, 64); c += __shfl_down(c, d, 64);
+  }
+  const int wv = threadIdx.x >> 6;
+  if ((threadIdx.x & 63) == 0) { s[wv][0] = a; s[wv][1] = c; }
+  __syncthreads();
+  pre[0] = s[0][0] + s[1][0] + s[2][0] + s[3][0];
+  pre[1] = s[0][1] + s[1][1] + s[2][1] + s[3][1];
+}
+
+__global__ void __launch_bounds__(256) k_trans_apply_steady(DevBatch b, const unsigned long long* part,
+                                                            const unsigned long long* bkt, unsigned long long* tot) {
+  const uint64_t p = (uint64_t)blockIdx.x * 256u + threadIdx.x;
+  const uint32_t va = p < b.P ? b.trans_cnt[p] : 0u, vc = p < b.P ? b.src_cnt[p] : 0u;
+  unsigned long long pre[2];
+  block_base_parts(part, bkt, pre);
+  __shared__ uint32_t sa[4], sc[4];
+  const int lane = threadIdx.x & 63, wv = threadIdx.x >> 6;
+  uint32_t ia = va, ic = vc;
+#pragma unroll
+  for (int d = 1; d < 64; d <<= 1) {
+    const uint32_t ta = __shfl_up(ia, d, 64), tc = __shfl_up(ic, d, 64);
+    if (lane >= d) { ia += ta; ic += tc; }
+  }
+  if (lane == 63) { sa[wv] = ia; sc[wv] = ic; }
+  __syncthreads();
+  uint32_t ba = 0, bc = 0;
+#pragma unroll
+  for (int w = 0; w < 4; ++w) {
+    ba += w < wv ? sa[w] : 0u;
+    bc += w < wv ? sc[w] : 0u;
+  }
+  if (p < b.P) {
+    const unsigned long long at = pre[1] + bc + ic - vc;
+    b.trans_off[p] = (uint32_t)(pre[0] + ba + ia - va);
+    b.src_off[p] = (uint32_t)at;
+    for (uint32_t i = 0; i < vc; ++i)
+      if (at + i < b.src_cap) b.src_item[at + i] = (uint32_t)p;
+  }
+  if (blockIdx.x == gridDim.x - 1 && threadIdx.x == 255) {
+    tot[0] = pre[0] + ba + ia;
+    tot[1] = pre[1] + bc + ic;
+  }
+}
+
+__global__ void __launch_bounds__(256) k_path_apply_steady(DevBatch b, const unsigned long long* part,
+                                                           const unsigned long long* bkt, unsigned long long* tot,
+                                                           uint32_t* rec_slot) {
+  __shared__ unsigned long long sa[4], sc[4];
+  const uint64_t n = b.P;
+  const uint64_t i = ((uint64_t)blockIdx.x * 256u + threadIdx.x) * 4u;
+  uint32_t v[4] = {0u, 0u, 0u, 0u};
+  if (i + 4 <= n) {
+    const uint4 q = *reinterpret_cast<const uint4*>(b.path_cnt + i);
+    v[0] = q.x; v[1] = q.y; v[2] = q.z; v[3] = q.w;
+  } else {
+    for (uint64_t x = i; x < n; ++x) v[x - i] = b.path_cnt[x];
+  }
+  unsigned long long pre[2];
+  block_base_parts(part, bkt, pre);
+  const unsigned long long mine = (unsigned long long)v[0] + v[1] + v[2] + v[3];
+  unsigned long long ea, ec;
+  block_excl_scan2(mine, 0ull, ea, ec, sa, sc, 4);
+  const unsigned long long base = pre[0] + ea;
+  const uint32_t o0 = (uint32_t)base, o1 = o0 + v[0], o2 = o1 + v[1], o3 = o2 + v[2];
+  if (i + 4 <= n) {
+    *reinterpret_cast<uint4*>(b.trav_off + i) = make_uint4(o0, o1, o2, o3);
+  } else {
+    const uint32_t o[4] = {o0, o1, o2, o3};
+    for (uint64_t x = i; x < n; ++x) b.trav_off[x] = o[x - i];
+  }
+  unsigned long long o = base;
+#pragma unroll
+  for (int j = 0; j < 4; ++j) {
+    const uint32_t c = v[j];
+    for (uint32_t q = 0; q < c; ++q)
+      if (o + q < b.seg_cap) rec_slot[o + q] = (uint32_t)(i + j);
+    o += c;
+  }
+  if (blockIdx.x == gridDim.x - 1 && threadIdx.x == 255) tot[2] = base + mine;
 }
 
 __global__ void __launch_bounds__(64) k_gather_recs(uint32_t T, const uint32_t* base, const uint32_t* cnt,
@@ -4635,6 +4736,7 @@
     w.trace_err = dalloc<uint32_t>(L, ct);
     w.tot64 = dalloc<unsigned long long>(L, 4);
     w.tot_part = dalloc<unsigned long long>(L, 2 * ((cp + 255) / 256) + 2);
+    w.scan_bkt = dalloc<unsigned long long>(L, 2 * (scan_buckets((uint32_t)((cp + 255) / 256)) + 1));
     w.cap_points = cp; w.cap_traces = ct; w.cap_opts = co;
     w.gsearch = nullptr;
     w.route = nullptr; w.route_d = nullptr; w.cap_turn = 0; w.walk = nullptr; w.cap_walk = 0; w.rl_routes_a = nullptr; w.rl_routes_b = nullptr; w.rl_routes_0 = nullptr; w.rl_routes_c = nullptr; w.path_pool = nullptr; w.segs = nullptr; w.reps = nullptr; w.src_item = nullptr; w.rec_slot = nullptr;
@@ -5265,6 +5367,17 @@
   locality_used_ = false;
   const uint32_t count_grid = (uint32_t)((P + 255) / 256);
   const uint32_t sum_grid = (uint32_t)((P + 1023) / 1024);
+  const bool balls = (mode_mask_ & g.ball_mask) != 0u;
+  const char* tiers_env = std::getenv("RM_STEADY_TIERS");
+  const bool may_skip = balls && !(tiers_env && *tiers_env == '0');
+  const bool skip_routes = may_skip && clean_routes_ >= 2;
+  const bool skip_paths = may_skip && clean_paths_ >= 2;
+  if (skip_paths) v.gate |= 16u;
+  DevBatch vk = v;
+  if (skip_routes) v.gate |= 8u;
+  ++run_stats_[0];
+  if (skip_routes) ++run_stats_[2];
+  if (skip_paths) ++run_stats_[3];
   static const bool prev_grids = [] { const char* e = std::getenv("RM_STEADY_GRIDS"); return !(e && *e == '0'); }();
   const auto sgrid = [&](uint32_t full, int word, uint32_t per_block) {
     if (!prev_grids) return (uint32_t)(full == 2048u ? 2048u : tier_grid(P, full));
@@ -5283,34 +5396,37 @@
   toc(kKCandidates);
   tic(kKScan);
   hipLaunchKernelGGL(k_trans_count, dim3(count_grid), dim3(256), 0, st, v, w.tot_part);
-  hipLaunchKernelGGL(k_scan_parts, dim3(1), dim3(1024), 0, st, w.tot_part, count_grid, w.tot64);
-  hipLaunchKernelGGL(k_scan_apply2, dim3(count_grid), dim3(256), 0, st, (const uint32_t*)w.trans_cnt,
-                     (const uint32_t*)w.src_cnt, P, (const unsigned long long*)w.tot_part, w.trans_off, w.src_off);
+  hipLaunchKernelGGL(k_scan_buckets, dim3((scan_buckets(count_grid) + 3) / 4), dim3(256), 0, st,
+                     (const unsigned long long*)w.tot_part, count_grid, w.scan_bkt);
+  hipLaunchKernelGGL(k_trans_apply_steady, dim3(count_grid), dim3(256), 0, st, v, (const unsigned long long*)w.tot_part,
+                     (const unsigned long long*)w.scan_bkt, w.tot64);
   toc(kKScan);
-  const bool balls = (mode_mask_ & g.ball_mask) != 0u;
   const uint32_t item_grid = (uint32_t)((src_cover + kK2Items - 1) / kK2Items);
   const uint32_t lane_grid = (uint32_t)((src_cover + 255) / 256);
   tic(kKRoutes);
-  hipLaunchKernelGGL(k_src_items, dim3(count_grid), dim3(256), 0, st, v);
   if (balls) {
     if (v.route_d) {
-      hipLaunchKernelGGL(k_routes_ball2<true>, dim3(item_grid), dim3(kK2Threads), 0, st, g, v, kNone);
-      hipLaunchKernelGGL(k_turn_walks, dim3(item_grid), dim3(kWalkThreads), 0, st, g, v, kNone);
-      hipLaunchKernelGGL(k_turn_walks_marked, dim3(kWalkScanGrid), dim3(256), 0, st, g, v);
+      hipLaunchKernelGGL(k_routes_ball2<true>, dim3(item_grid), dim3(kK2Threads), 0, st, g, vk, kNone);
+      hipLaunchKernelGGL(k_turn_walks, dim3(item_grid), dim3(kWalkThreads), 0, st, g, vk, kNone);
+      hipLaunchKernelGGL(k_turn_walks_marked, dim3(kWalkScanGrid), dim3(256), 0, st, g, vk);
     } else {
-      hipLaunchKernelGGL(k_routes_ball2<false>, dim3(item_grid), dim3(kK2Threads), 0, st, g, v, kNone);
-    }
-    const uint32_t lg = std::min<uint32_t>(lane_grid, sgrid(kListedGrid, 1, 256));
-    if (v.route_d) hipLaunchKernelGGL(k_routes_lane<true>, dim3(lg), dim3(256), 0, st, g, v, 0u, 1);
-    else hipLaunchKernelGGL(k_routes_lane<false>, dim3(lg), dim3(256), 0, st, g, v, 0u, 1);
+      hipLaunchKernelGGL(k_routes_ball2<false>, dim3(item_grid), dim3(kK2Threads), 0, st, g, vk, kNone);
+    }
+    if (!skip_routes) {
+      const uint32_t lg = std::min<uint32_t>(lane_grid, sgrid(kListedGrid, 1, 256));
+      if (v.route_d) hipLaunchKernelGGL(k_routes_lane<true>, dim3(lg), dim3(256), 0, st, g, v, 0u, 1);
+      else hipLaunchKernelGGL(k_routes_lane<false>, dim3(lg), dim3(256), 0, st, g, v, 0u, 1);
+    }
   } else {
     if (v.route_d) hipLaunchKernelGGL(k_routes_lane<true>, dim3(lane_grid), dim3(256), 0, st, g, v, kNone, 0);
     else hipLaunchKernelGGL(k_routes_lane<false>, dim3(lane_grid), dim3(256), 0, st, g, v, kNone, 0);
   }
-  hipLaunchKernelGGL(k_routes_reg2, dim3(sgrid(kReg2Grid, 3, 256)), dim3(256), 0, st, g, v);
-  hipLaunchKernelGGL(k_routes_grp, dim3(sgrid(kGrpGrid, 5, kWave / kGrpW)), dim3(64), 0, st, g, v, 0);
-  hipLaunchKernelGGL(k_routes_wave_s, dim3(sgrid(kMidGrid, 11, 1)), dim3(64), 0, st, g, v);
-  hipLaunchKernelGGL(k_routes_wave, dim3(sgrid(1024, 13, 1)), dim3(64), 0, st, g, v, 0);
+  if (!skip_routes) {
+    hipLaunchKernelGGL(k_routes_reg2, dim3(sgrid(kReg2Grid, 3, 256)), dim3(256), 0, st, g, v);
+    hipLaunchKernelGGL(k_routes_grp, dim3(sgrid(kGrpGrid, 5, kWave / kGrpW)), dim3(64), 0, st, g, v, 0);
+    hipLaunchKernelGGL(k_routes_wave_s, dim3(sgrid(kMidGrid, 11, 1)), dim3(64), 0, st, g, v);
+    hipLaunchKernelGGL(k_routes_wave, dim3(sgrid(1024, 13, 1)), dim3(64), 0, st, g, v, 0);
+  }
   if (w.gsearch) hipLaunchKernelGGL(k_routes_global, dim3(kGlobalGrid), dim3(64), 0, st, g, v, (GlobalPathSmem*)w.gsearch);
   toc(kKRoutes);
   tic(kKViterbi);
@@ -5319,23 +5435,26 @@
   tic(kKPaths);
   if (balls) {
     hipLaunchKernelGGL(k_paths_ball, dim3(count_grid), dim3(256), 0, st, g, v);
-    hipLaunchKernelGGL(k_paths_lane, dim3(std::min<uint32_t>(count_grid, sgrid(kListedGrid, 8, 256))), dim3(256), 0, st, g, v, 1);
+    if (!skip_paths)
+      hipLaunchKernelGGL(k_paths_lane, dim3(std::min<uint32_t>(count_grid, sgrid(kListedGrid, 8, 256))), dim3(256), 0, st, g, v, 1);
   } else {
     hipLaunchKernelGGL(k_paths_lane, dim3(count_grid), dim3(256), 0, st, g, v, 0);
   }
-  hipLaunchKernelGGL(k_paths_reg2, dim3(sgrid(kReg2Grid, 4, 256)), dim3(256), 0, st, g, v);
-  hipLaunchKernelGGL(k_paths_grp, dim3(sgrid(kGrpGrid, 6, kWave / kGrpW)), dim3(64), 0, st, g, v, 0);
-  hipLaunchKernelGGL(k_paths_wave_s, dim3(sgrid(kMidGrid, 12, 1)), dim3(64), 0, st, g, v);
-  hipLaunchKernelGGL(k_paths_wave, dim3(sgrid(1024, 14, 1)), dim3(64), 0, st, g, v, 0);
+  if (!skip_paths) {
+    hipLaunchKernelGGL(k_paths_reg2, dim3(sgrid(kReg2Grid, 4, 256)), dim3(256), 0, st, g, v);
+    hipLaunchKernelGGL(k_paths_grp, dim3(sgrid(kGrpGrid, 6, kWave / kGrpW)), dim3(64), 0, st, g, v, 0);
+    hipLaunchKernelGGL(k_paths_wave_s, dim3(sgrid(kMidGrid, 12, 1)), dim3(64), 0, st, g, v);
+    hipLaunchKernelGGL(k_paths_wave, dim3(sgrid(1024, 14, 1)), dim3(64), 0, st, g, v, 0);
+  }
   if (w.gsearch) hipLaunchKernelGGL(k_paths_global, dim3(kGlobalGrid), dim3(64), 0, st, g, v, (GlobalPathSmem*)w.gsearch);
   toc(kKPaths);
   tic(kKSegments);
   hipLaunchKernelGGL(k_sum_u64, dim3(sum_grid), dim3(256), 0, st, w.path_cnt, P, w.tot_part);
-  hipLaunchKernelGGL(k_scan_parts, dim3(1), dim3(1024), 0, st, w.tot_part, sum_grid, w.tot64 + 2);
-  hipLaunchKernelGGL(k_scan_apply4, dim3(sum_grid), dim3(256), 0, st, (const uint32_t*)w.path_cnt, P,
-                     (const unsigned long long*)w.tot_part, w.trav_off);
+  hipLaunchKernelGGL(k_scan_buckets, dim3((scan_buckets(sum_grid) + 3) / 4), dim3(256), 0, st,
+                     (const unsigned long long*)w.tot_part, sum_grid, w.scan_bkt);
+  hipLaunchKernelGGL(k_path_apply_steady, dim3(sum_grid), dim3(256), 0, st, v, (const unsigned long long*)w.tot_part,
+                     (const unsigned long long*)w.scan_bkt, w.tot64, w.rec_slot);
   if (rp.do_report && rp.zero_hist) zero_hist(rp);
-  hipLaunchKernelGGL(k_rec_slot, dim3(count_grid), dim3(256), 0, st, v, w.rec_slot);
   hipLaunchKernelGGL(k_seg_wave, dim3(T), dim3(64), 0, st, g, v, (const uint32_t*)w.rec_slot, kNone, report_args(rp));
   toc(kKSegments);
   RM_HIP(hipGetLastError());
@@ -5343,13 +5462,16 @@
   RM_HIP(hipMemcpyAsync(htot, w.tot64, 3 * sizeof(unsigned long long), hipMemcpyDeviceToHost, st));
   sync();
   if (htot[0] > w.cap_trans || htot[1] > src_cover || (hctl_[2] & kErrPathOverflow) ||
-      (!w.gsearch && (hctl_[9] | hctl_[10])) || htot[2] > v.seg_cap)
+      (!w.gsearch && (hctl_[9] | hctl_[10])) || htot[2] > v.seg_cap || (skip_routes && hctl_[1]) ||
+      (skip_paths && hctl_[8])) {
+    ++run_stats_[1];
     return false;
+  }
   n_trans_ = htot[0];
   n_path_ = htot[2];
   seg_used_ = htot[2];
   steady_src_ = htot[1];
-  std::memcpy(steady_ctl_, hctl_, sizeof(steady_ctl_));
+  keep_ctl();
   has_report_ = rp.do_report != 0;
   err_bits_ = hctl_[2] & (kErrCandOverflow | kErrSearchOverflow | kErrRounds);
   if (err_bits_ && !isolate_) throw std::runtime_error(error_text(err_bits_));
@@ -5567,7 +5689,9 @@
   has_report_ = rp.do_report != 0;
   if (!locality_used_) {
     steady_src_ = steady_next;
-    std::memcpy(steady_ctl_, hctl_, sizeof(steady_ctl_));
+    keep_ctl();
+  } else {
+    count_clean(hctl_);
   }
   err_bits_ = hctl_[2] & (kErrCandOverflow | kErrSearchOverflow | kErrRounds);
   if (err_bits_ && !isolate_) throw std::runtime_error(error_text(err_bits_));
@@ -5687,6 +5811,19 @@
   }
 }
 
+void Matcher::keep_ctl() {
+  std::memcpy(steady_ctl_, hctl_, sizeof(steady_ctl_));
+  count_clean(steady_ctl_);
+}
+void Matcher::count_clean(const uint32_t* c) {
+  clean_routes_ = (c[1] | c[3] | c[5] | c[11] | c[13]) ? 0u : std::min(clean_routes_ + 1u, 2u);
+  clean_paths_ = (c[8] | c[4] | c[6] | c[12] | c[14]) ? 0u : std::min(clean_paths_ + 1u, 2u);
+}
+
+void Matcher::run_stats(uint64_t* out4) const {
+  for (int i = 0; i < 4; ++i) out4[i] = run_stats_[i];
+}
+
 void Matcher::ctl_words(uint32_t* out) {
   sync();
   for (int i = 0; i < kCtlWords; ++i) out[i] = 0;
diff --git a/reporter_amd/csrc/engine.hpp b/reporter_amd/csrc/engine.hpp
--- a/reporter_amd/csrc/engine.hpp
+++ b/reporter_amd/csrc/engine.hpp
@@ -133,6 +133,7 @@
   uint32_t* rl_routes_c = nullptr; uint32_t* rl_paths_c = nullptr; void* gsearch = nullptr;
   uint32_t* trace_err = nullptr;
   unsigned long long* tot64 = nullptr;
+  unsigned long long* scan_bkt = nullptr;
   unsigned long long* tot_part = nullptr;
   uint64_t cap_sort = 0;
   uint32_t* perm = nullptr; uint16_t* loc_key = nullptr; uint32_t* loc_cursor = nullptr; uint32_t* pcnt = nullptr;
@@ -246,6 +247,7 @@
   void kernel_times(double* ms, uint64_t* launches);
   void tier_counts(uint32_t* out4);
   void ctl_words(uint32_t* out);
+  void run_stats(uint64_t* out4) const;
   void reset_kernel_times();
   void set_timing(bool on) { timing_mask_ = on ? ~0u : 0u; }
   void set_timing_mask(uint32_t mask) { timing_mask_ = mask; }
@@ -296,6 +298,10 @@
   bool run_steady(const RunParams& rp, const DevGraph& g);
   uint64_t steady_src_ = 0;
   uint32_t steady_ctl_[16] = {0};
+  uint32_t clean_routes_ = 0, clean_paths_ = 0;
+  uint64_t run_stats_[4] = {0, 0, 0, 0};
+  void keep_ctl();
+  void count_clean(const uint32_t* ctl);
   void zero_hist(const RunParams& rp);
   void use_ws_inputs();
   void ensure_pack(uint64_t bytes);
diff --git a/reporter_amd/csrc/rm_common.hpp b/reporter_amd/csrc/rm_common.hpp
--- a/reporter_amd/csrc/rm_common.hpp
+++ b/reporter_amd/csrc/rm_common.hpp
@@ -364,4 +364,15 @@
 
 constexpr int kHistBins = 16;
 
-}
+constexpr uint32_t kScanGroup = 64;
+RM_HD uint32_t scan_bucket(uint32_t blk) { return blk / kScanGroup; }
+RM_HD uint32_t scan_buckets(uint32_t nb) { return (nb + kScanGroup - 1) / kScanGroup; }
+RM_HD void scan_base_lane(const unsigned long long* part, const unsigned long long* bkt, uint32_t blk, uint32_t lane,
+                          uint32_t lanes, unsigned long long& a, unsigned long long& c) {
+  const uint32_t g = scan_bucket(blk);
+  a = 0; c = 0;
+  for (uint32_t q = lane; q < g; q += lanes) { a += bkt[2 * q]; c += bkt[2 * q + 1]; }
+  for (uint32_t q = g * kScanGroup + lane; q < blk; q += lanes) { a += part[2 * q]; c += part[2 * q + 1]; }
+}
+
+}
diff --git a/reporter_amd/engine.py b/reporter_amd/engine.py
--- a/reporter_amd/engine.py
+++ b/reporter_amd/engine.py
@@ -243,6 +243,12 @@
                          "wave_to_global", "paths_wave_to_global", "group_to_wave512", "paths_group_to_wave512",
                          "wave512_to_wave4096", "paths_wave512_to_wave4096"), [int(x) for x in out]))
 
+    def run_stats(self):
+        out = (C.c_uint64 * 4)()
+        _lib.check(_lib.lib().rm_runner_run_stats(self._h, out))
+        return dict(zip(("steady", "steady_rerun", "routes_tiers_skipped", "paths_tiers_skipped"),
+                        [int(x) for x in out]))
+
     def states(self):
         s = self.sizes()
         n_states = np.empty(s["traces"], np.uint32)
```

After: 2.088 billion (median of 6 runs). 2.5% higher.
